# TopAY-Planner/TopAY

Hardware: AMD Instinct MI355X
Metric: trajectories/sec to L-BFGS convergence (benchmark_tables batch) at 1/2/4/8 GPU (higher is better)
Workload: dtype f64

## Files before the change

### topay_amd/csrc/topay_eval.h

```cpp
#pragma once

#include "topay_esdf.h"
#include "topay_eval_ctx.h"
#include "topay_mani.h"
#include "topay_math.h"
#include "topay_minco.h"
#include "topay_wave.h"

namespace topay {

struct GradGate {
  bool always;
  bool has_early;
  double finit, thr , early ;
  bool early_ok;
  double skip_thr;
  __device__ __forceinline__ bool needs(double f) const {
    if (always) return true;
    if (isinf(f) || isnan(f)) return false;
    if (has_early && fabs(finit - f) / (fabs(finit) + 1.0) < early) return true;
    return !(f > thr);
  }
};

struct Basis {
  double b0[6], b1[6], b2[6], b3[6];
};
__device__ __forceinline__ void make_basis(double s1, Basis& B) {
  const double s2 = s1 * s1, s3 = s2 * s1, s4 = s2 * s2, s5 = s3 * s2;
  B.b0[0] = 1.0; B.b0[1] = s1; B.b0[2] = s2; B.b0[3] = s3; B.b0[4] = s4; B.b0[5] = s5;
  B.b1[0] = 0.0; B.b1[1] = 1.0; B.b1[2] = 2.0 * s1; B.b1[3] = 3.0 * s2; B.b1[4] = 4.0 * s3; B.b1[5] = 5.0 * s4;
  B.b2[0] = 0.0; B.b2[1] = 0.0; B.b2[2] = 2.0; B.b2[3] = 6.0 * s1; B.b2[4] = 12.0 * s2; B.b2[5] = 20.0 * s3;
  B.b3[0] = 0.0; B.b3[1] = 0.0; B.b3[2] = 0.0; B.b3[3] = 6.0; B.b3[4] = 24.0 * s1; B.b3[5] = 60.0 * s2;
}
__device__ __forceinline__ void poly4(lds_cdp cL, int rows, int i, int d, const Basis& B, double& p0, double& p1,
                                      double& p2, double& p3) {
  lds_cdp c = cL + d * rows + 6 * i;
  const double c0 = c[0], c1 = c[1], c2 = c[2], c3 = c[3], c4 = c[4], c5 = c[5];
  p0 = fma(c5, B.b0[5], fma(c4, B.b0[4], fma(c3, B.b0[3], fma(c2, B.b0[2], fma(c1, B.b0[1], c0)))));
  p1 = fma(c5, B.b1[5], fma(c4, B.b1[4], fma(c3, B.b1[3], fma(c2, B.b1[2], c1))));
  p2 = fma(c5, B.b2[5], fma(c4, B.b2[4], fma(c3, B.b2[3], c2 * B.b2[2])));
  p3 = fma(c5, B.b3[5], fma(c4, B.b3[4], c3 * B.b3[3]));
}
__device__ __forceinline__ void poly3(lds_cdp cL, int rows, int i, int d, const Basis& B, double& p0, double& p1,
                                      double& p2) {
  lds_cdp c = cL + d * rows + 6 * i;
  const double c0 = c[0], c1 = c[1], c2 = c[2], c3 = c[3], c4 = c[4], c5 = c[5];
  p0 = fma(c5, B.b0[5], fma(c4, B.b0[4], fma(c3, B.b0[3], fma(c2, B.b0[2], fma(c1, B.b0[1], c0)))));
  p1 = fma(c5, B.b1[5], fma(c4, B.b1[4], fma(c3, B.b1[3], fma(c2, B.b1[2], c1))));
  p2 = fma(c5, B.b2[5], fma(c4, B.b2[4], fma(c3, B.b2[3], c2 * B.b2[2])));
}

__device__ __forceinline__ void xy_integrand(lds_cdp cL, int rows, int i, double s1, double& fx, double& fy) {
  const double s2 = s1 * s1, s3 = s2 * s1, s4 = s2 * s2, s5 = s3 * s2;
  lds_cdp ct = cL + 0 * rows + 6 * i;
  lds_cdp cs = cL + 1 * rows + 6 * i;
  const double th = fma(ct[5], s5, fma(ct[4], s4, fma(ct[3], s3, fma(ct[2], s2, fma(ct[1], s1, ct[0])))));
  const double sd = fma(cs[5], 5.0 * s4, fma(cs[4], 4.0 * s3, fma(cs[3], 3.0 * s2, fma(cs[2], 2.0 * s1, cs[1]))));
  double sn, cn;
  det_sincos(th, &sn, &cn);
  fx = sd * cn;
  fy = sd * sn;
}

__device__ __forceinline__ void kinodynamic_block(dev_params_ref P, double wM, double wA, double wD, double omg,
                                                  double step, double real_alpha, double th1, double th2, double th3,
                                                  double sd1, double sd2, double sd3, double& cost, double& gdT,
                                                  double& gth1, double& gth2, double& gs1, double& gs2) {
  const double mu = P.relu_mu;
  const double max_v = P.max_v, max_w = P.max_w, max_a = P.max_a, max_dw = P.max_dw;
  const double w = omg * step;
#pragma unroll
  for (int sgn = -1; sgn <= 1; sgn += 2) {
    const double v = sgn * max_v * th1 + max_w * sd1 - P.max_vw;
    if (v > 0) {
      double pe, pd;
      smoothL1(P, v, mu, pe, pd);
      const double gt = real_alpha * (sgn * max_v * th2 + max_w * sd2);
      gth1 += w * wM * pd * sgn * max_v;
      gs1 += w * wM * pd * max_w;
      gdT += omg * wM * (pd * gt * step + pe * TOPAY_INV_K);
      cost += w * wM * pe;
    }
  }
#pragma unroll
  for (int sgn = -1; sgn <= 1; sgn += 2) {
    const double v = sgn * max_v * th1 - max_w * sd1 - P.max_vw;
    if (v > 0) {
      double pe, pd;
      smoothL1(P, v, mu, pe, pd);
      const double gt = real_alpha * (sgn * max_v * th2 - max_w * sd2);
      gth1 += w * wM * pd * sgn * max_v;
      gs1 -= w * wM * pd * max_w;
      gdT += omg * wM * (pd * gt * step + pe * TOPAY_INV_K);
      cost += w * wM * pe;
    }
  }
  const double vAcc = sd2 * sd2 - P.max_a2;
  const double vAlp = th2 * th2 - P.max_dw2;
  if (vAcc > 0) {
    double pe, pd;
    smoothL1(P, vAcc, mu, pe, pd);
    const double gt = 2.0 * real_alpha * sd2 * sd3;
    gs2 += w * wA * pd * 2.0 * sd2;
    gdT += omg * wA * (pd * gt * step + pe * TOPAY_INV_K);
    cost += w * wA * pe;
  }
  if (vAlp > 0) {
    double pe, pd;
    smoothL1(P, vAlp, mu, pe, pd);
    const double gt = 2.0 * real_alpha * th2 * th3;
    gth2 += w * wD * pd * 2.0 * th2;
    gdT += omg * wD * (pd * gt * step + pe * TOPAY_INV_K);
    cost += w * wD * pe;
  }
}

__device__ __forceinline__ void basis_k(int k, double s, double& b0, double& b1, double& b2) {
  double pm2 = 1.0, pm1 = 1.0, p = 1.0;
#pragma unroll
  for (int t = 1; t <= 5; t++) {
    if (t <= k) p *= s;
    if (t <= k - 1) pm1 *= s;
    if (t <= k - 2) pm2 *= s;
  }
  b0 = p;
  b1 = (k >= 1) ? (double)k * pm1 : 0.0;
  b2 = (k >= 2) ? (double)(k * (k - 1)) * pm2 : 0.0;
}

template <int OCC>
__device__ __forceinline__ ManiOut sample_mani(lds_cdp cL, int rows, int i, int j, int e, bool act, double step, double half, double posx,
                                               double posy, const TOPAY_GLB DevMap* mp, glb_dp mstash, lds_dp mg_lds) {
  ManiOut mo_;
  if (topay_opaque_true()) mo_ = manipulator_block<OCC>(mp, cL, rows, i, j, half, step, posx, posy, act ? e : -1, mstash, mg_lds);
  return mo_;
}

template <int STAGE>
__device__ __forceinline__ void sample_rest(dev_params_ref P, lds_cdp cL, int rows, int i, int j, double step, double half, double posx, double posy,
                                            const TOPAY_GLB DevMap* mp, double wM, double wA, double wD, const ManiOut& mo_, lds_cdp mg_lds,
                                            double (&gB)[12], double& gdTs, double& gpx, double& gpy, bool& jva, double& cst) {
#pragma unroll
  for (int v = 0; v < 12; v++) gB[v] = 0.0;
  gdTs = 0.0; gpx = 0.0; gpy = 0.0;
  jva = false;
  Basis B;
  make_basis(j * half, B);
  const double omg = (j == 0 || j == 2 * TOPAY_K) ? 0.5 : 1.0;
  const double real_alpha = 1.0 / TOPAY_K * ((double)j / 2.0);
  double th0, th1, th2, th3, s0, sd1, sd2, sd3;
  poly4(cL, rows, i, 0, B, th0, th1, th2, th3);
  poly4(cL, rows, i, 1, B, s0, sd1, sd2, sd3);
  cst = 0.0;
  kinodynamic_block(P, wM, wA, wD, omg, step, real_alpha, th1, th2, th3, sd1, sd2, sd3, cst, gdTs, gB[1], gB[2],
                    gB[3], gB[4]);
  if (STAGE == 2) {
    double d2, g2x, g2y;
    {
      const DevMap M = load_map(mp);
      esdf2d_query(M, posx, posy, d2, g2x, g2y);
    }
    const double viola = P.chassis_r105 - d2;
    if (viola > 0) {
      double pe, pd;
      smoothL1(P, viola, P.relu_mu, pe, pd);
      const double sc = -omg * step * P.s2_collision_weight * pd;
      gpx += sc * g2x;
      gpy += sc * g2y;
      gdTs += omg * P.s2_collision_weight * (pe * TOPAY_INV_K);
      cst += omg * step * P.s2_collision_weight * pe;
    }
    double qacc = 0.0;
#pragma unroll
    for (int q = 0; q < 7; q++) {
      double a0, a1, a2, a3;
      poly4(cL, rows, i, 2 + q, B, a0, a1, a2, a3);
      const double vDq = a1 * a1 - P.joint_vel_limit2[q];
      const double vD2q = a2 * a2 - P.joint_acc_limit2[q];
      if (vDq > 0) {
        double pe, pd;
        smoothL1(P, vDq, P.relu_mu, pe, pd);
        gdTs += omg * P.s2_mani_vel_weight * (pd * (2.0 * real_alpha * a1 * a2) * step + pe * TOPAY_INV_K);
        cst += omg * step * P.s2_mani_vel_weight * pe;
        jva = true;
      }
      if (vD2q > 0) {
        double pe, pd;
        smoothL1(P, vD2q, P.relu_mu, pe, pd);
        gdTs += omg * P.s2_mani_acc_weight * (pd * (2.0 * real_alpha * a2 * a3) * step + pe * TOPAY_INV_K);
        cst += omg * step * P.s2_mani_acc_weight * pe;
        jva = true;
      }
      const double mgq = mg_lds[q * 64];
      gB[5 + q] = mgq;
      qacc += mgq * a1;
    }
    cst = cst + mo_.cost;
    gdTs = gdTs + mo_.gdT;
    gpx += mo_.gx;
    gpy += mo_.gy;
    gB[0] = mo_.gth;
    gdTs += mo_.gth * th1 * real_alpha;
    gdTs += qacc * real_alpha;
  }
}

template <int STAGE, int RMAX, int NW, int OCC = 1>
__device__ __noinline__ TOPAY_CALLS_BIG_FUNCTIONS double eval_cost_grad(EvalCtx& C, const TOPAY_GLB DevMap* mp, const GradGate gate) {
  constexpr int NT = 64 * NW;
  const lds_dp c_Tp = uniform_ptr(C.Tp);
  const lds_dp c_X = uniform_ptr(C.X);
  const double c_ex = uniform_f64(C.ex);
  const double c_ey = uniform_f64(C.ey);
  const glb_dp c_g = uniform_ptr(C.g);
  const lds_dp c_gdT = uniform_ptr(C.gdT);
  const glb_cdp c_init_xy = uniform_ptr(C.init_xy);
  const double c_lam0 = uniform_f64(C.lam0);
  const double c_lam1 = uniform_f64(C.lam1);
  const glb_dp c_lu = uniform_ptr(C.lu);
  const lds_dp c_pcs = uniform_ptr(C.pcs);
  const lds_dp c_pw = uniform_ptr(C.pw);
  const double c_rho0 = uniform_f64(C.rho0);
  const double c_rho1 = uniform_f64(C.rho1);
  const double c_sx = uniform_f64(C.sx);
  const double c_sy = uniform_f64(C.sy);
  const glb_cdp c_x = uniform_ptr(C.x);
  const lds_dp c_red = uniform_ptr(C.red);
  const lds_dp c_adj = uniform_ptr(C.adj);
  const glb_dp c_coefg = uniform_ptr(C.coefg);

  dev_params_ref P = dev_params();
  int lane = C.lane, tid = C.tid;
  const int wave = __builtin_amdgcn_readfirstlane(C.wave);
  const int N = __builtin_amdgcn_readfirstlane(C.N), rows = __builtin_amdgcn_readfirstlane(C.rows);
  lds_cdp cL = uniform_ptr(C.cL);
  const glb_dp c_sbuf = uniform_ptr(C.sbuf);
  const glb_dp c_mstash = uniform_ptr(C.mstash);
  const int c_sbs = __builtin_amdgcn_readfirstlane(C.sb_stride);
  const double g_skip_thr = uniform_f64(gate.skip_thr);
  const bool g_early_ok = __builtin_amdgcn_readfirstlane(gate.early_ok ? 1 : 0) != 0;
  GradGate ugate;
  ugate.always = __builtin_amdgcn_readfirstlane(gate.always ? 1 : 0) != 0;
  ugate.has_early = __builtin_amdgcn_readfirstlane(gate.has_early ? 1 : 0) != 0;
  ugate.finit = uniform_f64(gate.finit); ugate.thr = uniform_f64(gate.thr); ugate.early = uniform_f64(gate.early);
  ugate.early_ok = g_early_ok; ugate.skip_thr = g_skip_thr;
  int rp = 0;
  const int npl = __builtin_amdgcn_readfirstlane(C.npass_lds);
  constexpr int RD = eval_red_doubles(NW);
  const lds_dp ptot = c_red + RD;
  const lds_dp csr = c_red + RD + 2 * npl;
  TOPAY_LDS unsigned long long* jmask = (TOPAY_LDS unsigned long long*)(c_red + RD + 2 * npl + (NW > 1 ? 2 * NW * 64 : 0));
  constexpr int PBR = eval_pb_rows(NW);
  minco_generate<NW, OCC>(C);

  auto jerk_terms = [&](int i, double& e_out, double& gdT_out) __attribute__((always_inline)) {
    double w33 = 0, w43 = 0, w44 = 0, w53 = 0, w54 = 0, w55 = 0;
#pragma unroll
    for (int d = 0; d < 9; d++) {
      const double c3 = cL[d * rows + 6 * i + 3], c4 = cL[d * rows + 6 * i + 4], c5 = cL[d * rows + 6 * i + 5];
      const double e = P.energy_weights[d];
      w33 += (c3 * e) * c3; w43 += (c4 * e) * c3; w44 += (c4 * e) * c4;
      w53 += (c5 * e) * c3; w54 += (c5 * e) * c4; w55 += (c5 * e) * c5;
    }
    const double T1 = c_Tp[i], T2 = c_Tp[N + i], T3 = c_Tp[2 * N + i], T4 = c_Tp[3 * N + i], T5 = c_Tp[4 * N + i];
    e_out = 36.0 * w33 * T1 + 144.0 * w43 * T2 + 192.0 * w44 * T3 + 240.0 * w53 * T3 + 720.0 * w54 * T4 + 720.0 * w55 * T5;
    gdT_out = 36.0 * w33 + 288.0 * w43 * T1 + 576.0 * w44 * T2 + 720.0 * w53 * T2 + 2880.0 * w54 * T3 + 3600.0 * w55 * T4;
  };
  double jerk_e = 0.0;
  if (tid < N) {
    double unused_;
    jerk_terms(tid, jerk_e, unused_);
  }
  const double jerk_cost = wg_sum<NW>(c_red, rp, wave, jerk_e);

  lds_dp gxy = c_X;
  lds_dp pball = c_X + 26 * N;
  lds_dp pbuf = pball + wave * (PBR * 64);
  const int NE = TOPAY_EP * N;
  const int npass = (NE + 63) / 64;
  const int nround = (npass + NW - 1) / NW;
  const double wT = STAGE == 1 ? P.s1_time_weight : P.s2_time_weight;
  const double time_cost = wT * wg_sum<NW>(c_red, rp, wave, tid < N ? c_Tp[tid] : 0.0);
  bool skip_body = false;
  double f_skip = 0.0;
  if (STAGE == 2 && g_early_ok) {
    const double partial = jerk_cost + time_cost;
    if (partial > g_skip_thr && partial <= 1.79769313486231570e308) {
      skip_body = true;
      f_skip = partial;
    }
  }
  const double wM = STAGE == 1 ? P.s1_moment_weight : P.s2_moment_weight;
  const double wA = STAGE == 1 ? P.s1_acc_weight : P.s2_acc_weight;
  const double wD = STAGE == 1 ? P.s1_domega_weight : P.s2_domega_weight;

  STAMP(C, 3);
  for (int k = 0; k < nround; k++) {
    const int pass = k * NW + wave;
    if (pass < npass) {
      const int e = pass * 64 + lane;
      const bool act = e < NE;
      const int i = act ? e / TOPAY_EP : N - 1;
      const int m = act ? e - TOPAY_EP * i : 0;
      const int j = 2 * m;
      const double T1 = c_Tp[i];
      const double step = T1 / TOPAY_K, half = step / 2.0, coeff = step / 6.0;
      double f0x, f0y, Ix = 0.0, Iy = 0.0;
      xy_integrand(cL, rows, i, j * half, f0x, f0y);
      if (act && m < TOPAY_K) {
        double f1x, f1y, f2x, f2y;
        xy_integrand(cL, rows, i, (j + 1) * half, f1x, f1y);
        xy_integrand(cL, rows, i, (j + 2) * half, f2x, f2y);
        Ix = coeff * f0x + 4 * coeff * f1x + coeff * f2x;
        Iy = coeff * f0y + 4 * coeff * f1y + coeff * f2y;
      }
      const double incx = wave_incl_scan(Ix, lane), incy = wave_incl_scan(Iy, lane);
      if (act) {
        gxy[2 * e] = incx - Ix;
        gxy[2 * e + 1] = incy - Iy;
      }
      if (lane == 63) {
        ptot[2 * pass] = incx;
        ptot[2 * pass + 1] = incy;
      }
    }
  }
  wg_barrier<NW>();

  double carryx = 0.0, carryy = 0.0;
  int pc = 0;
  double cost_pen = 0.0;
  for (int k = 0; k < nround; k++) {
    const int pass = k * NW + wave;
    double cst_out = 0.0;
    if (pass < npass) {
      while (pc < pass) {
        carryx = uniform_f64(carryx + ptot[2 * pc]);
        carryy = uniform_f64(carryy + ptot[2 * pc + 1]);
        pc++;
      }
      int e, i, m, j;
      bool act;
      double step, half, posx, posy;
      auto geometry = [&](int ln) __attribute__((always_inline)) {
        e = pass * 64 + ln;
        act = e < NE;
        i = act ? e / TOPAY_EP : N - 1;
        m = act ? e - TOPAY_EP * i : 0;
        j = 2 * m;
        const double T1 = c_Tp[i];
        step = T1 / TOPAY_K;
        half = step / 2.0;
        const double px0 = act ? gxy[2 * e] : 0.0, py0 = act ? gxy[2 * e + 1] : 0.0;
        posx = c_sx + (carryx + px0);
        posy = c_sy + (carryy + py0);
      };
      geometry(lane);
      if (act && m == TOPAY_K) {
        c_pcs[2 * N + 2 * (i + 1)] = posx;
        c_pcs[2 * N + 2 * (i + 1) + 1] = posy;
      }
      if (!skip_body) {
        ManiOut mo;
        mo.gx = mo.gy = mo.gth = mo.cost = mo.gdT = 0.0;
        if (STAGE == 2) {
          mo = sample_mani<OCC>(cL, rows, i, j, e, act, step, half, posx, posy, mp, c_mstash, pbuf + lane);
          lane = fresh_lane_id(lane);
          tid = wave * 64 + lane;
          geometry(lane);
        }
        double gB[12], gdTs, gpx, gpy, cst;
        bool jva;
        sample_rest<STAGE>(P, cL, rows, i, j, step, half, posx, posy, mp, wM, wA, wD, mo, pbuf + lane, gB, gdTs, gpx, gpy, jva, cst);
        if (act) {
          cst_out = cst;
          gxy[2 * e] = gpx;
          gxy[2 * e + 1] = gpy;
          glb_dp sb = c_sbuf + e;
          const int ss = c_sbs;
#pragma unroll
          for (int v = 0; v < 5; v++) sb[v * ss] = gB[v];
          sb[5 * ss] = gdTs;
          if (STAGE == 2) {
#pragma unroll
            for (int v = 0; v < 7; v++) sb[(6 + v) * ss] = gB[5 + v];
            sb[13 * ss] = jva ? 1.0 : 0.0;
          }
        }
      }
    }
    lds_dp cs = csr + (k & 1) * (NW * 64);
    if (NW > 1) {
      cs[wave * 64 + lane] = cst_out;
      wg_barrier<NW>();
    }
#pragma unroll
    for (int q = 0; q < NW; q++) {
      const int p2 = k * NW + q;
      if (p2 < npass) {
        cost_pen += NW > 1 ? cs[q * 64 + lane] : cst_out;
        if (STAGE == 2 && g_early_ok && !skip_body && p2 + 1 < npass) {
          const double partial = jerk_cost + wave_sum(cost_pen) + time_cost;
          if (partial > g_skip_thr && partial <= 1.79769313486231570e308) {
            skip_body = true;
            f_skip = partial;
          }
        }
      }
    }
  }
  while (pc < npass) {
    carryx = uniform_f64(carryx + ptot[2 * pc]);
    carryy = uniform_f64(carryy + ptot[2 * pc + 1]);
    pc++;
  }
  if (NW == 1) lds_sync();
  STAMP(C, 4);

  double cost_piece = 0.0;
  double chain0x = 0.0, chain0y = 0.0;
  double mt_add_all = 0.0, mt_add_own = 0.0;
  if (STAGE == 1) {
    if (tid < N) {
      const double ex = c_pcs[2 * N + 2 * (tid + 1)] - c_init_xy[2 * tid];
      const double ey = c_pcs[2 * N + 2 * (tid + 1) + 1] - c_init_xy[2 * tid + 1];
      cost_piece = P.s1_path_pos_weight * (ex * ex + ey * ey);
      c_pcs[2 * tid] = P.s1_path_pos_weight * 2.0 * ex;
      c_pcs[2 * tid + 1] = P.s1_path_pos_weight * 2.0 * ey;
    }
    wg_barrier<NW>();
  } else {
    const double Tm = tid < N ? c_Tp[tid] : 0.0;
    const double avg = wg_sum<NW>(c_red, rp, wave, Tm) / N;
    double add_all = 0.0, add_own = 0.0;
    if (tid < N) {
      const double wMT = P.s2_mean_time_weight;
      if (Tm < avg * 0.5) {
        const double dd = Tm - avg * 0.5;
        cost_piece += wMT * dd * dd;
        add_all += wMT * 2.0 * dd * (-0.5 / N);
        add_own += wMT * 2.0 * dd;
      }
      if (Tm > avg * 2.0) {
        const double dd = Tm - avg * 2.0;
        cost_piece += wMT * dd * dd;
        add_all += wMT * 2.0 * dd * (-2.0 / N);
        add_own += wMT * 2.0 * dd;
      }
    }
    mt_add_all = add_all;
    mt_add_own = add_own;
    C.fxe0 = (c_sx + carryx) - c_ex;
    C.fxe1 = (c_sy + carryy) - c_ey;
    const double ea = C.fxe0 + c_lam0 / c_rho0, eb = C.fxe1 + c_lam1 / c_rho1;
    if (tid == 0) cost_piece += 0.5 * (c_rho0 * (ea * ea) + c_rho1 * (eb * eb));
    chain0x = c_rho0 * ea;
    chain0y = c_rho1 * eb;
  }
  double penalty_cost = wg_sum<NW>(c_red, rp, wave, (wave == 0 ? cost_pen : 0.0) + cost_piece);
  const bool bad = (STAGE == 2) && !(fabs(penalty_cost) <= 1.79769313486231570e308);
  const double f_total = jerk_cost + (bad ? 1.0e+22 : penalty_cost) + time_cost;

  STAMP(C, 5);
  if (skip_body) return f_skip;
  if (!ugate.needs(f_total)) return f_total;

  int rrow[RMAX], rpiece[RMAX], rk[RMAX];
  bool ract[RMAX];
#pragma unroll
  for (int r = 0; r < RMAX; r++) {
    rrow[r] = tid + NT * r;
    ract[r] = rrow[r] < rows;
    rpiece[r] = rrow[r] / 6;
    rk[r] = rrow[r] - 6 * rpiece[r];
  }
  double jerk_gdT = 0.0;
  if (tid < N) {
    double unused_;
    jerk_terms(tid, unused_, jerk_gdT);
  }
  double a0[RMAX], a1[RMAX], aq[RMAX][7];
  double rbh[RMAX][3];
#pragma unroll
  for (int r = 0; r < RMAX; r++) {
    a0[r] = 0.0;
    a1[r] = 0.0;
#pragma unroll
    for (int q = 0; q < 7; q++) aq[r][q] = 0.0;
    rbh[r][0] = rbh[r][1] = rbh[r][2] = 0.0;
    if (ract[r]) {
      const double hs = c_Tp[rpiece[r]] / TOPAY_K / 2.0;
      basis_k(rk[r], hs, rbh[r][0], rbh[r][1], rbh[r][2]);
    }
  }
  constexpr int NV = (STAGE == 2) ? 13 : 6;
  if constexpr (NW == 1) {
    for (int pass = 0; pass < npass; pass++) {
      const int e = pass * 64 + lane;
      const bool act = e < NE;
      const int i = act ? e / TOPAY_EP : N - 1;
      const int m = act ? e - TOPAY_EP * i : 0;
      const int j = 2 * m;
      const double step = c_Tp[i] / TOPAY_K, half = step / 2.0;
      bool jva = false;
      double rawq[7];
      {
        glb_cdp sb = c_sbuf + (act ? e : NE - 1);
        const int ss = c_sbs;
        double raw[14];
#pragma unroll
        for (int v = 0; v < ((STAGE == 2) ? 14 : 6); v++) raw[v] = sb[v * ss];
#pragma unroll
        for (int v = 0; v < 6; v++) pbuf[v * 64 + lane] = act ? raw[v] : 0.0;
#pragma unroll
        for (int v = 0; v < 7; v++) rawq[v] = (STAGE == 2 && act) ? raw[6 + v] : 0.0;
        if (STAGE == 2) jva = act && raw[13] != 0.0;
      }
      lds_sync();
#pragma unroll
      for (int r = 0; r < RMAX; r++) {
        if (ract[r]) {
          const int pi = rpiece[r];
          const double h0 = rbh[r][0], h1 = rbh[r][1], h2 = rbh[r][2];
          const int k0 = rk[r], k1 = rk[r] >= 1 ? rk[r] - 1 : 0, k2 = rk[r] >= 2 ? rk[r] - 2 : 0;
          const int e_lo = max(TOPAY_EP * pi, pass * 64), e_hi = min(min(TOPAY_EP * pi + TOPAY_EP, pass * 64 + 64), NE);
          double gt = 0.0;
          constexpr int CH = 3;
          for (int c0 = e_lo; c0 < e_hi; c0 += CH) {
            double pb[CH][6], t0[CH], t1[CH], t2[CH];
#pragma unroll
            for (int u = 0; u < CH; u++) {
              const int ee = (c0 + u < e_hi) ? c0 + u : e_hi - 1;
              const int l = ee - pass * 64, mm = ee - TOPAY_EP * pi;
              lds_cdp pj = c_pw + 12 * mm;
              t0[u] = pj[k0]; t1[u] = pj[k1]; t2[u] = pj[k2];
#pragma unroll
              for (int v = 0; v < 6; v++) pb[u][v] = pbuf[v * 64 + l];
            }
#pragma unroll
            for (int u = 0; u < CH; u++) {
              const bool ok = c0 + u < e_hi;
              const double b0 = h0 * t0[u], b1 = h1 * t1[u], b2 = h2 * t2[u];
              const double i0 = fma(b2, pb[u][2], fma(b1, pb[u][1], b0 * pb[u][0]));
              const double i1 = fma(b2, pb[u][4], b1 * pb[u][3]);
              a0[r] += ok ? i0 : 0.0;
              a1[r] += ok ? i1 : 0.0;
              gt += ok ? pb[u][5] : 0.0;
            }
          }
          if (e_lo < e_hi && rk[r] == 0) c_gdT[pi] += gt;
        }
      }
      if (STAGE == 2) {
        lds_sync();
#pragma unroll
        for (int v = 0; v < 7; v++) pbuf[v * 64 + lane] = rawq[v];
// ... 99 lines not shown
      double raw[14];
#pragma unroll
      for (int v = 0; v < ((STAGE == 2) ? 14 : 6); v++) raw[v] = sb[v * ss];
#pragma unroll
      for (int v = 0; v < 6; v++) pbuf[v * 64 + lane] = act ? raw[v] : 0.0;
      if (STAGE == 2) {
#pragma unroll
        for (int v = 0; v < 7; v++) pbuf[(6 + v) * 64 + lane] = act ? raw[6 + v] : 0.0;
        jva = act && raw[13] != 0.0;
      }
    }
    if (STAGE == 2) {
      const unsigned long long mk = __ballot(jva);
      if (lane == 0) jmask[wave] = mk;
    }
    wg_barrier<NW>();
    auto accumulate = [&](int r, int q) __attribute__((always_inline)) {
      const int p2 = k * NW + q;
      const int pi = rpiece[r];
      const double h0 = rbh[r][0], h1 = rbh[r][1], h2 = rbh[r][2];
      const int k0 = rk[r], k1 = rk[r] >= 1 ? rk[r] - 1 : 0, k2 = rk[r] >= 2 ? rk[r] - 2 : 0;
      const int e_lo = max(TOPAY_EP * pi, p2 * 64), e_hi = min(min(TOPAY_EP * pi + TOPAY_EP, p2 * 64 + 64), NE);
      if (e_lo >= e_hi) return;
      lds_cdp pq = pball + q * (PBR * 64);
      double gt = 0.0;
      constexpr int CH = 3;
      for (int c0 = e_lo; c0 < e_hi; c0 += CH) {
        double pb[CH][NV], t0[CH], t1[CH], t2[CH];
#pragma unroll
        for (int u = 0; u < CH; u++) {
          const int ee = (c0 + u < e_hi) ? c0 + u : e_hi - 1;
          const int l = ee - p2 * 64, mm = ee - TOPAY_EP * pi;
          lds_cdp pj = c_pw + 12 * mm;
          t0[u] = pj[k0]; t1[u] = pj[k1]; t2[u] = pj[k2];
#pragma unroll
          for (int v = 0; v < NV; v++) pb[u][v] = pq[v * 64 + l];
        }
#pragma unroll
        for (int u = 0; u < CH; u++) {
          const bool ok = c0 + u < e_hi;
          const double b0 = h0 * t0[u], b1 = h1 * t1[u], b2 = h2 * t2[u];
          const double i0 = fma(b2, pb[u][2], fma(b1, pb[u][1], b0 * pb[u][0]));
          const double i1 = fma(b2, pb[u][4], b1 * pb[u][3]);
          a0[r] += ok ? i0 : 0.0;
          a1[r] += ok ? i1 : 0.0;
          gt += ok ? pb[u][5] : 0.0;
          if (STAGE == 2) {
#pragma unroll
            for (int qq = 0; qq < 7; qq++) {
              const double nq = fma(b0, pb[u][6 + qq], aq[r][qq]);
              aq[r][qq] = ok ? nq : aq[r][qq];
            }
          }
        }
      }
      if (rk[r] == 0) c_gdT[pi] += gt;
    };
    unsigned long long any = 0;
    if (STAGE == 2) {
#pragma unroll
      for (int q = 0; q < NW; q++) any |= jmask[q];
    }
    if (any == 0) {
#pragma unroll
      for (int r = 0; r < RMAX; r++) {
        if (ract[r]) {
          for (int q = 0; q < NW; q++) accumulate(r, q);
        }
      }
    } else {
      for (int q = 0; q < NW; q++) {
#pragma unroll
        for (int r = 0; r < RMAX; r++) {
          if (ract[r]) accumulate(r, q);
        }
        unsigned long long todo = jmask[q];
        if (todo == 0) continue;
        wg_barrier<NW>();
        if (wave == q && jva) {
          Basis B;
          make_basis(j * half, B);
          const double omg = (j == 0 || j == 2 * TOPAY_K) ? 0.5 : 1.0;
#pragma unroll
          for (int qq = 0; qq < 7; qq++) {
            double p0, p1, p2, g1 = 0.0, g2 = 0.0;
            poly3(cL, rows, i, 2 + qq, B, p0, p1, p2);
            const double vDq = p1 * p1 - P.joint_vel_limit2[qq];
            const double vD2q = p2 * p2 - P.joint_acc_limit2[qq];
            if (vDq > 0) {
              double pe, pd;
              smoothL1(P, vDq, P.relu_mu, pe, pd);
              g1 = omg * step * P.s2_mani_vel_weight * pd * 2.0 * p1;
            }
            if (vD2q > 0) {
              double pe, pd;
              smoothL1(P, vD2q, P.relu_mu, pe, pd);
              g2 = omg * step * P.s2_mani_acc_weight * pd * 2.0 * p2;
            }
            pbuf[qq * 64 + lane] = g1;
            pbuf[(7 + qq) * 64 + lane] = g2;
          }
        }
        wg_barrier<NW>();
        lds_cdp pq = pball + q * (PBR * 64);
        while (todo) {
          const int src = __ffsll(todo) - 1;
          todo &= todo - 1;
          const int se = (k * NW + q) * 64 + src;
          const int spi = se / TOPAY_EP, smm = se - TOPAY_EP * spi;
          double b1v[7], b2v[7];
#pragma unroll
          for (int qq = 0; qq < 7; qq++) { b1v[qq] = pq[qq * 64 + src]; b2v[qq] = pq[(7 + qq) * 64 + src]; }
#pragma unroll
          for (int r = 0; r < RMAX; r++) {
            if (ract[r] && rpiece[r] == spi) {
              const int k1 = rk[r] >= 1 ? rk[r] - 1 : 0, k2 = rk[r] >= 2 ? rk[r] - 2 : 0;
              const double b1 = rbh[r][1] * c_pw[12 * smm + k1], b2 = rbh[r][2] * c_pw[12 * smm + k2];
#pragma unroll
              for (int qq = 0; qq < 7; qq++) {
                double a = aq[r][qq];
                a = fma(b1, b1v[qq], a);
                a = fma(b2, b2v[qq], a);
                aq[r][qq] = a;
              }
            }
          }
        }
      }
    }
    wg_barrier<NW>();
  }

  }
  if (STAGE == 2) {
    const double all = wg_sum<NW>(c_red, rp, wave, mt_add_all);
    if (tid < N) c_gdT[tid] += all + mt_add_own;
  }
  wg_barrier<NW>();
  if (!bad) {
    if (STAGE == 2) {
      for (int k = 0; k < nround; k++) {
        const int pass = k * NW + wave;
        if (pass < npass) {
          const int e = pass * 64 + lane;
          const bool act = e < NE;
          const double gx = act ? gxy[2 * e] : 0.0, gy = act ? gxy[2 * e + 1] : 0.0;
          const double sx_ = wave_incl_rscan(gx, lane), sy_ = wave_incl_rscan(gy, lane);
          if (lane == 0) {
            ptot[2 * pass] = sx_;
            ptot[2 * pass + 1] = sy_;
          }
        }
      }
      wg_barrier<NW>();
    }
    double rcx = chain0x, rcy = chain0y;
    pc = npass;
    for (int k = nround - 1; k >= 0; k--) {
      const int pass = k * NW + wave;
      double v0 = 0, v1 = 0, v2 = 0, v3 = 0, vT = 0;
      if (pass < npass) {
        const int e = pass * 64 + lane;
        const bool act = e < NE;
        const int i = act ? e / TOPAY_EP : N - 1;
        const int m = act ? e - TOPAY_EP * i : 0;
        const int j = 2 * m;
        double chx_in, chy_in, chx_ex, chy_ex;
        if (STAGE == 2) {
          while (pc > pass + 1) {
            pc--;
            rcx += ptot[2 * pc];
            rcy += ptot[2 * pc + 1];
          }
          const double gx = act ? gxy[2 * e] : 0.0, gy = act ? gxy[2 * e + 1] : 0.0;
          const double sx_ = wave_incl_rscan(gx, lane), sy_ = wave_incl_rscan(gy, lane);
          chx_in = sx_ + rcx; chy_in = sy_ + rcy;
          chx_ex = chx_in - gx;   chy_ex = chy_in - gy;
        } else {
          double sx_ = 0.0, sy_ = 0.0;
          for (int ii = i + 1; ii < N; ii++) { sx_ += c_pcs[2 * ii]; sy_ += c_pcs[2 * ii + 1]; }
          chx_in = chx_ex = sx_;
          chy_in = chy_ex = sy_;
        }
        if (act) {
          const double T1 = c_Tp[i];
          const double step = T1 / TOPAY_K, half = step / 2.0, coeff = step / 6.0;
          const int int_6K = TOPAY_K * 6;
#pragma unroll
          for (int odd = 0; odd < 2; odd++) {
            if (odd == 1 && m == TOPAY_K) break;
            const int jj = j + odd;
            Basis B;
            make_basis(jj * half, B);
            double th0, th1, th2, s0, sd1, sd2;
            poly3(cL, rows, i, 0, B, th0, th1, th2);
            poly3(cL, rows, i, 1, B, s0, sd1, sd2);
            double sn, cn;
            det_sincos(th0, &sn, &cn);
            const double alpha = 1.0 / (2 * TOPAY_K) * jj;
            const double W = odd ? 4.0 : ((jj == 0 || jj == 2 * TOPAY_K) ? 1.0 : 2.0);
            const double Cx = (odd ? chx_ex : chx_in) * W, Cy = (odd ? chy_ex : chy_in) * W;
            const double aTh = (-sd1 * sn * coeff) * Cx + (sd1 * cn * coeff) * Cy;
            const double aS = (cn * coeff) * Cx + (sn * coeff) * Cy;
            const double gTx = (sd2 * cn - sd1 * th1 * sn) * alpha * coeff + sd1 * cn / int_6K;
            const double gTy = (sd2 * sn + sd1 * th1 * cn) * alpha * coeff + sd1 * sn / int_6K;
            vT += gTx * Cx + gTy * Cy;
            if (odd) { v2 = aTh; v3 = aS; } else { v0 = aTh; v1 = aS; }
          }
        }
      }
      pbuf[0 * 64 + lane] = v0; pbuf[1 * 64 + lane] = v1; pbuf[2 * 64 + lane] = v2; pbuf[3 * 64 + lane] = v3;
      pbuf[4 * 64 + lane] = vT;
      wg_barrier<NW>();
#pragma unroll
      for (int r = 0; r < RMAX; r++) {
        if (ract[r]) {
          const int pi = rpiece[r];
          const double h0 = rbh[r][0], h1 = rbh[r][1];
          const int k1 = rk[r] >= 1 ? rk[r] - 1 : 0;
          for (int q = NW - 1; q >= 0; q--) {
            const int p2 = k * NW + q;
            const int e_lo = max(TOPAY_EP * pi, p2 * 64), e_hi = min(min(TOPAY_EP * pi + TOPAY_EP, p2 * 64 + 64), NE);
            if (e_lo >= e_hi) continue;
            lds_cdp pq = pball + q * (PBR * 64);
            double gt = 0.0;
            constexpr int CH = 3;
            for (int c0 = e_lo; c0 < e_hi; c0 += CH) {
              double pb[CH][5], tb[CH][4];
#pragma unroll
              for (int u = 0; u < CH; u++) {
                const int ee = (c0 + u < e_hi) ? c0 + u : e_hi - 1;
                const int l = ee - p2 * 64, mm = ee - TOPAY_EP * pi;
                lds_cdp pj = c_pw + 12 * mm;
                tb[u][0] = pj[rk[r]]; tb[u][1] = pj[k1]; tb[u][2] = pj[6 + rk[r]]; tb[u][3] = pj[6 + k1];
#pragma unroll
                for (int v = 0; v < 5; v++) pb[u][v] = pq[v * 64 + l];
              }
#pragma unroll
              for (int u = 0; u < CH; u++) {
                const bool ok = c0 + u < e_hi;
                const double b0 = h0 * tb[u][0], b1 = h1 * tb[u][1];
                const double o0 = h0 * tb[u][2], o1 = h1 * tb[u][3];
                const double i0 = fma(o0, pb[u][2], b0 * pb[u][0]);
                const double i1 = fma(o1, pb[u][3], b1 * pb[u][1]);
                a0[r] += ok ? i0 : 0.0;
                a1[r] += ok ? i1 : 0.0;
                gt += ok ? pb[u][4] : 0.0;
              }
            }
            if (rk[r] == 0) c_gdT[pi] += gt;
          }
        }
      }
      wg_barrier<NW>();
    }
  } else {
    penalty_cost = 1.0e+22;
#pragma unroll
    for (int r = 0; r < RMAX; r++) {
      a0[r] = 0.0;
      a1[r] = 0.0;
#pragma unroll
      for (int q = 0; q < 7; q++) aq[r][q] = 0.0;
    }
    if (tid < N) c_gdT[tid] = 0.0;
    wg_barrier<NW>();
  }

  STAMP(C, 6);
  double tot[RMAX][9];
#pragma unroll
  for (int r = 0; r < RMAX; r++) {
    if (ract[r]) {
      const int pi = rpiece[r], kk = rk[r];
      const double T1 = c_Tp[pi], T2 = c_Tp[N + pi], T3 = c_Tp[2 * N + pi], T4 = c_Tp[3 * N + pi], T5 = c_Tp[4 * N + pi];
#pragma unroll
      for (int d = 0; d < 9; d++) {
        double jg = 0.0;
        if (kk >= 3) {
          const double c3 = cL[d * rows + 6 * pi + 3], c4 = cL[d * rows + 6 * pi + 4], c5 = cL[d * rows + 6 * pi + 5];
          const double e = P.energy_weights[d];
          if (kk == 5) jg = 240.0 * c3 * e * T3 + 720.0 * c4 * e * T4 + 1440.0 * c5 * e * T5;
          else if (kk == 4) jg = 144.0 * c3 * e * T2 + 384.0 * c4 * e * T3 + 720.0 * c5 * e * T4;
          else jg = 72.0 * c3 * e * T1 + 144.0 * c4 * e * T2 + 240.0 * c5 * e * T3;
        }
        tot[r][d] = jg + (d == 0 ? a0[r] : (d == 1 ? a1[r] : aq[r][d >= 2 ? d - 2 : 0]));
      }
    }
  }
  for (int t = tid; t < 9 * rows; t += NT) c_coefg[t] = cL[t];
  C.cl_in_lds = 0;
  wg_global_barrier<NW>();
#pragma unroll
  for (int r = 0; r < RMAX; r++) {
    if (ract[r]) {
#pragma unroll
      for (int d = 0; d < 9; d++) c_adj[d * rows + rrow[r]] = tot[r][d];
    }
  }
  wg_barrier<NW>();
  if (wave == 0) {
    const bool owner = lane < 9;
    const lds_dp mine = c_adj + (owner ? lane : 8) * rows;
    band_sweep<2>(mine, owner, (glb_cdp)c_lu, c_X, rows, lane);
    band_sweep<3>(mine, owner, (glb_cdp)c_lu, c_X, rows, lane);
  }
  wg_barrier<NW>();
  STAMP(C, 7);
#pragma unroll
  for (int r = 0; r < RMAX; r++) {
    if (ract[r]) {
      const int row = rrow[r];
      int pi, br;
      bool use = true;
      if (row >= rows - 3) { pi = N - 1; br = 10 + (row - (rows - 3)); }
      else if (row < 3) { use = false; pi = 0; br = 0; }
      else { pi = (row - 3) / 6; br = (row - 3) - 6 * pi; }
      double part = 0.0;
      if (use) {
        const double T1 = c_Tp[pi], T2 = c_Tp[N + pi], T3 = c_Tp[2 * N + pi], T4 = c_Tp[3 * N + pi];
#pragma unroll
        for (int d = 0; d < 9; d++) {
          glb_cdp cg = c_coefg + d * rows + 6 * pi;
          const double c1 = cg[1], c2 = cg[2], c3 = cg[3], c4 = cg[4], c5 = cg[5];
          double b;
          if (br == 0) b = -(24.0 * c4 + 120.0 * T1 * c5);
          else if (br == 1) b = -120.0 * c5;
          else if (br == 2 || br == 3 || br == 10) b = -(c1 + 2.0 * T1 * c2 + 3.0 * T2 * c3 + 4.0 * T3 * c4 + 5.0 * T4 * c5);
          else if (br == 4 || br == 11) b = -(2.0 * c2 + 6.0 * T1 * c3 + 12.0 * T2 * c4 + 20.0 * T3 * c5);
          else b = -(6.0 * c3 + 24.0 * T1 * c4 + 60.0 * T2 * c5);
          part += b * c_adj[d * rows + row];
        }
      }
      c_X[row] = part;
    }
  }
  wg_barrier<NW>();
  double gdT_tot = 0.0;
  if (tid < N) {
    const int i = tid;
    double s = 0.0;
    if (i < N - 1) { for (int r = 0; r < 6; r++) s += c_X[6 * i + 3 + r]; }
    else { for (int r = 0; r < 3; r++) s += c_X[rows - 3 + r]; }
    gdT_tot = jerk_gdT + c_gdT[i] + s;
  }
  glb_cdp Tau = c_x;
  glb_cdp Vq = c_x + 3 * N - 1;
  if (tid < N) c_g[tid] = (gdT_tot + wT) * dTdTau(Tau[tid]);
  for (int t = tid; t < 9 * (N - 1); t += NT) {
    const int i = t / 9, d = t - 9 * i;
    const double gp = c_adj[d * rows + 6 * i + 5];
    const int dq = d >= 2 ? d - 2 : 0;
    if (d == 0) c_g[N + i] = gp;
    else if (d == 1) c_g[2 * N - 1 + i] = gp;
    else c_g[3 * N - 1 + 7 * i + dq] = gp * dQdVq(Vq[7 * i + dq], P.joint_pos_limit_max[dq]);
  }
  if (tid == 0) c_g[3 * N - 2] = c_adj[1 * rows + rows - 3];
  wg_global_barrier<NW>();
  STAMP(C, 8);
  return f_total;
}

}
```

### topay_amd/csrc/topay_eval_ctx.h

```cpp
#pragma once

#include <hip/hip_runtime.h>

#include "topay_types.h"

__constant__ DevParams g_P;
typedef const TOPAY_CST DevParams& dev_params_ref;
__device__ __forceinline__ dev_params_ref dev_params() {
#ifndef TOPAY_CPU_EMU
  const TOPAY_CST DevParams* p = (const TOPAY_CST DevParams*)&g_P;
  asm("" : "+s"(p));
  return *p;
#else
  return g_P;
#endif
}

namespace topay {

__device__ __forceinline__ double expC2(double tau) {
  return tau > 0.0 ? ((0.5 * tau + 1.0) * tau + 1.0) : 1.0 / ((0.5 * tau - 1.0) * tau + 1.0);
}
__device__ __forceinline__ double logC2(double T) {
  return T > 1.0 ? (sqrt(2.0 * T - 1.0) - 1.0) : (1.0 - sqrt(2.0 / T - 1.0));
}
__device__ __forceinline__ double dTdTau(double tau) {
  if (tau > 0) return tau + 1.0;
  double den = (0.5 * tau - 1.0) * tau + 1.0;
  return (1.0 - tau) / (den * den);
}
__device__ __forceinline__ double sigmoidC2(double vq, double max_q) {
  double e = expC2(vq);
  return 2.0 * max_q * e / (1.0 + e) - max_q;
}
__device__ __forceinline__ double invSigmoidC2(double q, double max_q) {
  double b = 0.5 * (max_q + q) / max_q;
  return logC2(b / (1 - b));
}
__device__ __forceinline__ double dQdVq(double vq, double max_q) {
  double e1 = expC2(vq) + 1.0;
  return 2.0 * max_q * dTdTau(vq) / (e1 * e1);
}
__device__ __forceinline__ void smoothL1(dev_params_ref P, double x, double mu, double& f, double& df) {
  if (x < mu) {
    f = (P.sl_f4c * x + P.sl_f3c) * x * x * x;
    df = (P.sl_d3c * x + P.sl_d2c) * x * x;
  } else {
    f = x - P.sl_half;
    df = 1.0;
  }
}
#define TOPAY_INV_K (1.0 / TOPAY_K)

struct EvalCtx {
  int lane, N, rows, n;
  int tid, wave;
  lds_dp red;
  lds_dp adj;
  glb_dp coefg;
  int cl_in_lds;
  lds_dp cL;
  lds_dp Tp;
  glb_cdp hd, tl;
  int npass_lds;
  lds_dp gdT;
  lds_dp pcs;
  lds_dp gC;
  glb_dp sbuf;
  int sb_stride;
  glb_dp mstash;
  lds_dp pw;
  lds_dp X;
  glb_cdp x;
  glb_dp g;
  glb_dp lu;
  glb_cdp init_xy;
  double sx, sy, ex, ey;
  double lam0, lam1, rho0, rho1;
  double fxe0, fxe1;
  TOPAY_GLB long long* stamps;
  long long t_last;
};

__device__ __forceinline__ void fill_power_table(lds_dp pw, int lane) {
  for (int t = lane; t < 156; t += 64) {
    const int jj = t / 6, k = t - 6 * jj;
    double v = 1.0;
    for (int u = 0; u < k; u++) v *= (double)jj;
    pw[t] = v;
  }
}

#ifdef TOPAY_STAMPS
#define STAMP(C, k)                                                    \
  do {                                                                 \
    const long long now_ = (long long)__builtin_amdgcn_s_memtime();    \
    if ((C).stamps && (C).lane == 0) (C).stamps[k] += now_ - (C).t_last; \
    (C).t_last = (long long)__builtin_amdgcn_s_memtime();              \
  } while (0)
#else
#define STAMP(C, k) do { } while (0)
#endif
#ifdef TOPAY_STAMPS
#define SUBSTAMP_BEGIN(C) const long long sub_t0_ = (long long)__builtin_amdgcn_s_memtime()
#define SUBSTAMP_END(C, k)                                                                                   \
  do {                                                                                                       \
    if ((C).stamps && (C).lane == 0) (C).stamps[k] += (long long)__builtin_amdgcn_s_memtime() - sub_t0_;      \
  } while (0)
#else
#define SUBSTAMP_BEGIN(C) do { } while (0)
#define SUBSTAMP_END(C, k) do { } while (0)
#endif

__host__ __device__ constexpr int eval_pb_rows(int NW) { return NW == 1 ? 7 : 14; }
__host__ __device__ constexpr int eval_npass(int Nmax) { return (TOPAY_EP * Nmax + 63) / 64; }
__host__ __device__ constexpr int eval_red_doubles(int NW) { return NW > 1 ? 8 : 0; }
__host__ __device__ constexpr int eval_misc_doubles(int Nmax, int NW) {
  return eval_red_doubles(NW) + 2 * eval_npass(Nmax) + (NW > 1 ? 2 * NW * 64 : 0) + NW;
}
__host__ __device__ constexpr int eval_union_doubles(int Nmax, int NW) {
  const int rows = 6 * Nmax;
  const int lu = 14 * rows, sw = 9 * rows + 26 * Nmax + eval_pb_rows(NW) * 64 * NW;
  return lu > sw ? lu : sw;
}
__host__ __device__ constexpr int eval_borrow_doubles(int Nmax, int NW) { return eval_union_doubles(Nmax, NW) - 9 * 6 * Nmax; }
template <typename P>
struct EvalLds {
  P Tp, gdT, pcs, pw, red, cL, adj, gC, X;
};
template <typename L, typename P>
__host__ __device__ constexpr P eval_lds_plan(L& C, P base, int Nmax, int NW) {
  const int rows = 6 * Nmax;
  P p = base;
  C.Tp = p; p += 5 * Nmax;
  C.gdT = p; p += Nmax;
  C.pcs = p; p += 4 * (Nmax + 1);
  C.pw = p; p += 156;
  C.red = p; p += eval_misc_doubles(Nmax, NW);
  C.cL = p;
  C.adj = C.cL;
  C.gC = C.adj;
  C.X = p + 9 * rows;
  return p + eval_union_doubles(Nmax, NW);
}
__host__ __device__ constexpr int eval_lds_total(int Nmax, int NW) {
  EvalLds<int> offsets{};
  return eval_lds_plan(offsets, 0, Nmax, NW);
}
__device__ __forceinline__ void eval_lds_carve(EvalCtx& C, lds_dp base, int Nmax, int NW) {
  eval_lds_plan(C, base, Nmax, NW);
  C.npass_lds = eval_npass(Nmax);
}
static_assert(eval_lds_total(10, 1) == 1515 && eval_lds_total(15, 1) == 1967 && eval_lds_total(21, 1) == 2509 &&
              eval_lds_total(32, 1) == 3503 && eval_lds_total(42, 1) == 4407 && eval_lds_total(64, 1) == 6395, "LDS plan, one wave");
static_assert(eval_lds_total(42, 2) == 6016 && eval_lds_total(64, 2) == 8004, "LDS plan, two waves");
static_assert(eval_lds_total(10, 4) == 5174 && eval_lds_total(15, 4) == 5626 && eval_lds_total(21, 4) == 6168 &&
              eval_lds_total(32, 4) == 7162 && eval_lds_total(42, 4) == 8066 && eval_lds_total(64, 4) == 10054 &&
              eval_lds_total(85, 4) == 11954 && eval_lds_total(128, 4) == 15840 && eval_lds_total(TOPAY_MAX_N, 4) == 19638,
              "LDS plan, four waves");

}
```

### topay_amd/csrc/topay_host_batch.h

```cpp

#pragma once

static topay_status run_init(topay_ctx* c) {
  const int B = c->B;
  topay_status ps = push_params(c);
  if (ps != TOPAY_OK) return ps;
  const int scratch_stride = (3 * c->Pmax + 1 + TOPAY_MAX_N) * ND;
  hipLaunchKernelGGL(k_init, dim3((B + 63) / 64), dim3(64), 0, c->stream, c->db, c->paths.as<double>(),
                     c->path_off.as<long long>(), c->path_len.as<int>(), c->bvel.as<double>(), c->bacc.as<double>(),
                     c->scratch.as<double>(), scratch_stride, TOPAY_MAX_N, kX0Stride);
  HIPCHK(hipGetLastError());
  return TOPAY_OK;
}

static topay_status set_init_traj_impl(topay_ctx* c, int batch, const int* path_len, const double* init_paths, const double* boundary_vel,
                                       const double* boundary_acc, const int* map_ids, hipMemcpyKind kind) {
  if (!c || batch <= 0 || !path_len || !init_paths) return TOPAY_ERR_INVALID_ARG;
  HIPCHK(hipSetDevice(c->device));
  if (topay_status ws = wait_pending(c)) return ws;
  c->have_traj = false;
  c->solved = false;
  std::vector<long long> off(batch + 1, 0);
  int Pmax = 0;
  for (int b = 0; b < batch; b++) {
    if (path_len[b] < 2) { set_err("every init path needs at least 2 states"); return TOPAY_ERR_INVALID_ARG; }
    off[b + 1] = off[b] + path_len[b];
    Pmax = std::max(Pmax, path_len[b]);
  }
  if (check_map_slots(c, batch, map_ids, kMapResident, "topay_set_init_traj") != TOPAY_OK) return TOPAY_ERR_NO_MAP;
  std::vector<int> mids(batch, 0);
  if (map_ids) mids.assign(map_ids, map_ids + batch);
  c->B = batch;
  c->Pmax = Pmax;
  c->h_map_id = mids;
  const size_t tot = (size_t)off[batch];
  topay_status s;
#define ENS(buf, bytes) if ((s = c->buf.ensure(bytes)) != TOPAY_OK) return s
  ENS(paths, tot * 10 * 8);
  ENS(path_off, (size_t)(batch + 1) * 8);
  ENS(path_len, (size_t)batch * 4);
  ENS(bvel, (size_t)batch * 20 * 8);
  ENS(bacc, (size_t)batch * 20 * 8);
  ENS(scratch, (size_t)batch * (3 * Pmax + 1 + TOPAY_MAX_N) * ND * 8);
  ENS(N, (size_t)batch * 4);
  ENS(s1_past, (size_t)batch * 4);
  ENS(map_id, (size_t)batch * 4);
  ENS(head, (size_t)batch * kHeadLen * 8);
  ENS(tail, (size_t)batch * kHeadLen * 8);
  ENS(start_xy, (size_t)batch * 2 * 8);
  ENS(goal_xy, (size_t)batch * 2 * 8);
  ENS(init_xy, (size_t)batch * kInitXyStride * 8);
  ENS(x0, (size_t)batch * kX0Stride * 8);
  ENS(order, (size_t)batch * 4);
  HIPCHK(copy_sync(c, c->paths.as<double>(), init_paths, tot * 10, kind));
  HIPCHK(h2d_sync(c, c->path_off.as<long long>(), off.data(), (size_t)(batch + 1)));
  HIPCHK(h2d_sync(c, c->path_len.as<int>(), path_len, (size_t)batch));
  HIPCHK(h2d_sync(c, c->map_id.as<int>(), mids.data(), (size_t)batch));
  if (boundary_vel) HIPCHK(copy_sync(c, c->bvel.as<double>(), boundary_vel, (size_t)batch * 20, kind));
  else HIPCHK(hipMemsetAsync(c->bvel.p, 0, (size_t)batch * 20 * 8, c->stream));
  if (boundary_acc) HIPCHK(h2d_sync(c, c->bacc.as<double>(), boundary_acc, (size_t)batch * 20));
  else HIPCHK(hipMemsetAsync(c->bacc.p, 0, (size_t)batch * 20 * 8, c->stream));
  DevBatch& d = c->db;
  memset(&d, 0, sizeof(d));
  d.B = batch;
  d.N = c->N.as<int>(); d.s1_past = c->s1_past.as<int>(); d.map_id = c->map_id.as<int>();
  d.head = c->head.as<double>(); d.tail = c->tail.as<double>();
  d.start_xy = c->start_xy.as<double>(); d.goal_xy = c->goal_xy.as<double>();
  d.init_xy = c->init_xy.as<double>(); d.x0 = c->x0.as<double>();
  d.order = c->order.as<int>();
  if ((s = run_init(c)) != TOPAY_OK) return s;
  HIPCHK(hipStreamSynchronize(c->stream));
  c->hN.assign(batch, 0);
  HIPCHK(d2h_sync(c, c->hN.data(), c->N.as<int>(), (size_t)batch));
  int Nmax = 0;
  for (int b = 0; b < batch; b++) {
    if (c->hN[b] <= 0) c->hN[b] = 0;
    Nmax = std::max(Nmax, c->hN[b]);
  }
  if (Nmax == 0) { set_err("every trajectory needs more pieces than TOPAY_MAX_N"); return TOPAY_ERR_TOO_MANY_PIECES; }
  c->Nmax = Nmax;
  c->h_poff.assign((size_t)batch + 1, 0);
  c->h_noff.assign((size_t)batch + 1, 0);
  for (int b = 0; b < batch; b++) {
    c->h_poff[b + 1] = c->h_poff[b] + c->hN[b];
    c->h_noff[b + 1] = c->h_noff[b] + (c->hN[b] > 0 ? 10 * c->hN[b] - 8 : 0);
  }
  const size_t P = (size_t)c->h_poff[batch], NN = (size_t)c->h_noff[batch];
  const int m = std::max(c->hp.s1_lbfgs.mem_size, c->hp.s2_lbfgs.mem_size);
  std::vector<int> idx(batch);
  std::iota(idx.begin(), idx.end(), 0);
  std::stable_sort(idx.begin(), idx.end(), [&](int a, int b2) {
    return c->hN[a] != c->hN[b2] ? c->hN[a] > c->hN[b2] : path_len[a] > path_len[b2];
  });
  for (auto& v : c->cls) v.clear();
  for (int b : idx) {
    if (c->hN[b] == 0) continue;
    c->cls[bucket_of(c->hN[b])].push_back(b);
  }
  c->h_path_len.assign(path_len, path_len + batch);
  {
    std::vector<int> ord;
    for (int k = topay_ctx::NBUCKET - 1; k >= 0; k--) ord.insert(ord.end(), c->cls[k].begin(), c->cls[k].end());
    ord.resize(batch, 0);
    HIPCHK(h2d_sync(c, c->order.as<int>(), ord.data(), (size_t)batch));
  }
  ENS(poff, ((size_t)batch + 1) * 8);
  ENS(noff, ((size_t)batch + 1) * 8);
  HIPCHK(h2d_sync(c, c->poff.as<long long>(), c->h_poff.data(), ((size_t)batch + 1)));
  HIPCHK(h2d_sync(c, c->noff.as<long long>(), c->h_noff.data(), ((size_t)batch + 1)));
  ENS(x, NN * 8);
  ENS(work, 4 * NN * 8);
  ENS(hist_s, (size_t)m * NN * 8);
  ENS(hist_y, (size_t)m * NN * 8);
  ENS(hist_ys, (size_t)batch * m * 8);
  ENS(hist_alpha, (size_t)batch * m * 8);
  ENS(lu, kLuPerPiece * P * 8);
  ENS(success, (size_t)batch * 4);
  ENS(cost, (size_t)batch * 8);
  ENS(stats, (size_t)batch * kStatsLen * 4);
  ENS(xyerr, (size_t)batch * 2 * 8);
  ENS(coef, kCoefPerPiece * P * 8);
  ENS(T, P * 8);
  ENS(knots, 2 * (P + batch) * 8);
  ENS(alm, (size_t)batch * kAlmLen * 8);
  ENS(fout, (size_t)batch * 8);
  ENS(sbuf, kSbufPerPiece * P * 8);
  ENS(mstash, kMstashPerPiece * P * 8);
  ENS(elapsed, (size_t)batch * 8);
  ENS(startus, (size_t)batch * 8);
  ENS(hwid, (size_t)batch * 4);
  ENS(feas_flags, (size_t)batch * 2 * 4);
  ENS(feas_report, (size_t)batch * kReportLen * 8);
  ENS(interrupted, (size_t)batch * 4);
#undef ENS
  {
    DevBuf* all[] = {&c->paths, &c->path_off, &c->path_len, &c->bvel, &c->bacc, &c->scratch, &c->N, &c->s1_past, &c->map_id, &c->head, &c->tail,
                     &c->start_xy, &c->goal_xy, &c->init_xy, &c->x0, &c->order, &c->poff, &c->noff, &c->x, &c->work, &c->hist_s, &c->hist_y,
                     &c->hist_ys, &c->hist_alpha, &c->lu, &c->success, &c->cost, &c->stats, &c->xyerr, &c->coef, &c->T, &c->knots, &c->alm,
                     &c->fout, &c->sbuf, &c->mstash, &c->elapsed, &c->startus, &c->hwid};
    c->workspace_bytes = 0;
    for (DevBuf* q : all) c->workspace_bytes += q->bytes;
  }
  d.hist_m = m;
  d.poff = c->poff.as<long long>(); d.noff = c->noff.as<long long>();
  d.x = c->x.as<double>(); d.work = c->work.as<double>();
  d.hist_s = c->hist_s.as<double>(); d.hist_y = c->hist_y.as<double>();
  d.hist_ys = c->hist_ys.as<double>(); d.hist_alpha = c->hist_alpha.as<double>();
  d.lu = c->lu.as<double>();
  d.success = c->success.as<int>(); d.cost = c->cost.as<double>(); d.stats = c->stats.as<int>();
  d.xyerr = c->xyerr.as<double>(); d.coef = c->coef.as<double>(); d.T = c->T.as<double>();
  d.knots = c->knots.as<double>(); d.alm = c->alm.as<double>(); d.fout = c->fout.as<double>();
  d.sbuf = c->sbuf.as<double>();
  d.mstash = c->mstash.as<double>();
  d.elapsed_us = c->elapsed.as<double>();
  d.start_us = c->startus.as<double>();
  d.hw_id = c->hwid.as<int>();
  d.gate_in_solve = 1;
  d.feas_flags = c->feas_flags.as<int>();
  d.feas_report = c->feas_report.as<double>();
  d.interrupted = c->interrupted.as<int>();
  HIPCHK(hipMemsetAsync(c->interrupted.p, 0, (size_t)batch * 4, c->stream));
  c->h_group.clear();
  c->n_groups = 0;
  d.group_id = nullptr; d.group_tau = nullptr; d.cancel_budget = 0; d.cancel_flag = nullptr;
  c->gate_done = false;
  HIPCHK(hipMemsetAsync(c->elapsed.p, 0, (size_t)batch * 8, c->stream));
  HIPCHK(hipMemsetAsync(c->success.p, 0, (size_t)batch * 4, c->stream));
  HIPCHK(hipMemsetAsync(c->cost.p, 0xFF, (size_t)batch * 8, c->stream));
  HIPCHK(hipMemsetAsync(c->stats.p, 0, (size_t)batch * kStatsLen * 4, c->stream));
  c->have_traj = true;
  return TOPAY_OK;
}

static void compute_grids(topay_ctx* c, const int* nm, double cus, int* grid) {
  const ClassDef* ct = kClassTable;
  double wt[topay_ctx::NBUCKET] = {0}, rk[topay_ctx::NBUCKET] = {0}, need = 0.0;
  for (int k = 0; k < topay_ctx::NBUCKET; k++) {
    grid[k] = 0;
    if (c->cls[k].empty()) continue;
    double t = ct[k].nw == 1 ? 1.0 : (ct[k].nw == 2 ? 1.0 / 1.48 : 0.5);
    const double regs = (double)ct[k].nw / (4.0 * ct[k].occ), lds = (double)class_lds_bytes(ct[k], nm[k]) / (160.0 * 1024.0);
    rk[k] = std::max(regs, lds);
    if (ct[k].occ == 2 && lds <= 0.1875) t *= 2.0 / kOcc2Gain;
    if (k == 0) t *= 0.8;
    for (int b : c->cls[k]) wt[k] += t * std::pow((double)c->hN[b], 1.5);
    need += wt[k] * rk[k];
  }
  if (need <= 0.0) return;
  const double G = cus / need;
  for (int k = 0; k < topay_ctx::NBUCKET; k++) {
    if (c->cls[k].empty()) continue;
    grid[k] = std::max(1, std::min((int)c->cls[k].size(), (int)std::floor(G * wt[k] + 0.5)));
  }
}

static std::once_flag g_attr_once[16];
static hipError_t g_attr_err[16];
static hipError_t set_kernel_attributes(int device) {
  std::call_once(g_attr_once[device % 16], [device] {
    (void)device;
    hipError_t e = hipSuccess;
    const ClassDef* ct = kClassTable;
    const int lds = kLdsDoublesPerCU * 8;
    for (int k = 0; k < TOPAY_NBUCKET && e == hipSuccess; k++) {
      e = hipFuncSetAttribute((const void*)ct[k].solve, hipFuncAttributeMaxDynamicSharedMemorySize, lds);
      if (e == hipSuccess) e = hipFuncSetAttribute((const void*)ct[k].eval, hipFuncAttributeMaxDynamicSharedMemorySize, lds);
      if (e == hipSuccess && ct[k].lat) e = hipFuncSetAttribute((const void*)ct[k].lat, hipFuncAttributeMaxDynamicSharedMemorySize, lds);
    }
    g_attr_err[device % 16] = e;
  });
  return g_attr_err[device % 16];
}

static int steal_floor(int k) {
  const ClassDef* ct = kClassTable;
  int lo = k;
  while (lo > 0 && ct[lo - 1].nw == ct[k].nw && ((lo - 1 >= kBigFirst) == (k >= kBigFirst))) lo--;
  return lo;
}

template <bool EVAL, typename... Args>
static topay_status launch_classes(topay_ctx* c, bool persistent, Args... args) {
  const ClassDef* ct = kClassTable;
  int launches = 0, helper_launches = 0, off = 0;
  topay_status ps = push_params(c);
  if (ps != TOPAY_OK) return ps;
  HIPCHK(set_kernel_attributes(c->device));
  int slots = 0;
  if (persistent) {
    if (c->qnext.ensure(sizeof(int) * topay_ctx::NBUCKET) != TOPAY_OK) return TOPAY_ERR_NO_DEVICE;
    HIPCHK(hipMemsetAsync(c->qnext.p, 0, sizeof(int) * topay_ctx::NBUCKET, c->stream));
    slots = c->simd_slots;
  }
  int pgrid[topay_ctx::NBUCKET] = {0}, nmk[topay_ctx::NBUCKET] = {0};
  for (int k = 0; k < topay_ctx::NBUCKET; k++) {
    for (int b : c->cls[k]) nmk[k] = std::max(nmk[k], c->hN[b]);
    if (persistent && c->steal)
      for (int k2 = steal_floor(k); k2 < k; k2++)
        for (int b : c->cls[k2]) nmk[k] = std::max(nmk[k], c->hN[b]);
  }
  if (persistent) {
    compute_grids(c, nmk, slots / 4.0 * 1.08, pgrid);
  }
  HIPCHK(hipEventRecord(c->bstart, c->stream));
  for (int k = topay_ctx::NBUCKET - 1; k >= 0; k--) {
    const std::vector<int>& v = c->cls[k];
    const int nk = (int)v.size();
    if (nk == 0) continue;
    const int nm = nmk[k];
    DevBatch d = c->db;
    d.order = c->db.order + off;
    int grid = nk;
    if (persistent) {
      d.order = c->db.order;
      d.queue_next = c->qnext.as<int>();
      d.queue_class = k;
      d.queue_lowest = c->steal ? steal_floor(k) : k;
      int o2 = 0;
      for (int kk = topay_ctx::NBUCKET - 1; kk >= 0; kk--) {
        d.queue_off[kk] = o2;
        d.queue_count[kk] = (int)c->cls[kk].size();
        o2 += d.queue_count[kk];
      }
      grid = pgrid[k];
    }
    off += nk;
    const bool lat = !EVAL && ct[k].lat && (c->latency_mode == 2 || (c->latency_mode == 1 && c->B <= c->simd_slots));
    size_t lds = class_lds_bytes(ct[k], nm);
    if (lat) {
      lds = (size_t)(eval_lds_total(nm, kLatWaves) + solve_tail_doubles(true)) * sizeof(double);
      grid = nk;
    }
    if (k == topay_ctx::NBUCKET - 2 && !c->cls[topay_ctx::NBUCKET - 1].empty() && c->bstream[k] == c->stream)
      HIPCHK(hipStreamCreateWithFlags(&c->bstream[k], hipStreamNonBlocking));
    hipStream_t st = c->bstream[k];
    if (st != c->stream) HIPCHK(hipStreamWaitEvent(st, c->bstart, 0));
    if constexpr (EVAL) hipLaunchKernelGGL(ct[k].eval, dim3(grid), dim3(64 * ct[k].nw), lds, st, d, (const DevMap*)c->dmaps.p, args..., nm);
    else if (lat) { hipLaunchKernelGGL(ct[k].lat, dim3(grid), dim3(64 * kLatWaves), lds, st, d, (const DevMap*)c->dmaps.p, nm); helper_launches++; }
    else hipLaunchKernelGGL(ct[k].solve, dim3(grid), dim3(64 * ct[k].nw), lds, st, d, (const DevMap*)c->dmaps.p, nm);
    HIPCHK(hipGetLastError());
    if (st != c->stream) HIPCHK(hipEventRecord(c->bevent[k], st));
    launches++;
  }
  for (int k = 0; k < topay_ctx::NBUCKET; k++)
    if (!c->cls[k].empty() && c->bstream[k] != c->stream) HIPCHK(hipStreamWaitEvent(c->stream, c->bevent[k], 0));
  c->last_launches = launches;
  c->last_helper_launches = helper_launches;
  return TOPAY_OK;
}


static bool batch_done(topay_ctx* p) { return !p->pending || hipStreamQuery(p->stream) == hipSuccess; }

static topay_status upload_order(topay_ctx* c, bool shortest_first) {
  std::vector<int> ord;
  for (int k = topay_ctx::NBUCKET - 1; k >= 0; k--) {
    std::vector<int>& v = c->cls[k];
    if (shortest_first) std::stable_sort(v.begin(), v.end(), [&](int a, int b2) { return c->hN[a] < c->hN[b2]; });
    else std::stable_sort(v.begin(), v.end(), [&](int a, int b2) {
      return c->hN[a] != c->hN[b2] ? c->hN[a] > c->hN[b2] : (c->h_path_len[a] != c->h_path_len[b2] ? c->h_path_len[a] > c->h_path_len[b2] : a < b2);
    });
    ord.insert(ord.end(), v.begin(), v.end());
  }
  ord.resize(c->B, 0);
  HIPCHK(h2d_sync(c, c->order.as<int>(), ord.data(), (size_t)c->B));
  return TOPAY_OK;
}

extern "C" {

topay_status topay_set_init_traj(topay_ctx* c, int batch, const int* path_len, const double* init_paths,
                                 const double* boundary_vel, const double* boundary_acc, const int* map_ids) {
  return set_init_traj_impl(c, batch, path_len, init_paths, boundary_vel, boundary_acc, map_ids, hipMemcpyHostToDevice);
}

topay_status topay_reset(topay_ctx* c) {
  if (!c || !c->have_traj) return TOPAY_ERR_NO_TRAJ;
  HIPCHK(hipSetDevice(c->device));
  if (topay_status ws = wait_pending(c)) return ws;
  c->solved = false;
  return run_init(c);
}

topay_status topay_optimize_async(topay_ctx* c) {
  if (!c || !c->have_traj) return TOPAY_ERR_NO_TRAJ;
  HIPCHK(hipSetDevice(c->device));
  if (topay_status s0 = wait_pending(c)) return s0;
  {
    std::lock_guard<std::mutex> lk(g_issue_mutex);
    topay_ctx* p = g_last_issued;
    if (p && p != c && p->pending && p->device == c->device && p->h_started) {
      volatile int* cnt = p->h_started;
      const auto t0 = std::chrono::steady_clock::now();
      while (*cnt < p->n_gate) {
        if (batch_done(p)) break;
        if (std::chrono::steady_clock::now() - t0 > std::chrono::seconds(120)) {
          c->gate_timeouts++;
          set_err("dispatch gate: the previous batch did not become resident within 120 s; issuing anyway");
          break;
        }
        std::this_thread::sleep_for(std::chrono::microseconds(100));
      }
    }
    c->h_started[0] = 0;
    int nl = 0, ng = 0;
    for (int k = 0; k < topay_ctx::NBUCKET; k++) {
      nl += (int)c->cls[k].size();
      if (k < kBigFirst) ng += (int)c->cls[k].size();
    }
    c->n_launched = nl;
    c->n_gate = ng;
    c->db.gate_maxN = kBucketMaxN[kBigFirst - 1];
    void* dp = nullptr;
    HIPCHK(hipHostGetDevicePointer(&dp, c->h_started, 0));
    c->db.started = (int*)dp;
    g_last_issued = c;
  }
  HIPCHK(c->solve_timer.start(c->stream));
  c->h_cancel[0] = 0;
  {
    void* dp = nullptr;
    HIPCHK(hipHostGetDevicePointer(&dp, c->h_cancel, 0));
    c->db.cancel_flag = (const int*)dp;
  }
  c->h_started[12] = 0;
  {
    void* dp = nullptr;
    HIPCHK(hipHostGetDevicePointer(&dp, c->h_started + 12, 0));
    c->db.gate_truncated = (int*)dp;
  }
  c->db.cancel_budget = c->n_groups > 0 ? c->cancel_budget : 0;
  if (c->n_groups > 0) HIPCHK(hipMemsetAsync(c->group_tau.p, 0x7f, (size_t)c->n_groups * 4, c->stream));
  HIPCHK(hipMemsetAsync(c->interrupted.p, 0, (size_t)c->B * 4, c->stream));
  HIPCHK(hipMemsetAsync(c->feas_flags.p, 0, (size_t)c->B * 8, c->stream));
  c->gate_done = false;
  HIPCHK(hipMemsetAsync(c->success.p, 0, (size_t)c->B * 4, c->stream));
  HIPCHK(hipMemsetAsync(c->cost.p, 0xFF, (size_t)c->B * 8, c->stream));
  topay_status s = launch_classes<false>(c, c->persistent);
  if (s != TOPAY_OK) {
    for (int k = 0; k < topay_ctx::NBUCKET; k++)
      if (c->bstream[k]) (void)hipStreamSynchronize(c->bstream[k]);
    (void)hipStreamSynchronize(c->stream);
    return s;
  }
  HIPCHK(c->solve_timer.stop(c->stream));
  c->pending = true;
  return TOPAY_OK;
}

topay_status topay_synchronize(topay_ctx* c) {
  if (!c) return TOPAY_ERR_INVALID_ARG;
  HIPCHK(hipSetDevice(c->device));
  HIPCHK(hipStreamSynchronize(c->stream));
  if (c->pending) {
    HIPCHK(c->solve_timer.read(&c->last_ms));
    c->solved = true;
    c->pending = false;
    c->gate_done = c->h_started[12] == 0;
    if (c->n_groups > 0 && c->cancel_budget > 0) {
      const int B = c->B;
      std::vector<int> succ(B), st((size_t)B * kStatsLen), fl((size_t)B * 2), intr(B), tau(c->n_groups);
      HIPCHK(d2h_sync(c, succ.data(), c->success.as<int>(), (size_t)B));
      HIPCHK(d2h_sync(c, st.data(), c->stats.as<int>(), st.size()));
      HIPCHK(d2h_sync(c, fl.data(), c->feas_flags.as<int>(), fl.size()));
      HIPCHK(d2h_sync(c, intr.data(), c->interrupted.as<int>(), (size_t)B));
      HIPCHK(d2h_sync(c, tau.data(), c->group_tau.as<int>(), (size_t)c->n_groups));
      bool changed = false;
      for (int b = 0; b < B; b++) {
        const int g = c->h_group[b];
        if (g < 0 || intr[b] || c->hN[b] == 0) continue;
        const int* sb = &st[(size_t)b * kStatsLen];
        const long long clock = (long long)(sb[2] + sb[5]) * c->hN[b];
        if (clock > (long long)tau[g] + c->cancel_budget) {
          intr[b] = 1; succ[b] = 0; fl[2 * b] = 0; fl[2 * b + 1] = 0;
          st[(size_t)b * kStatsLen + 3] = TOPAY_INTERRUPTED;
          changed = true;
        }
      }
      if (changed) {
        HIPCHK(h2d_sync(c, c->success.as<int>(), succ.data(), (size_t)B));
        HIPCHK(h2d_sync(c, c->stats.as<int>(), st.data(), st.size()));
        HIPCHK(h2d_sync(c, c->feas_flags.as<int>(), fl.data(), fl.size()));
        HIPCHK(h2d_sync(c, c->interrupted.as<int>(), intr.data(), (size_t)B));
      }
    }
  }
  return TOPAY_OK;
}

topay_status topay_set_groups(topay_ctx* c, const int* group_id, int cancel_budget) {
  if (!c || !c->have_traj) return TOPAY_ERR_NO_TRAJ;
  if (cancel_budget < 0) return TOPAY_ERR_INVALID_ARG;
  HIPCHK(hipSetDevice(c->device));
  if (topay_status ws = wait_pending(c)) return ws;
  const bool had_groups = c->n_groups > 0;
  c->h_group.clear();
  c->n_groups = 0;
  c->cancel_budget = cancel_budget;
  c->db.group_id = nullptr; c->db.group_tau = nullptr;
  if (!group_id || cancel_budget == 0) {
    if (had_groups) return upload_order(c, false);
    return TOPAY_OK;
  }
  if (std::max(c->hp.s1_lbfgs.mem_size, c->hp.s2_lbfgs.mem_size) < 64) {
    set_err("cancellation window: the L-BFGS mem_size must be at least 64 (the in-solve gate works in the history block)");
    return TOPAY_ERR_INVALID_ARG;
  }
  std::vector<int> dense(c->B, -1);
  {
    std::vector<int> ids;
    for (int b = 0; b < c->B; b++) {
      if (group_id[b] < -1) return TOPAY_ERR_INVALID_ARG;
      if (group_id[b] >= 0) ids.push_back(group_id[b]);
    }
    std::sort(ids.begin(), ids.end());
    ids.erase(std::unique(ids.begin(), ids.end()), ids.end());
    for (int b = 0; b < c->B; b++)
      if (group_id[b] >= 0) dense[b] = (int)(std::lower_bound(ids.begin(), ids.end(), group_id[b]) - ids.begin());
    c->n_groups = (int)ids.size();
  }
  const int ng = c->n_groups;
  c->h_group = dense;
  if (ng == 0) { c->cancel_budget = cancel_budget; return TOPAY_OK; }
  topay_status s;
  if ((s = c->group_id.ensure((size_t)c->B * 4)) != TOPAY_OK) return s;
  if ((s = c->group_tau.ensure((size_t)std::max(1, ng) * 4)) != TOPAY_OK) return s;
  HIPCHK(h2d_sync(c, c->group_id.as<int>(), dense.data(), (size_t)c->B));
  c->db.group_id = c->group_id.as<int>();
  c->db.group_tau = c->group_tau.as<int>();
  return upload_order(c, true);
}

topay_status topay_set_latency_mode(topay_ctx* c, int mode) {
  if (!c || mode < 0 || mode > 2) return TOPAY_ERR_INVALID_ARG;
  c->latency_mode = mode;
  return TOPAY_OK;
}

topay_status topay_cancel(topay_ctx* c) {
  if (!c) return TOPAY_ERR_INVALID_ARG;
  if (c->h_cancel) __atomic_store_n(c->h_cancel, 1, __ATOMIC_RELEASE);
  return TOPAY_OK;
}

topay_status topay_get_interrupted(topay_ctx* c, int* interrupted) {
  if (!c || !c->have_traj || !interrupted) return TOPAY_ERR_NO_TRAJ;
  HIPCHK(hipSetDevice(c->device));
  if (topay_status ws = wait_pending(c)) return ws;
  HIPCHK(d2h_sync(c, interrupted, c->interrupted.as<int>(), (size_t)c->B));
  return TOPAY_OK;
}

topay_status topay_optimize(topay_ctx* c) {
  topay_status s = topay_optimize_async(c);
  if (s != TOPAY_OK) return s;
  return topay_synchronize(c);
}

topay_status topay_optimize_within(topay_ctx* c, double budget_ms, int* timed_out) {
  if (timed_out) *timed_out = 0;
  if (!(budget_ms > 0.0)) return TOPAY_ERR_INVALID_ARG;
  const auto t0 = std::chrono::steady_clock::now();
  topay_status s = topay_optimize_async(c);
  if (s != TOPAY_OK) return s;
  while (hipStreamQuery(c->stream) == hipErrorNotReady) {
    if (std::chrono::duration<double, std::milli>(std::chrono::steady_clock::now() - t0).count() >= budget_ms) {
      (void)topay_cancel(c);
      if (timed_out) *timed_out = 1;
      break;
    }
    std::this_thread::sleep_for(std::chrono::microseconds(200));
  }
  return topay_synchronize(c);
}

}
```

### topay_amd/csrc/topay_host_ctx.h

```cpp

#pragma once

static thread_local std::string g_err;
static void set_err(const std::string& s) { g_err = s; }
#define HIPCHK(call)                                                                             \
  do {                                                                                           \
    hipError_t e_ = (call);                                                                      \
    if (e_ != hipSuccess) {                                                                      \
      set_err(std::string(#call) + ": " + hipGetErrorString(e_));                                \
      return TOPAY_ERR_NO_DEVICE;                                                                \
    }                                                                                            \
  } while (0)


struct Carver {
  uintptr_t base;
  size_t off = 0;
  explicit Carver(void* b = nullptr) : base((uintptr_t)b) {}
  template <typename T> T* take(size_t count) {
    off = (off + alignof(T) - 1) & ~(alignof(T) - 1);
    T* q = (T*)(base + off);
    off += count * sizeof(T);
    return q;
  }
};

struct DevBuf {
  void* p = nullptr;
  size_t bytes = 0;
  DevBuf() = default;
  DevBuf(const DevBuf&) = delete; DevBuf& operator=(const DevBuf&) = delete;
  DevBuf(DevBuf&& o) noexcept { *this = std::move(o); }
  DevBuf& operator=(DevBuf&& o) noexcept {
    if (this != &o) { release(); p = o.p; bytes = o.bytes; o.p = nullptr; o.bytes = 0; }
    return *this;
  }
  ~DevBuf() { release(); }
  topay_status ensure(size_t n) {
    if (n <= bytes) return TOPAY_OK;
    release();
    const hipError_t e_ = hipMalloc(&p, n);
    if (e_ != hipSuccess) {
      p = nullptr;
      set_err("device allocation of " + std::to_string(n >> 20) + " MiB failed: " + hipGetErrorString(e_));
      return TOPAY_ERR_NO_DEVICE;
    }
    bytes = n;
    return TOPAY_OK;
  }
  topay_status ensure_keep(hipStream_t stream, size_t need, size_t used) {
    if (need <= bytes) return TOPAY_OK;
    DevBuf nb;
    const topay_status s = nb.ensure(std::max(need, 2 * bytes));
    if (s != TOPAY_OK) return s;
    if (used > 0 && p) {
      hipError_t e = hipMemcpyAsync(nb.p, p, used, hipMemcpyDeviceToDevice, stream);
      if (e == hipSuccess) e = hipStreamSynchronize(stream);
      if (e != hipSuccess) { set_err(std::string("grow_keep: ") + hipGetErrorString(e)); return TOPAY_ERR_NO_DEVICE; }
    }
    *this = std::move(nb);
    return TOPAY_OK;
  }
  void release() {
    if (p) (void)hipFree(p);
    p = nullptr;
    bytes = 0;
  }
  template <typename T> T* as() { return (T*)p; }
  template <typename F> topay_status carve(F&& lay) {
    Carver size;
    lay(size);
    const topay_status s = ensure(size.off);
    Carver at(p);
    if (s == TOPAY_OK) lay(at);
    return s;
  }
  template <typename B> topay_status place(B& block) {
    return carve([&](Carver& k) { block.lay(k); });
  }
};

struct DevTimer {
  hipEvent_t a = nullptr, b = nullptr;
  bool stopped = false;
  DevTimer() = default;
  DevTimer(const DevTimer&) = delete; DevTimer& operator=(const DevTimer&) = delete;
  DevTimer(DevTimer&& o) noexcept { *this = std::move(o); }
  DevTimer& operator=(DevTimer&& o) noexcept {
    if (this != &o) { release(); a = o.a; b = o.b; stopped = o.stopped; o.a = o.b = nullptr; o.stopped = false; }
    return *this;
  }
  ~DevTimer() { release(); }
  hipError_t start(hipStream_t stream) {
    stopped = false;
    hipError_t e = a ? hipSuccess : hipEventCreate(&a);
    if (e == hipSuccess && !b) e = hipEventCreate(&b);
    return e == hipSuccess ? hipEventRecord(a, stream) : e;
  }
  hipError_t stop(hipStream_t stream) {
    const hipError_t e = hipEventRecord(b, stream);
    stopped = e == hipSuccess;
    return e;
  }
  hipError_t read(double* ms) const {
    float f = 0.f;
    const hipError_t e = stopped ? hipEventElapsedTime(&f, a, b) : hipErrorNotReady;
    if (e == hipSuccess) *ms = f;
    return e;
  }
  void release() {
    if (a) (void)hipEventDestroy(a);
    if (b) (void)hipEventDestroy(b);
    a = b = nullptr;
    stopped = false;
  }
};

static const int kBucketMaxN[TOPAY_NBUCKET] = {10, 15, 21, 32, 42, 64, TOPAY_MAX_N};
static const int kBigFirst = 4;

typedef void (*solve_kernel_t)(DevBatch, const DevMap*, int);
typedef void (*eval_kernel_t)(DevBatch, const DevMap*, int, int, int);
struct ClassDef {
  int max_n, rmax, nw;
  solve_kernel_t solve;
  eval_kernel_t eval;
  int occ = 2;
  solve_kernel_t lat = nullptr;
  int solver_rmax = 0;
  int srmax() const { return solver_rmax ? solver_rmax : rmax; }
  bool helpers() const { return nw > 1; }
};
static const int kLatWaves = 4;
static const ClassDef kClassTable[TOPAY_NBUCKET] = {
    {10, 1, 1, k_solve1, k_eval1, 2, k_lat1}, {15, 2, 1, k_solve2, k_eval2, 2, k_lat2}, {21, 2, 1, k_solve2, k_eval2, 2, k_lat2},
    {32, 3, 1, k_solve3, k_eval3, 2, k_lat3},
    {42, 2, 4, k_long5, k_eval2w4, 2, nullptr, 5}, {64, 2, 4, k_long5, k_eval2w4, 2, nullptr, 5},
    {TOPAY_MAX_N, 4, 4, k_long14, k_eval4w4, 2, nullptr, 14}};
static const double kOcc2Gain = 1.7;
static const int kLdsDoublesPerCU = 160 * 1024 / 8;
static size_t class_lds_bytes(const ClassDef& cd, int nm) {
  return (size_t)(eval_lds_total(nm, cd.nw) + solve_tail_doubles(cd.helpers())) * sizeof(double);
}

__attribute__((constructor)) static void topay_request_hw_queues() { setenv("GPU_MAX_HW_QUEUES", "24", 0); }
struct topay_ctx;
static std::mutex g_issue_mutex;
static std::mutex g_registry_mutex;
static std::vector<topay_ctx*> g_contexts;

static topay_ctx* g_last_issued = nullptr;

struct PlanStore {
  struct Entry { int n_pieces = 0, piece0 = 0, knot0 = 0, front0 = 0, front_len = 0; };
  struct Winners {
    std::vector<int> call, idx, piece_off{0}, front_off{0};
    void add(int p, int b, int n_pieces, int front_len) {
      call.push_back(p); idx.push_back(b);
      piece_off.push_back(piece_off.back() + n_pieces); front_off.push_back(front_off.back() + front_len);
    }
    size_t size() const { return idx.size(); }
  };
  struct Dest { double *dur, *coef, *knots, *front; };

  void reset(int n_calls) { calls.assign((size_t)n_calls, Entry()); pieces = winners = states = 0; }
  void clear() { calls.clear(); }
  bool empty() const { return calls.empty(); }
  bool has(int call) const { return call >= 0 && call < (int)calls.size(); }
  const Entry& entry(int call) const { return calls[(size_t)call]; }
  size_t n_pieces() const { return pieces; }
  double* durations() { return dur.as<double>(); }
  double* coeffs() { return coef.as<double>(); }
  double* knots() { return kn.as<double>(); }
  double* fronts() { return front.as<double>(); }
  static long long front_double0(const Entry& e) { return 10ll * e.front0; }

  topay_status reserve(hipStream_t stream, const Winners& W, Dest& d) {
    const size_t np = (size_t)W.piece_off.back(), nw = W.size(), ns = (size_t)W.front_off.back();
    for (size_t w = 0; w < nw; w++) {
      Entry& e = calls[(size_t)W.call[w]];
      e.n_pieces = W.piece_off[w + 1] - W.piece_off[w];
      e.piece0 = (int)pieces + W.piece_off[w];
      e.knot0 = (int)pieces + (int)winners + W.piece_off[w] + (int)w;
      e.front0 = (int)states + W.front_off[w];
      e.front_len = W.front_off[w + 1] - W.front_off[w];
    }
    topay_status s;
    if ((s = dur.ensure_keep(stream, (pieces + np) * 8, pieces * 8)) != TOPAY_OK ||
        (s = coef.ensure_keep(stream, (pieces + np) * kCoefPerPiece * 8, pieces * kCoefPerPiece * 8)) != TOPAY_OK ||
        (s = kn.ensure_keep(stream, 2 * (pieces + winners + np + nw) * 8, 2 * (pieces + winners) * 8)) != TOPAY_OK ||
        (s = front.ensure_keep(stream, (states + ns) * 80, states * 80)) != TOPAY_OK)
      return s;
    d.dur = durations() + pieces; d.coef = coeffs() + kCoefPerPiece * pieces; d.knots = knots() + 2 * (pieces + winners); d.front = fronts() + 10 * states;
    return TOPAY_OK;
  }
  void appended(const Winners& W) { pieces += (size_t)W.piece_off.back(); winners += W.size(); states += (size_t)W.front_off.back(); }

 private:
  DevBuf dur, coef, kn, front;
  std::vector<Entry> calls;
  size_t pieces = 0, winners = 0, states = 0;
};

struct PlanWork {
  DevBuf raw, jps_io;
  DevBuf io, tab, mc;
  DevBuf paths, bvel;
  DevBuf idx, win;
  std::vector<DevTimer> timers;
  std::vector<int> timer_stage;
  double stage_ms[TOPAY_PLAN_MS_LEN] = {0};
  int chunk = 0;
};

struct FrontState {
  DevBuf mc_i, mc_d, mc_k, mc_rs, mc_in;
  int mc_n = 0, mc_node_cap = 0;
  DevBuf tp_i, tp_d, tp_raw, tp_pts, tp_io;
  int tp_n = 0, tp_pt_cap = 0, tp_nbuf = 0;
  topay_topo_params_t tp_P;
  DevTimer tp_timer;
};

struct TrackSlot { topay::TrackDesc d[2] = {{0, 0, 0}, {0, 0, 0}}; long long cap[2] = {0, 0}; double T[2] = {0, 0}; };
struct TrackState {
  DevBuf arena, stage, io;
  size_t used = 0;
  std::vector<TrackSlot> slots;
  DevTimer safe_timer;
  double safe_ms = 0.0;
  const topay::TrackDesc* find(int robot, int w) const { return slots.empty() || slots[robot].d[w].N <= 0 ? nullptr : &slots[robot].d[w]; }
};

struct EeState {
  DevBuf hist, io;
  DevTimer timer;
  double ms = 0.0;
};

struct WorldState {
  DevBuf occ, prims, io;
  int first = 0, n = 0, dims[3] = {0, 0, 0}, path = 0;
  int force_path = 0, max_tries = 0;
  enum { kGen, kRaster, kFields, kSample };
  DevTimer timer[4];
  double ms[4] = {0, 0, 0, 0};
  static size_t pad16(size_t bytes) { return (bytes + 15) & ~(size_t)15; }
  const signed char* occ3_of(int slot, int* d) const {
    if (n <= 0 || slot < first || slot >= first + n || !occ.p) return nullptr;
    for (int a = 0; a < 3; a++) d[a] = dims[a];
    return (const signed char*)occ.p + (size_t)(slot - first) * dims[0] * dims[1] * dims[2];
  }
  const signed char* occ2_of(int slot, bool critical) const {
    const size_t n2 = (size_t)dims[0] * dims[1], b3 = pad16((size_t)n * n2 * dims[2]), b2 = pad16((size_t)n * n2);
    return (const signed char*)occ.p + b3 + (critical ? b2 : 0) + (size_t)(slot - first) * n2;
  }
  void forget(int first_, int n_) {
    if (n > 0 && first_ < first + n && first < first_ + n_) { n = 0; occ.release(); }
  }
};

struct SenseBelief {
  DevBuf buf;
  float* logodds = nullptr; int* cnt = nullptr; int* box = nullptr;
  topay_map_desc_t desc;
  topay_sense_params_t prm;
  int batch_counter = 0, pending_rays = 0;
  size_t occ3_off = 0, occ2_off = 0, occ2c_off = 0;
  bool have = false, have_occ = false;
};
struct SenseState {
  std::vector<SenseBelief> slot;
  DevBuf pts, io, scan, occ;
  size_t scan_points = 0;
  enum { kScan, kInsert, kFlush, kCommit };
  DevTimer timer[4];
  double ms[4] = {0, 0, 0, 0};
  bool has_belief(int m) const { return m >= 0 && m < (int)slot.size() && slot[m].have; }
  bool has_occ(int m) const { return m >= 0 && m < (int)slot.size() && slot[m].have_occ; }
  const signed char* occ3_of(int m, int* d) const {
    if (!has_occ(m)) return nullptr;
    for (int a = 0; a < 3; a++) d[a] = slot[m].desc.dims[a];
    return (const signed char*)occ.p + slot[m].occ3_off;
  }
  const signed char* occ2_of(int m, bool critical) const { return (const signed char*)occ.p + (critical ? slot[m].occ2c_off : slot[m].occ2_off); }
  void forget(int first, int n) {
    for (int m = first; m < first + n && m < (int)slot.size(); m++) slot[m].have_occ = false;
  }
};

struct MpcState {
  DevBuf slots, sims, io, dense;
  std::vector<topay_mpc_params_t> prm;
  std::vector<char> have, sim_have;
  DevTimer timer;
  double ms = 0.0;
  topay_status alloc(hipStream_t stream) {
    if (slots.p) return TOPAY_OK;
    topay_status s;
    if ((s = slots.ensure(sizeof(topay::MpcSlot) * TOPAY_TRACK_SLOTS)) != TOPAY_OK) return s;
    if ((s = sims.ensure(sizeof(topay::SimSlot) * TOPAY_TRACK_SLOTS)) != TOPAY_OK) return s;
    HIPCHK(hipMemsetAsync(slots.p, 0, slots.bytes, stream));
    HIPCHK(hipMemsetAsync(sims.p, 0, sims.bytes, stream));
    HIPCHK(hipStreamSynchronize(stream));
    prm.resize(TOPAY_TRACK_SLOTS);
    have.assign(TOPAY_TRACK_SLOTS, 0);
    sim_have.assign(TOPAY_TRACK_SLOTS, 0);
    return TOPAY_OK;
  }
};

struct EdtState {
  DevBuf occ, thr, tmp1, tmp2, v, z, out2;
  DevTimer timer;
  double ms = 0.0;
};

struct topay_ctx {
  int device = 0;
  topay_params_t hp;
  DevParams dp;
  hipStream_t stream = nullptr;
  std::vector<DevMap> hmaps = std::vector<DevMap>(TOPAY_MAX_MAPS);
  std::vector<DevBuf> map2d = std::vector<DevBuf>(TOPAY_MAX_MAPS), map3d = std::vector<DevBuf>(TOPAY_MAX_MAPS);
  std::vector<DevBuf> map2d_inf = std::vector<DevBuf>(TOPAY_MAX_MAPS), map2d_crit = std::vector<DevBuf>(TOPAY_MAX_MAPS);
  struct MapArena { DevBuf buf; int first = 0, n = 0; };
  std::vector<MapArena> map_arenas;
  DevBuf dmaps;
  std::vector<char> have_map = std::vector<char>(TOPAY_MAX_MAPS, 0);
  std::vector<topay_ctx*> map_owner = std::vector<topay_ctx*>(TOPAY_MAX_MAPS, nullptr);
  std::vector<topay_ctx*> map_sharers;
  std::vector<int> h_map_id;
  std::vector<int> h_path_len;
  int B = 0, Nmax = 0, total_states = 0, Pmax = 0;
  std::vector<long long> h_poff, h_noff;
  DevBuf poff, noff;
  size_t workspace_bytes = 0;
  std::vector<int> hN;
  static constexpr int NBUCKET = TOPAY_NBUCKET;
  std::vector<int> cls[NBUCKET];
  hipStream_t bstream[NBUCKET] = {nullptr};
  hipEvent_t bevent[NBUCKET] = {nullptr};
  hipEvent_t bstart = nullptr;
  bool pending = false;
  int* h_started = nullptr;
  int n_launched = 0;
  int n_gate = 0;
  int latency_mode = 0;
  bool gate_done = false;
  std::vector<int> h_group;
  int n_groups = 0, cancel_budget = 0;
  DevBuf group_id, group_tau, interrupted;
  int* h_cancel = nullptr;
  void* comm = nullptr;
  int comm_world = 0, comm_rank = 0;
  hipStream_t comm_stream = nullptr;
  DevBuf comm_send, comm_recv;
  int gate_timeouts = 0;
  bool persistent = true;
  bool steal = true;
  int simd_slots = 1024;
  DevBuf qnext;
  DevBuf paths, path_off, path_len, bvel, bacc, scratch;
  DevBuf N, s1_past, map_id, head, tail, start_xy, goal_xy, init_xy, x0;
  DevBuf x, work, hist_s, hist_y, hist_ys, hist_alpha, lu;
  DevBuf success, cost, stats, xyerr, coef, T, knots, alm, fout, order, trace, elapsed, startus, hwid, sbuf, mstash, feas_cseq, feas_tk, feas_report, feas_flags, pb_io;
  DevTimer solve_timer, eval_timer;
  FrontState front;
  PlanWork plan;
  PlanStore plan_store;
  TrackState track;
  EeState ee;
  WorldState world;
  SenseState sense;
  MpcState mpc;
  EdtState edt;
  int trace_cap = 0;
  DevBatch db;
  bool have_traj = false, solved = false;
  double last_ms = 0.0;
  int last_launches = 0, last_helper_launches = 0;
};

static DevLbfgs to_dev_lbfgs(const topay_lbfgs_params_t& a) {
  DevLbfgs b;
  b.mem_size = a.mem_size; b.past = a.past; b.max_iterations = a.max_iterations; b.max_linesearch = a.max_linesearch;
  b.g_epsilon = a.g_epsilon; b.delta = a.delta; b.min_step = a.min_step; b.max_step = a.max_step;
  b.f_dec_coeff = a.f_dec_coeff; b.s_curv_coeff = a.s_curv_coeff; b.cautious_factor = a.cautious_factor;
  b.machine_prec = a.machine_prec;
  return b;
}

static bool all_finite(const double* v, size_t n, double bound = 1.0e9) {
  for (size_t i = 0; i < n; i++)
    if (!(std::fabs(v[i]) < bound)) return false;
  return true;
}

static void make_dev_params(const topay_params_t& p, DevParams& d) {
  memset(&d, 0, sizeof(d));
  d.relu_mu = p.relu_mu;
  {
    const double pe = p.relu_mu;
    d.sl_half = 0.5 * pe;
    d.sl_f3c = 1.0 / (pe * pe);
    d.sl_f4c = -0.5 * d.sl_f3c / pe;
    d.sl_d2c = 3.0 * d.sl_f3c;
    d.sl_d3c = 4.0 * d.sl_f4c;
  }
  for (int i = 0; i < 9; i++) d.energy_weights[i] = p.energy_weights[i];
  d.s1_time_weight = p.s1_time_weight; d.s1_moment_weight = p.s1_moment_weight; d.s1_acc_weight = p.s1_acc_weight;
  d.s1_domega_weight = p.s1_domega_weight; d.s1_path_pos_weight = p.s1_path_pos_weight;
  d.s2_time_weight = p.s2_time_weight; d.s2_moment_weight = p.s2_moment_weight; d.s2_acc_weight = p.s2_acc_weight;
  d.s2_domega_weight = p.s2_domega_weight; d.s2_collision_weight = p.s2_collision_weight;
  d.s2_mani_colli_weight = p.s2_mani_colli_weight; d.s2_self_colli_weight = p.s2_self_colli_weight;
  d.s2_mani_pos_weight = p.s2_mani_pos_weight; d.s2_mani_vel_weight = p.s2_mani_vel_weight;
  d.s2_mani_acc_weight = p.s2_mani_acc_weight; d.s2_mean_time_weight = p.s2_mean_time_weight;
  for (int i = 0; i < 2; i++) {
    d.alm_init_lambda[i] = p.alm_init_lambda[i]; d.alm_init_rho[i] = p.alm_init_rho[i];
    d.alm_rho_max[i] = p.alm_rho_max[i]; d.alm_gamma[i] = p.alm_gamma[i];
  }
  d.alm_tolerance = p.alm_tolerance;
  d.alm_max_outer = p.alm_max_outer;
  d.alm_work_budget = p.alm_work_budget;
  d.min_piece_num = p.min_piece_num;
  d.sample_interval = p.sample_interval;
  d.s1_normal_past = p.s1_normal_past; d.s1_shot_path_past = p.s1_shot_path_past;
  d.s1_shot_path_horizon = p.s1_shot_path_horizon;
  d.s1_lbfgs = to_dev_lbfgs(p.s1_lbfgs);
  d.s2_lbfgs = to_dev_lbfgs(p.s2_lbfgs);
  d.chassis_height = p.chassis_height; d.chassis_colli_radius = p.chassis_colli_radius;
  d.max_v = p.max_v; d.max_a = p.max_a; d.max_w = p.max_w; d.max_dw = p.max_dw;
  for (int i = 0; i < 8; i++) d.colli_length[i] = p.colli_length[i];
  int s = 0;
  for (int i = 0; i < 16 && s < TOPAY_NSPH; i++)
    if (p.colli_points[i] != 0.0) {
      d.sph_off[s] = p.colli_points[i];
      d.sph_r[s] = p.colli_point_radius[i];
      s++;
    }
  for (int i = 0; i < 7; i++) {
    d.joint_pos_limit_max[i] = p.joint_pos_limit_max[i];
    d.joint_vel_limit[i] = p.joint_vel_limit[i];
    d.joint_acc_limit[i] = p.joint_acc_limit[i];
  }
  for (int i = 0; i < 9; i++) d.relR[i] = p.relative_R[i];
// ... 289 lines not shown
```

### topay_amd/csrc/topay_host_results.h

```cpp

#pragma once

static bool class_for_waves(int N, int nw, ClassDef& out) {
  static const ClassDef w1[] = {{10, 1, 1, nullptr, k_eval1, 2}, {21, 2, 1, nullptr, k_eval2, 2}, {32, 3, 1, nullptr, k_eval3, 2},
                                {42, 4, 1, nullptr, k_eval4, 2}, {64, 6, 1, nullptr, k_eval6, 2}};
  static const ClassDef w2[] = {{42, 2, 2, nullptr, k_eval2w2, 2}, {64, 3, 2, nullptr, k_eval3w2, 2}};
  static const ClassDef w4[] = {{85, 2, 4, nullptr, k_eval2w4, 2}, {128, 3, 4, nullptr, k_eval3w4, 2}, {TOPAY_MAX_N, 4, 4, nullptr, k_eval4w4, 2}};
  const ClassDef* t = nw == 1 ? w1 : (nw == 2 ? w2 : (nw == 4 ? w4 : nullptr));
  const int cnt = nw == 1 ? 5 : (nw == 4 ? 3 : 2);
  if (!t) return false;
  for (int k = 0; k < cnt; k++)
    if (N <= t[k].max_n) { out = t[k]; return true; }
  return false;
}

static topay_status eval_one(topay_ctx* c, int stage, int i, const double* x, const double* alm_lambda, const double* alm_rho,
                             double* f, double* g, double* final_xy_error, bool commit, int force_nw = 0) {
  if (!c || !c->have_traj) return TOPAY_ERR_NO_TRAJ;
  if (i < 0 || i >= c->B || (stage != 1 && stage != 2) || !x) return TOPAY_ERR_INVALID_ARG;
  HIPCHK(hipSetDevice(c->device));
  if (topay_status ws = wait_pending(c)) return ws;
  const int N = c->hN[i], nn = 10 * N - 8;
  if (N == 0) return TOPAY_ERR_TOO_MANY_PIECES;
  HIPCHK(h2d_sync(c, c->db.x_of(c->h_noff[i]), x, (size_t)nn));
  double alm[kAlmLen] = {alm_lambda ? alm_lambda[0] : c->hp.alm_init_lambda[0], alm_lambda ? alm_lambda[1] : c->hp.alm_init_lambda[1],
                   alm_rho ? alm_rho[0] : c->hp.alm_init_rho[0], alm_rho ? alm_rho[1] : c->hp.alm_init_rho[1]};
  HIPCHK(h2d_sync(c, c->db.alm_of(i), alm, kAlmLen));
  DevBuf tmp;
  topay_status s = tmp.ensure(4);
  if (s != TOPAY_OK) return s;
  HIPCHK(h2d_sync(c, tmp.as<int>(), &i, 1));
  DevBatch d = c->db;
  d.order = tmp.as<int>();
  ClassDef cd = kClassTable[bucket_of(N)];
  if (force_nw > 0 && !class_for_waves(N, force_nw, cd)) { set_err("no kernel with that many waves holds this candidate"); return TOPAY_ERR_UNSUPPORTED; }
  const size_t lds = class_lds_bytes(cd, N);
  if ((s = push_params(c)) != TOPAY_OK) return s;
  HIPCHK(set_kernel_attributes(c->device));
  if (force_nw > 0) HIPCHK(hipFuncSetAttribute((const void*)cd.eval, hipFuncAttributeMaxDynamicSharedMemorySize, kLdsDoublesPerCU * 8));
  hipLaunchKernelGGL(cd.eval, dim3(1), dim3(64 * cd.nw), lds, c->stream, d, (const DevMap*)c->dmaps.p, stage | (commit ? 16 : 0), 1, N);
  HIPCHK(hipGetLastError());
  HIPCHK(hipStreamSynchronize(c->stream));
  if (f) HIPCHK(d2h_sync(c, f, c->fout.as<double>() + i, 1));
  if (g) HIPCHK(d2h_sync(c, g, c->db.work_of(c->h_noff[i]), (size_t)nn));
  if (final_xy_error) HIPCHK(d2h_sync(c, final_xy_error, c->db.xyerr_of(i), 2));
  return TOPAY_OK;
}

extern "C" {

topay_status topay_get_nmax(topay_ctx* c, int* nmax, int* Nmax) {
  if (!c || !c->have_traj) return TOPAY_ERR_NO_TRAJ;
  if (nmax) *nmax = 10 * c->Nmax - 8;
  if (Nmax) *Nmax = c->Nmax;
  return TOPAY_OK;
}

topay_status topay_get_batch(topay_ctx* c, int* success, double* cost, int* n_pieces) {
  if (!c || !c->have_traj) return TOPAY_ERR_NO_TRAJ;
  HIPCHK(hipSetDevice(c->device));
  if (success) HIPCHK(d2h_sync(c, success, c->success.as<int>(), (size_t)c->B));
  if (cost) HIPCHK(d2h_sync(c, cost, c->cost.as<double>(), (size_t)c->B));
  if (n_pieces) memcpy(n_pieces, c->hN.data(), (size_t)c->B * 4);
  return TOPAY_OK;
}

topay_status topay_get_elapsed_us(topay_ctx* c, double* us, double* start_us, int* hw_id) {
  if (!c || !c->have_traj) return TOPAY_ERR_NO_TRAJ;
  HIPCHK(hipSetDevice(c->device));
  if (us) HIPCHK(d2h_sync(c, us, c->elapsed.as<double>(), (size_t)c->B));
  if (start_us) HIPCHK(d2h_sync(c, start_us, c->startus.as<double>(), (size_t)c->B));
  if (hw_id) HIPCHK(d2h_sync(c, hw_id, c->hwid.as<int>(), (size_t)c->B));
  return TOPAY_OK;
}

topay_status topay_playback(topay_ctx* c, int i, int n_times, const double* times, double* states, int seq_cap, double* seq,
                            int* n_seq) {
  if (!c || !c->have_traj || !c->solved) return TOPAY_ERR_NO_TRAJ;
  if (i < 0 || i >= c->B || n_times < 0 || (n_times > 0 && (!times || !states))) return TOPAY_ERR_INVALID_ARG;
  HIPCHK(hipSetDevice(c->device));
  std::vector<double> hT((size_t)std::max(1, c->hN[i]));
  if (c->hN[i] > 0) HIPCHK(d2h_sync(c, hT.data(), c->db.T_of(c->h_poff[i]), (size_t)c->hN[i]));
  double t = 0.0;
  for (int k = 0; k < c->hN[i]; k++) t += hT[k];
  if (!(t > 0.0 && t < 1.0e4)) t = 0.0;
  const long long cap_panels = (long long)(t / 0.025) + 4;
  const long long nseq_max = cap_panels / 4 + 2;
  topay_status s;
  if ((s = c->feas_cseq.ensure((size_t)2 * (cap_panels + 1) * 8)) != TOPAY_OK) return s;
  double *d_times, *d_states, *d_seq; int* d_nseq;
  auto lay = [&](Carver& k) {
    d_times = k.take<double>((size_t)n_times); d_states = k.take<double>((size_t)n_times * 10); d_seq = k.take<double>((size_t)nseq_max * 4);
    d_nseq = k.take<int>(1);
  };
  if ((s = c->pb_io.carve(lay)) != TOPAY_OK) return s;
  if (n_times) HIPCHK(h2d(c, d_times, times, (size_t)n_times));
  topay_status ps = push_params(c);
  if (ps != TOPAY_OK) return ps;
  hipLaunchKernelGGL(k_playback, dim3(1), dim3(64), 0, c->stream, c->db, i, c->feas_cseq.as<double>(), cap_panels, n_times,
                     (const double*)d_times, d_states, d_seq, d_nseq);
  HIPCHK(hipGetLastError());
  HIPCHK(hipStreamSynchronize(c->stream));
  int ns = 0;
  HIPCHK(d2h_sync(c, &ns, d_nseq, 1));
  if (n_seq) *n_seq = ns;
  if (seq && ns > 0) HIPCHK(d2h_sync(c, seq, d_seq, (size_t)std::min(ns, seq_cap) * 4));
  if (n_times) HIPCHK(d2h_sync(c, states, d_states, (size_t)n_times * 10));
  return TOPAY_OK;
}

topay_status topay_default_mesh_params(topay_mesh_params_t* p) {
  if (!p) return TOPAY_ERR_INVALID_ARG;
  const double ll[7] = {0.2405, 0.0, 0.256, 0.0, 0.21, 0.0, 0.144};
  const double lo[7] = {-3.1, -2.26, -3.1, -2.355, -3.1, -2.23, -6.28};
  for (int i = 0; i < 7; i++) {
    p->link_length[i] = ll[i];
    p->joint_pos_limit_min[i] = lo[i];
    for (int k = 0; k < 3; k++) { p->joint_offset[3 * i + k] = 0.0; p->joint_dof_axis[3 * i + k] = 0.0; }
    if (i < 6) {
      p->joint_offset[3 * i] = (i % 2 == 0) ? -1.5708 : 1.5708;
      p->joint_dof_axis[3 * i + 1] = (i % 2 == 0) ? -1.0 : 1.0;
    } else {
      p->joint_dof_axis[3 * i + 2] = 1.0;
    }
  }
  return TOPAY_OK;
}

topay_status topay_mesh_poses(topay_ctx* c, const topay_mesh_params_t* mesh, int n, const double* states, double* parts) {
  if (!c || !mesh || n < 0 || (n > 0 && (!states || !parts))) return TOPAY_ERR_INVALID_ARG;
  if (n == 0) return TOPAY_OK;
  HIPCHK(hipSetDevice(c->device));
  topay_status s;
  double *d_st, *d_parts;
  if ((s = c->pb_io.carve([&](Carver& k) { d_st = k.take<double>((size_t)n * 10); d_parts = k.take<double>((size_t)n * 77); })) != TOPAY_OK) return s;
  HIPCHK(h2d(c, d_st, states, (size_t)n * 10));
  topay_status ps = push_params(c);
  if (ps != TOPAY_OK) return ps;
  hipLaunchKernelGGL(k_mesh_pose, dim3((n + 63) / 64), dim3(64), 0, c->stream, *mesh, n, (const double*)d_st, d_parts);
  HIPCHK(hipGetLastError());
  HIPCHK(d2h(c, parts, d_parts, (size_t)n * 77));
  HIPCHK(hipStreamSynchronize(c->stream));
  return TOPAY_OK;
}

topay_status topay_mesh_traj(topay_ctx* c, int i, const topay_mesh_params_t* mesh, int res, int cap_states, double* parts,
                             double* yaws, double* arc_lengths, int* n_states) {
  if (!c || !c->have_traj || !c->solved) return TOPAY_ERR_NO_TRAJ;
  if (i < 0 || i >= c->B || !mesh || res <= 0 || cap_states < res + 1 || !parts || !yaws || !arc_lengths || !n_states) return TOPAY_ERR_INVALID_ARG;
  HIPCHK(hipSetDevice(c->device));
  std::vector<double> hT((size_t)std::max(1, c->hN[i]));
  if (c->hN[i] > 0) HIPCHK(d2h_sync(c, hT.data(), c->db.T_of(c->h_poff[i]), (size_t)c->hN[i]));
  double T = 0.0;
  for (int k = 0; k < c->hN[i]; k++) T += hT[k];
  if (!(T > 0.0 && T < 1.0e4)) { *n_states = 0; return TOPAY_OK; }
  const double intvl = T / res;
  std::vector<double> times;
  for (double t = 0.0; t < T && (int)times.size() < cap_states; t += intvl) times.push_back(t);
  const int n = (int)times.size();
  std::vector<double> st((size_t)(n + 1) * 10);
  times.push_back(0.0);
  topay_status s = topay_playback(c, i, n + 1, times.data(), st.data(), 0, nullptr, nullptr);
  if (s != TOPAY_OK) return s;
  if ((s = topay_mesh_poses(c, mesh, n, st.data(), parts)) != TOPAY_OK) return s;
  double acc = 0.0;
  const double* prev = &st[(size_t)n * 10];
  for (int k = 0; k < n; k++) {
    const double* cur = &st[(size_t)k * 10];
    const double dx = cur[0] - prev[0], dy = cur[1] - prev[1];
    acc += std::sqrt(dx * dx + dy * dy);
    arc_lengths[k] = acc;
    yaws[k] = cur[2];
    prev = cur;
  }
  *n_states = n;
  return TOPAY_OK;
}

topay_status topay_get_total_durations(topay_ctx* c, double* total) {
  if (!c || !c->have_traj || !total) return TOPAY_ERR_NO_TRAJ;
  HIPCHK(hipSetDevice(c->device));
  std::vector<double> hT((size_t)c->h_poff[c->B] + 1);
  HIPCHK(d2h_sync(c, hT.data(), c->T.as<double>(), (size_t)c->h_poff[c->B]));
  for (int b = 0; b < c->B; b++) {
    double t = 0.0;
    for (int i = 0; i < c->hN[b]; i++) t += hT[(size_t)c->h_poff[b] + i];
    total[b] = c->hN[b] > 0 ? t : 0.0 / 0.0;
  }
  return TOPAY_OK;
}

topay_status topay_get_alm(topay_ctx* c, double* alm) {
  if (!c || !c->have_traj || !alm) return TOPAY_ERR_NO_TRAJ;
  HIPCHK(hipSetDevice(c->device));
  HIPCHK(d2h_sync(c, alm, c->alm.as<double>(), (size_t)c->B * kAlmLen));
  return TOPAY_OK;
}

topay_status topay_get_stats(topay_ctx* c, int* stats) {
  if (!c || !c->have_traj || !stats) return TOPAY_ERR_NO_TRAJ;
  HIPCHK(hipSetDevice(c->device));
  HIPCHK(d2h_sync(c, stats, c->stats.as<int>(), (size_t)c->B * kStatsLen));
  return TOPAY_OK;
}

topay_status topay_get_result(topay_ctx* c, int i, int* success, double* cost, int* n_pieces, double* durations,
                              double* coeffs, double* knots_xy) {
  if (!c || !c->have_traj) return TOPAY_ERR_NO_TRAJ;
  if (i < 0 || i >= c->B) return TOPAY_ERR_INVALID_ARG;
  HIPCHK(hipSetDevice(c->device));
  if (topay_status ws = wait_pending(c)) return ws;
  const int N = c->hN[i], rows = 6 * N;
  if (N == 0) {
    if (success) *success = 0;
    if (cost) *cost = 0.0 / 0.0;
    if (n_pieces) *n_pieces = 0;
    return TOPAY_OK;
  }
  if (success) HIPCHK(d2h_sync(c, success, c->success.as<int>() + i, 1));
  if (cost) HIPCHK(d2h_sync(c, cost, c->cost.as<double>() + i, 1));
  if (n_pieces) *n_pieces = N;
  if (durations) HIPCHK(d2h_sync(c, durations, c->db.T_of(c->h_poff[i]), (size_t)N));
  if (coeffs) {
    std::vector<double> cm((size_t)9 * rows);
    HIPCHK(d2h_sync(c, cm.data(), c->db.coef_of(c->h_poff[i]), cm.size()));
    for (int p = 0; p < N; p++)
      for (int d = 0; d < 9; d++)
        for (int k = 0; k < 6; k++) coeffs[((size_t)p * 9 + d) * 6 + k] = cm[(size_t)d * rows + 6 * p + 5 - k];
  }
  if (knots_xy)
    HIPCHK(d2h_sync(c, knots_xy, c->db.knots_of(c->h_poff[i], i), (size_t)2 * (N + 1)));
  return TOPAY_OK;
}

topay_status topay_get_results(topay_ctx* c, int n, const int* idx, int cap_pieces, int* piece_off, double* durations,
                               double* coeffs, double* knots_xy) {
  if (!c || !c->have_traj) return TOPAY_ERR_NO_TRAJ;
  if (n < 0 || (n > 0 && (!idx || !piece_off))) return TOPAY_ERR_INVALID_ARG;
  if (n == 0) return TOPAY_OK;
  HIPCHK(hipSetDevice(c->device));
  if (topay_status ws = wait_pending(c)) return ws;
  if (!c->solved) { set_err("topay_get_results: the batch has not been optimised"); return TOPAY_ERR_NO_TRAJ; }
  std::vector<int> off((size_t)n + 1, 0);
  for (int k = 0; k < n; k++) {
    if (idx[k] < 0 || idx[k] >= c->B) return TOPAY_ERR_INVALID_ARG;
    off[k + 1] = off[k] + c->hN[idx[k]];
  }
  const int np = off[n];
  memcpy(piece_off, off.data(), ((size_t)n + 1) * sizeof(int));
  if (np > cap_pieces) { set_err("topay_get_results: cap_pieces too small for the selection"); return TOPAY_ERR_INVALID_ARG; }
  if (np == 0 || (!durations && !coeffs && !knots_xy)) return TOPAY_OK;
  const size_t kn = (size_t)2 * (np + n), dbl = (size_t)np + (size_t)np * kCoefPerPiece + kn;
  int *d_idx, *d_off; double *d_dur, *d_coef, *d_kn;
  auto lay = [&](Carver& k) {
    d_idx = k.take<int>((size_t)n); d_off = k.take<int>((size_t)n + 1);
    d_dur = k.take<double>((size_t)np); d_coef = k.take<double>((size_t)np * kCoefPerPiece); d_kn = k.take<double>(kn);
  };
  if (topay_status s = c->pb_io.carve(lay); s != TOPAY_OK) return s;
  HIPCHK(h2d(c, d_idx, idx, (size_t)n));
  HIPCHK(h2d(c, d_off, off.data(), (size_t)n + 1));
  HIPCHK(hipMemsetAsync(d_kn, 0, kn * sizeof(double), c->stream));
  hipLaunchKernelGGL(k_gather_results, dim3(n), dim3(64), 0, c->stream, c->db, n, (const int*)d_idx, (const int*)d_off, d_dur,
                     d_coef, d_kn);
  HIPCHK(hipGetLastError());
  std::vector<double> host(dbl);
  HIPCHK(d2h_sync(c, host.data(), d_dur, dbl));
  if (durations) memcpy(durations, host.data(), (size_t)np * 8);
  if (coeffs) memcpy(coeffs, host.data() + np, (size_t)np * kCoefPerPiece * 8);
  if (knots_xy) memcpy(knots_xy, host.data() + np + (size_t)np * kCoefPerPiece, kn * 8);
  return TOPAY_OK;
}

topay_status topay_get_polytraj_msg(topay_ctx* c, int i, int cap_pieces, unsigned char* order, float* coeff, float* durations,
                                    signed char* directions, int* n_pieces) {
  if (!c || !c->have_traj) return TOPAY_ERR_NO_TRAJ;
  if (i < 0 || i >= c->B) return TOPAY_ERR_INVALID_ARG;
  const int N = c->hN[i];
  if (n_pieces) *n_pieces = N;
  if (order) *order = 5;
  if (N == 0) return TOPAY_OK;
  if (N > cap_pieces) return TOPAY_ERR_INVALID_ARG;
  constexpr int CP = kCoefPerPiece;
  std::vector<double> dur((size_t)N), cf((size_t)N * CP);
  topay_status s = topay_get_result(c, i, nullptr, nullptr, nullptr, dur.data(), cf.data(), nullptr);
  if (s != TOPAY_OK) return s;
  for (int p = 0; p < N; p++) {
    if (durations) durations[p] = (float)dur[p];
    if (coeff)
      for (int t = 0; t < CP; t++) coeff[(size_t)p * CP + t] = (float)cf[(size_t)p * CP + t];
    if (directions) {
      const double* a = &cf[(size_t)p * CP + 6], t = 0.5 * dur[p];
      const double sd = ((((5.0 * a[0]) * t + 4.0 * a[1]) * t + 3.0 * a[2]) * t + 2.0 * a[3]) * t + a[4];
      directions[p] = sd < 0.0 ? -1 : 1;
    }
  }
  return TOPAY_OK;
}

topay_status topay_get_x(topay_ctx* c, int i, int* n, double* x) {
  if (!c || !c->have_traj) return TOPAY_ERR_NO_TRAJ;
  if (i < 0 || i >= c->B) return TOPAY_ERR_INVALID_ARG;
  HIPCHK(hipSetDevice(c->device));
  if (c->hN[i] == 0) { if (n) *n = 0; return TOPAY_ERR_TOO_MANY_PIECES; }
  const int nn = 10 * c->hN[i] - 8;
  if (n) *n = nn;
  if (x) {
    if (c->solved) HIPCHK(d2h_sync(c, x, c->db.x_of(c->h_noff[i]), (size_t)nn));
// ... 191 lines not shown
```

### topay_amd/csrc/topay_kernels.h

```cpp
#pragma once
#include <hip/hip_runtime.h>

#include "topay_solve.h"
#include "topay_feas.h"
#include "topay_edt.h"
#include "topay_front.h"
#include "topay_mcrrt.h"
#include "topay_jps.h"

using namespace topay;

#ifndef TOPAY_CPU_EMU
extern __shared__ double topay_lds[];
#define TOPAY_LDS_PTR ((lds_dp)topay_lds)
#else
#define TOPAY_LDS_PTR ((lds_dp)hip_emu::S().dyn_smem)
#endif

__global__ void k_init(DevBatch Bt, const double* paths, const long long* path_off, const int* path_len,
                       const double* bvel, const double* bacc, double* scratch, int scratch_stride, int maxN, int stride_n) {
  const int b = blockIdx.x * blockDim.x + threadIdx.x;
  if (b >= Bt.B) return;
  init_one(g_P, paths + path_off[b] * 10, path_len[b], bvel + (size_t)b * 20, bacc + (size_t)b * 20,
           scratch + (size_t)b * scratch_stride, maxN, Bt.N + b, Bt.s1_past + b, Bt.head_of(b), Bt.tail_of(b),
           Bt.start_xy + 2 * b, Bt.goal_xy + 2 * b, Bt.init_xy + (size_t)b * 2 * maxN, Bt.x0 + (size_t)b * stride_n);
}

__device__ __forceinline__ long long uniform_i64(long long v) {
  const unsigned lo = (unsigned)__builtin_amdgcn_readfirstlane((int)(v & 0xffffffffLL)), hi = (unsigned)__builtin_amdgcn_readfirstlane((int)(v >> 32));
  return (long long)(((unsigned long long)hi << 32) | lo);
}

template <int NW>
__host__ __device__ __forceinline__ int eval_lds_doubles(int Nmax_lds) {
  return eval_lds_total(Nmax_lds, NW);
}

template <int NW>
__device__ __forceinline__ void load_ctx(EvalCtx& C, const DevBatch& Bt, int b, int Nmax_lds) {
  C.tid = threadIdx.x;
  C.lane = threadIdx.x & 63;
  C.wave = threadIdx.x >> 6;
  C.N = __builtin_amdgcn_readfirstlane(Bt.N[b]);
  C.rows = 6 * C.N;
  C.n = 10 * C.N - 8;
  C.red = nullptr; C.adj = nullptr; C.cl_in_lds = 1;
  eval_lds_carve(C, TOPAY_LDS_PTR, Nmax_lds, NW);
  fill_power_table(C.pw, C.lane);
  C.hd = (glb_cdp)(Bt.head + (size_t)b * kHeadLen);
  C.tl = (glb_cdp)(Bt.tail + (size_t)b * kHeadLen);
  const long long po = uniform_i64(Bt.poff[b]);
  C.lu = (glb_dp)Bt.lu_of(po);
  C.sb_stride = TOPAY_EP * C.N;
  C.sbuf = (glb_dp)Bt.sbuf_of(po);
  C.mstash = (glb_dp)Bt.mstash_of(po);
  C.coefg = (glb_dp)Bt.coef_of(po);
  C.init_xy = (glb_cdp)Bt.init_xy_of(b);
  C.sx = Bt.start_xy[2 * b]; C.sy = Bt.start_xy[2 * b + 1];
  C.ex = Bt.goal_xy[2 * b];  C.ey = Bt.goal_xy[2 * b + 1];
  C.fxe0 = 0.0; C.fxe1 = 0.0;
  C.stamps = nullptr;
  C.t_last = 0;
#ifdef TOPAY_STAMPS
  if (Bt.trace && Bt.trace_cap >= 32) C.stamps = (TOPAY_GLB long long*)(Bt.trace + (size_t)b * Bt.trace_cap) + 8;
  C.t_last = (long long)__builtin_amdgcn_s_memtime();
#endif
}

template <int NW>
__device__ __forceinline__ void store_result(const EvalCtx& C, const DevBatch& Bt, int b) {
  constexpr int NT = 64 * NW;
  const int N = C.N, rows = C.rows;
  const long long po = uniform_i64(Bt.poff[b]);
  if (C.cl_in_lds) {
    double* coef = Bt.coef_of(po);
    for (int t = C.tid; t < 9 * rows; t += NT) coef[t] = C.cL[t];
  }
  for (int t = C.tid; t < N; t += NT) Bt.T[po + t] = C.Tp[t];
  double* kn = Bt.knots_of(po, b);
  if (C.tid == 0) { kn[0] = C.sx; kn[1] = C.sy; }
  for (int t = C.tid; t < 2 * N; t += NT) kn[2 + t] = C.pcs[2 * N + 2 + t];
}

template <int RMAX, int NW, int OCC>
__device__ __forceinline__ void eval_body(const DevBatch& Bt, const DevMap* maps, int stage, int Nmax_lds, int repeats) {
  const int b = Bt.order[blockIdx.x];
  const bool commit = (stage & 16) != 0;
  stage &= 15;
  EvalCtx C;
  load_ctx<NW>(C, Bt, b, Nmax_lds);
  const TOPAY_GLB DevMap* mp = (const TOPAY_GLB DevMap*)(maps + __builtin_amdgcn_readfirstlane(Bt.map_id[b]));
  const long long no = uniform_i64(Bt.noff[b]);
  C.x = (glb_cdp)Bt.x_of(no);
  C.g = (glb_dp)Bt.work_of(no);
  const double* alm = Bt.alm_of(b);
  C.lam0 = alm[0]; C.lam1 = alm[1]; C.rho0 = alm[2]; C.rho1 = alm[3];
  __syncthreads();
  double f = 0.0;
  const bool cost_only = repeats < 0;
  if (cost_only) repeats = -repeats;
  for (int r = 0; r < repeats; r++) {
    GradGate gate;
    gate.always = !cost_only; gate.has_early = false; gate.finit = 0.0; gate.thr = -1.0e300; gate.early = 0.0;
    gate.early_ok = false; gate.skip_thr = 0.0;
    __syncthreads();
    if (stage == 1) f = eval_cost_grad<1, RMAX, NW, OCC>(C, mp, gate);
    else f = eval_cost_grad<2, RMAX, NW, OCC>(C, mp, gate);
  }
  if (C.tid == 0) {
    Bt.fout[b] = f;
    Bt.xyerr_of(b)[0] = C.fxe0;
    Bt.xyerr_of(b)[1] = C.fxe1;
  }
  if (commit) {
    __syncthreads();
    store_result<NW>(C, Bt, b);
    if (C.tid == 0) { Bt.cost[b] = f; Bt.success[b] = 1; }
  }
}

__device__ __forceinline__ FeasIO feas_io_of(const DevBatch& Bt, int b, long long po) {
  FeasIO F;
  F.coef = Bt.coef_of(po);
  F.T = Bt.T_of(po);
  F.N = Bt.N[b];
  F.x0 = Bt.start_xy[2 * b]; F.y0 = Bt.start_xy[2 * b + 1];
  F.th0 = Bt.head_of(b)[0];
  F.cseq = nullptr; F.tk = nullptr;
  F.cap_panels = 0; F.cap_samples = 0;
  F.report = nullptr; F.feasible = nullptr; F.truncated = nullptr;
  return F;
}

template <int OCC>
__device__ __noinline__ void feasibility_gate_in_solve(const FeasIO F, const TOPAY_GLB DevMap* mp) { feasibility_gate(F, mp); }

template <int RMAX, int OCC, int NWE = 1, int RMAX_E = RMAX>
__device__ __forceinline__ void solve_one(const DevBatch& Bt, const DevMap* maps, int Nmax_lds, int b) {
  constexpr int NT = 64 * NWE;
  const unsigned long long t_begin = wall_clock64();
  if (threadIdx.x == 0 && Bt.started && Bt.N[b] <= Bt.gate_maxN) {
#ifndef TOPAY_CPU_EMU
    __hip_atomic_fetch_add(Bt.started, 1, __ATOMIC_RELAXED, __HIP_MEMORY_SCOPE_SYSTEM);
#else
    Bt.started[0] += 1;
#endif
  }
  EvalCtx C;
  load_ctx<NWE>(C, Bt, b, Nmax_lds);
  const TOPAY_GLB DevMap* mp = (const TOPAY_GLB DevMap*)(maps + __builtin_amdgcn_readfirstlane(Bt.map_id[b]));
  lds_dp pf = TOPAY_LDS_PTR + eval_lds_doubles<NWE>(Nmax_lds);
  const long long no = uniform_i64(Bt.noff[b]);
  const int n = C.n;
  SolveIO S;
  S.x = (glb_dp)Bt.x_of(no);
  S.g = (glb_dp)Bt.work_of(no);
  S.xp = (glb_dp)(Bt.work_of(no) + n);
  S.gp = (glb_dp)(Bt.work_of(no) + 2 * (long long)n);
  S.d = (glb_dp)(Bt.work_of(no) + 3 * (long long)n);
  S.hist_s = (glb_dp)Bt.hist_s_of(no);
  S.hist_y = (glb_dp)Bt.hist_y_of(no);
  S.hist_ys = (glb_dp)Bt.hist_ys_of(b);
  S.hist_al = (glb_dp)Bt.hist_alpha_of(b);
  S.nstride = n;
  S.stats = (glb_ip)Bt.stats_of(b);
  S.trace = Bt.trace ? (glb_dp)(Bt.trace + (size_t)b * Bt.trace_cap) : (glb_dp)nullptr;
  S.trace_cap = Bt.trace_cap;
  const int grp = Bt.group_id ? __builtin_amdgcn_readfirstlane(Bt.group_id[b]) : -1;
  S.grp_tau = (grp >= 0 && Bt.cancel_budget > 0) ? (TOPAY_GLB int*)(Bt.group_tau + grp) : (TOPAY_GLB int*)nullptr;
  S.cancel_flag = (const TOPAY_GLB int*)Bt.cancel_flag;
  S.cancel_budget = Bt.cancel_budget;
  {
    const double* x0 = Bt.x0_of(b);
    for (int e = C.tid; e < C.n; e += NT) S.x[e] = x0[e];
  }
  int success = 0, interrupted = 0;
  double cost = 0.0;
  if constexpr (NWE != 1) {
    C.x = S.x;
    C.g = S.g;
    __syncthreads();
    if (C.wave == 0) solve_trajectory<RMAX, OCC, NWE, RMAX_E>(C, mp, S, Bt.s1_past[b], pf, success, cost, interrupted);
    else eval_helper_loop<RMAX_E, NWE, OCC>(C, mp, pf + kSolvePastDoubles + kSolveParkDoubles);
  } else {
    solve_trajectory<RMAX, OCC>(C, mp, S, Bt.s1_past[b], pf, success, cost, interrupted);
  }
  __syncthreads();
  store_result<NWE>(C, Bt, b);
  if (Bt.gate_in_solve) {
    __syncthreads();
    int* fl = Bt.flags_of(b);
    if (interrupted) {
      if (C.tid == 0) { fl[0] = 0; fl[1] = 0; }
    } else if (threadIdx.x < 64) {
      const long long po = uniform_i64(Bt.poff[b]);
      const long long hist_doubles = (long long)Bt.hist_m * C.n;
      FeasIO F;
      F.coef = Bt.coef_of(po);
      F.T = Bt.T_of(po);
      F.N = C.N;
      F.x0 = C.sx; F.y0 = C.sy;
      F.th0 = Bt.head_of(b)[0];
      F.cseq = Bt.hist_s_of(no);
      F.tk = Bt.hist_y_of(no);
      F.cap_panels = hist_doubles / 2 - 1;
      F.cap_samples = hist_doubles;
      F.report = Bt.report_of(b);
      F.feasible = fl;
      F.truncated = Bt.gate_truncated;
      feasibility_gate_in_solve<OCC>(F, mp);
      if (S.grp_tau && success) {
        wave_global_sync();
        if (C.tid == 0 && fl[0]) {
          const int clock = (S.stats[2] + S.stats[5]) * C.N;
          atomicMin((int*)S.grp_tau, clock);
        }
      }
    }
    __syncthreads();
  }
  if (C.tid == 0) {
    if (Bt.interrupted) Bt.interrupted[b] = interrupted;
    Bt.success[b] = success;
    Bt.cost[b] = cost;
    Bt.xyerr_of(b)[0] = C.fxe0;
    Bt.xyerr_of(b)[1] = C.fxe1;
    Bt.alm_of(b)[0] = C.lam0; Bt.alm_of(b)[1] = C.lam1; Bt.alm_of(b)[2] = C.rho0; Bt.alm_of(b)[3] = C.rho1;
    Bt.elapsed_us[b] = (double)(wall_clock64() - t_begin) * 0.01;
    Bt.start_us[b] = (double)t_begin * 0.01;
#ifndef TOPAY_CPU_EMU
    {
      const unsigned hw = __builtin_amdgcn_s_getreg((4 ) | (0 << 6) | (31 << 11));
      const unsigned xcc = __builtin_amdgcn_s_getreg((20 ) | (0 << 6) | (3 << 11));
      Bt.hw_id[b] = (int)(((xcc & 0xF) << 16) | (((hw >> 13) & 0x7) << 12) | (((hw >> 8) & 0xF) << 4) | ((hw >> 4) & 0x3));
    }
#else
    Bt.hw_id[b] = 0;
#endif
  }
}

template <int RMAX, int OCC, int NWE = 1, int RMAX_E = RMAX>
__device__ __forceinline__ void drain_queues(const DevBatch& B, const DevMap* maps, int Nmax_lds, int my_class) {
  const bool queued = B.queue_next != nullptr;
  const int lowest = queued ? B.queue_lowest : my_class;
  for (int cls = my_class; cls >= lowest; cls--) {
    const int count = queued ? B.queue_count[cls] : 1, off = queued ? B.queue_off[cls] : (int)blockIdx.x;
    for (int once = 0;; once++) {
      int pos = 0;
      if (threadIdx.x == 0) {
        pos = queued ? atomicAdd(B.queue_next + cls, 1) : once;
        int stop = 0;
#ifndef TOPAY_CPU_EMU
        if (B.cancel_flag) stop = __hip_atomic_load(B.cancel_flag, __ATOMIC_RELAXED, __HIP_MEMORY_SCOPE_SYSTEM) != 0;
#else
        if (B.cancel_flag) stop = *B.cancel_flag != 0;
#endif
        pos = (pos < 0x40000000 ? pos : 0x3fffffff) | (stop << 30);
      }
      if (NWE == 1) {
        pos = __shfl(pos, 0);
      } else {
        TOPAY_LDS int* w0 = (TOPAY_LDS int*)TOPAY_LDS_PTR;
        if (threadIdx.x == 0) w0[0] = pos;
        __syncthreads();
        pos = w0[0];
        __syncthreads();
      }
      const bool cancelled = (pos & 0x40000000) != 0;
      pos &= 0x3fffffff;
      if (cancelled && pos < count) {
        if (threadIdx.x == 0) {
          const int b = B.order[off + pos];
          int* st = B.stats_of(b);
          for (int q = 0; q < kStatsLen; q++) st[q] = 0;
          st[3] = TOPAY_INTERRUPTED;
          if (B.interrupted) B.interrupted[b] = 1;
          B.success[b] = 0;
          if (B.gate_in_solve) { B.flags_of(b)[0] = 0; B.flags_of(b)[1] = 0; }
        }
        continue;
      }
      if (pos >= count) break;
      solve_one<RMAX, OCC, NWE, RMAX_E>(B, maps, Nmax_lds, B.order[off + pos]);
      __syncthreads();
    }
  }
}

template <int RMAX, int OCC, int NWE = 1, int RMAX_E = RMAX>
__device__ __forceinline__ void solve_body(const DevBatch& Bt, const DevMap* maps, int Nmax_lds) {
  drain_queues<RMAX, OCC, NWE, RMAX_E>(Bt, maps, Nmax_lds, Bt.queue_class);
}

#define TOPAY_SOLVE_KERNEL(NAME, R, OCC)                                                             \
  __global__ void __launch_bounds__(64, OCC) NAME(DevBatch Bt, const DevMap* maps, int Nmax_lds) {   \
    solve_body<R, OCC>(Bt, maps, Nmax_lds);                                                          \
  }
#define TOPAY_LATENCY_KERNEL(NAME, RS, RE, WE, OCC)                                                        \
  __global__ void __launch_bounds__(64 * WE, OCC) NAME(DevBatch Bt, const DevMap* maps, int Nmax_lds) {    \
    solve_body<RS, OCC, WE, RE>(Bt, maps, Nmax_lds);                                                       \
  }
#define TOPAY_EVAL_KERNEL(NAME, R, W, OCC)                                                                          \
  __global__ void __launch_bounds__(64 * W, OCC) NAME(DevBatch Bt, const DevMap* maps, int stage, int repeats, int Nmax_lds) { \
    eval_body<R, W, OCC>(Bt, maps, stage, Nmax_lds, repeats);                                              \
  }
#ifndef TOPAY_NO_KERNEL_TABLE
TOPAY_SOLVE_KERNEL(k_solve1, 1, 2)
TOPAY_SOLVE_KERNEL(k_solve2, 2, 2)
TOPAY_SOLVE_KERNEL(k_solve3, 3, 2)
TOPAY_LATENCY_KERNEL(k_long5, 5, 2, 4, 2)
TOPAY_LATENCY_KERNEL(k_long14, 14, 4, 4, 2)
TOPAY_LATENCY_KERNEL(k_lat1, 1, 1, 4, 2)
TOPAY_LATENCY_KERNEL(k_lat2, 2, 1, 4, 2)
TOPAY_LATENCY_KERNEL(k_lat3, 3, 1, 4, 2)
TOPAY_EVAL_KERNEL(k_eval1, 1, 1, 2)
TOPAY_EVAL_KERNEL(k_eval2, 2, 1, 2)
TOPAY_EVAL_KERNEL(k_eval3, 3, 1, 2)
TOPAY_EVAL_KERNEL(k_eval2w2, 2, 2, 2)
TOPAY_EVAL_KERNEL(k_eval3w2, 3, 2, 2)
TOPAY_EVAL_KERNEL(k_eval3w4, 3, 4, 2)
TOPAY_EVAL_KERNEL(k_eval4w4, 4, 4, 2)
TOPAY_EVAL_KERNEL(k_eval4, 4, 1, 2)
TOPAY_EVAL_KERNEL(k_eval6, 6, 1, 2)
TOPAY_EVAL_KERNEL(k_eval2w4, 2, 4, 2)
#endif

__global__ void __launch_bounds__(64, 2) k_feasible(DevBatch Bt, const DevMap* maps, double* cseq, double* tk, long long cap_panels,
                                                 long long cap_samples, double* report, int* flags) {
  const int b = blockIdx.x;
  const int N = Bt.N[b];
  if (N <= 0) {
    if (threadIdx.x == 0) { flags[2 * b] = 0; flags[2 * b + 1] = 0; }
    return;
  }
  FeasIO F = feas_io_of(Bt, b, Bt.poff[b]);
  F.cseq = cseq + (size_t)b * 2 * (cap_panels + 1);
  F.tk = tk + (size_t)b * cap_samples;
  F.cap_panels = cap_panels; F.cap_samples = cap_samples;
  F.report = report + (size_t)b * kReportLen;
  F.feasible = flags + 2 * b;
  const TOPAY_GLB DevMap* mp = (const TOPAY_GLB DevMap*)(maps + __builtin_amdgcn_readfirstlane(Bt.map_id[b]));
  feasibility_gate(F, mp);
}

__global__ void __launch_bounds__(64) k_mesh_pose(topay_mesh_params_t K, int n, const double* states, double* parts) {
  const int i = blockIdx.x * blockDim.x + threadIdx.x;
  if (i >= n) return;
  double st[10];
  for (int k = 0; k < 10; k++) st[k] = states[(size_t)i * 10 + k];
  mesh_pose(K, st, parts + (size_t)i * 77);
}

__global__ void __launch_bounds__(64) k_playback(DevBatch Bt, int b, double* cseq, long long cap_panels, int nq, const double* times,
                                                 double* states, double* seq_out, int* nseq_out) {
  const int N = Bt.N[b];
  if (N <= 0) {
    if (threadIdx.x == 0) *nseq_out = 0;
    return;
  }
  FeasIO F = feas_io_of(Bt, b, Bt.poff[b]);
  F.cseq = cseq;
  F.cap_panels = cap_panels;
  playback(F, nq, times, states, seq_out, nseq_out);
}

__global__ void k_gather_results(DevBatch Bt, int n, const int* idx, const int* piece_off, double* durations, double* coeffs,
                                 double* knots) {
  const int k = blockIdx.x;
  if (k >= n) return;
  const int b = idx[k];
  const int N = piece_off[k + 1] - piece_off[k];
  if (N <= 0) return;
  const int rows = 6 * N, p0 = piece_off[k];
  const long long po = Bt.poff[b];
  const double* cm = Bt.coef_of(po);
  constexpr int CP = kCoefPerPiece;
  for (int t = threadIdx.x; t < N * CP; t += blockDim.x) {
    const int p = t / CP, r = t - CP * p, d = r / 6, kk = r - 6 * d;
    coeffs[(size_t)p0 * CP + t] = cm[(size_t)d * rows + 6 * p + 5 - kk];
  }
  for (int t = threadIdx.x; t < N; t += blockDim.x) durations[p0 + t] = Bt.T_of(po)[t];
  for (int t = threadIdx.x; t < 2 * (N + 1); t += blockDim.x) knots[2 * (size_t)(p0 + k) + t] = Bt.knots_of(po, b)[t];
}

__global__ void k_whole_body(const DevMap* maps, int map_id, int n, const double* states, int* out) {
  const int i = blockIdx.x * blockDim.x + threadIdx.x;
  if (i >= n) return;
  const DevMap M = maps[map_id];
  out[i] = whole_body_collision(M, states + (size_t)i * 10) ? 1 : 0;
}

__global__ void k_math(const double* a, const double* b, double* out, int n) {
  const int i = blockIdx.x * blockDim.x + threadIdx.x;
  if (i >= n) return;
  double s, c;
  det_sincos(a[i], &s, &c);
  out[4 * i] = s;
  out[4 * i + 1] = c;
  out[4 * i + 2] = det_atan2(a[i], b[i]);
  out[4 * i + 3] = sqrt(fabs(a[i])) / (1.0 + fabs(b[i]));
}
```

### topay_amd/csrc/topay_minco.h

```cpp
#pragma once

#include <hip/hip_runtime.h>

#include "topay_eval_ctx.h"
#include "topay_wave.h"

namespace topay {

#define BAND(i, j) band[((i) - (j) + 6) * rows + (j)]

#define TOPAY_SWEEP_CHUNK 24
#define TOPAY_SWEEP_WCOLS 30
#define TOPAY_SWEEP_WIN (7 * TOPAY_SWEEP_WCOLS)
static_assert(2 * TOPAY_SWEEP_WIN <= eval_borrow_doubles(1, 1) && 2 * TOPAY_SWEEP_WIN <= eval_borrow_doubles(1, 2) &&
              2 * TOPAY_SWEEP_WIN <= eval_borrow_doubles(1, 4), "the sweeps' windows fit behind the coefficients");
template <int MODE>
__device__ __forceinline__ void band_sweep(lds_dp v, bool owner, glb_cdp lu, lds_dp win, int rows, int lane) {
  constexpr bool FWD = (MODE == 0 || MODE == 2);
  constexpr bool SCALE = (MODE == 1 || MODE == 2);
  constexpr int D0 = (MODE == 0 || MODE == 3) ? 7 : 0;
  constexpr int CH = TOPAY_SWEEP_CHUNK, WC = TOPAY_SWEEP_WCOLS, WIN = TOPAY_SWEEP_WIN;
  constexpr int NEL = (SCALE ? 7 : 6) * WC;
  constexpr int NQ = (NEL + 63) / 64;
  double w[6];
  double x = 0.0;
#pragma unroll
  for (int t = 0; t < 6; t++) w[t] = 0.0;
  if (owner) {
    if (FWD) {
      x = v[0];
#pragma unroll
      for (int t = 0; t < 6; t++) w[t] = v[1 + t];
    } else {
      x = v[rows - 1];
#pragma unroll
      for (int t = 0; t < 6; t++) w[t] = v[rows - 2 - t];
    }
  }
  const int nchunk = (rows + CH - 1) / CH;
  auto chunk_clo = [&](int k) { return FWD ? CH * k : rows - 1 - CH * k - (WC - 1); };
  auto request = [&](int k, double (&q)[NQ]) {
    const int clo = chunk_clo(k);
#pragma unroll
    for (int u = 0; u < NQ; u++) {
      const int e = lane + 64 * u;
      const int r = e / WC, cc = e - r * WC;
      int c = clo + cc;
      c = c < 0 ? 0 : (c > rows - 1 ? rows - 1 : c);
      const int d = (r < 6 ? D0 + r : 13);
      q[u] = lu[(d < 14 ? d : 13) * rows + c];
    }
  };
  auto deposit = [&](int k, const double (&q)[NQ]) {
    lds_dp wb = win + (k & 1) * WIN;
#pragma unroll
    for (int u = 0; u < NQ; u++) {
      const int e = lane + 64 * u;
      if (e < NEL) wb[e] = q[u];
    }
  };
  double q[NQ];
  request(0, q);
  deposit(0, q);
  lds_sync();
  for (int k = 0; k < nchunk; k++) {
    const bool more = k + 1 < nchunk;
    if (more) request(k + 1, q);
    if (owner) {
      lds_cdp wb = win + (k & 1) * WIN;
      const int clo = chunk_clo(k);
#pragma unroll 1
      for (int b0 = CH * k; b0 < CH * (k + 1) && b0 < rows; b0 += 6) {
        double cf[6][6], sc[6], nw[6];
#pragma unroll
        for (int u = 0; u < 6; u++) {
          const int j = FWD ? b0 + u : rows - 1 - (b0 + u);
#pragma unroll
          for (int t = 1; t <= 6; t++) {
            int idx;
            if (MODE == 0) idx = (t - 1) * WC + (j - clo);
            else if (MODE == 1) idx = (6 - t) * WC + (j - clo);
            else if (MODE == 2) idx = (6 - t) * WC + (j + t - clo);
            else idx = (t - 1) * WC + (j - t - clo);
            cf[u][t - 1] = wb[idx];
          }
          if (SCALE) sc[u] = wb[6 * WC + (j - clo)];
          int in = FWD ? j + 7 : j - 7;
          in = in < 0 ? 0 : (in > rows - 1 ? rows - 1 : in);
          nw[u] = v[in];
        }
        double xo[6];
#pragma unroll
        for (int u = 0; u < 6; u++) {
          const double xs = SCALE ? x * sc[u] : x;
          xo[u] = xs;
#pragma unroll
          for (int t = 0; t < 6; t++) w[(u + t) % 6] -= cf[u][t] * xs;
          x = w[u % 6];
          w[u % 6] = nw[u];
        }
#pragma unroll
        for (int u = 0; u < 6; u++) {
          const int j = FWD ? b0 + u : rows - 1 - (b0 + u);
          v[j] = xo[u];
        }
      }
    }
    if (more) deposit(k + 1, q);
    lds_sync();
  }
}

template <int NW, int OCC>
__device__ __noinline__ void minco_generate(EvalCtx& C) {
  constexpr int NT = 64 * NW;
  const lds_dp c_Tp = C.Tp;
  const lds_dp c_X = C.X;
  const lds_dp c_gdT = C.gdT;
  const glb_cdp c_hd = C.hd, c_tl = C.tl;
  const glb_dp c_lu = C.lu;
  const glb_cdp c_x = C.x;
  dev_params_ref P = dev_params();
  const int tid = C.tid, lane = C.lane, wave = __builtin_amdgcn_readfirstlane(C.wave);
  const int N = __builtin_amdgcn_readfirstlane(C.N), rows = __builtin_amdgcn_readfirstlane(C.rows);
  lds_dp cL = C.cL;
  lds_dp band = cL;
  lds_dp rdiag = cL + 13 * rows;
  glb_cdp Tau = c_x;
  glb_cdp Theta = c_x + N;
  glb_cdp Arc = c_x + 2 * N - 1;
  glb_cdp Vq = c_x + 3 * N - 1;

  const double tau_v = tid < N ? Tau[tid] : 0.0;
  constexpr int NI = 9;
  double inner_v[NI];
#pragma unroll
  for (int u = 0; u < NI; u++) {
    const int t = tid + NT * u;
    inner_v[u] = 0.0;
    if (t < 9 * (N - 1)) {
      const int i = t / 9, d = t - 9 * i;
      const int dq = d >= 2 ? d - 2 : 0;
      inner_v[u] = d == 0 ? Theta[i] : (d == 1 ? Arc[i] : Vq[i * 7 + dq]);
    }
  }
  double bc_v[6] = {0.0, 0.0, 0.0, 0.0, 0.0, 0.0};
  if (tid < 9) {
    const int d = tid;
    bc_v[0] = c_hd[0 * 9 + d]; bc_v[1] = c_hd[1 * 9 + d]; bc_v[2] = c_hd[2 * 9 + d];
    bc_v[3] = (d == 1) ? Arc[N - 1] : c_tl[0 * 9 + d];
    bc_v[4] = c_tl[1 * 9 + d]; bc_v[5] = c_tl[2 * 9 + d];
  }
  for (int t = tid; t < 13 * rows; t += NT) band[t] = 0.0;
  if (tid < N) {
    double T1 = expC2(tau_v);
    double T2 = T1 * T1, T3 = T2 * T1, T4 = T2 * T2, T5 = T4 * T1;
    c_Tp[0 * N + tid] = T1; c_Tp[1 * N + tid] = T2; c_Tp[2 * N + tid] = T3;
    c_Tp[3 * N + tid] = T4; c_Tp[4 * N + tid] = T5;
    c_gdT[tid] = 0.0;
  }
  wg_barrier<NW>();
  if (tid == 0) {
    BAND(0, 0) = 1.0; BAND(1, 1) = 1.0; BAND(2, 2) = 2.0;
  }
  if (tid < N - 1) {
    const int i = tid;
    const double T1 = c_Tp[i], T2 = c_Tp[N + i], T3 = c_Tp[2 * N + i], T4 = c_Tp[3 * N + i], T5 = c_Tp[4 * N + i];
    const int r = 6 * i;
    BAND(r + 3, r + 3) = 6.0;  BAND(r + 3, r + 4) = 24.0 * T1; BAND(r + 3, r + 5) = 60.0 * T2; BAND(r + 3, r + 9) = -6.0;
    BAND(r + 4, r + 4) = 24.0; BAND(r + 4, r + 5) = 120.0 * T1; BAND(r + 4, r + 10) = -24.0;
    BAND(r + 5, r) = 1.0; BAND(r + 5, r + 1) = T1; BAND(r + 5, r + 2) = T2; BAND(r + 5, r + 3) = T3;
    BAND(r + 5, r + 4) = T4; BAND(r + 5, r + 5) = T5;
    BAND(r + 6, r) = 1.0; BAND(r + 6, r + 1) = T1; BAND(r + 6, r + 2) = T2; BAND(r + 6, r + 3) = T3;
    BAND(r + 6, r + 4) = T4; BAND(r + 6, r + 5) = T5; BAND(r + 6, r + 6) = -1.0;
    BAND(r + 7, r + 1) = 1.0; BAND(r + 7, r + 2) = 2 * T1; BAND(r + 7, r + 3) = 3 * T2; BAND(r + 7, r + 4) = 4 * T3;
    BAND(r + 7, r + 5) = 5 * T4; BAND(r + 7, r + 7) = -1.0;
    BAND(r + 8, r + 2) = 2.0; BAND(r + 8, r + 3) = 6 * T1; BAND(r + 8, r + 4) = 12 * T2; BAND(r + 8, r + 5) = 20 * T3;
    BAND(r + 8, r + 8) = -2.0;
  }
  if (tid == NT - 1) {
    const int i = N - 1, R0 = 6 * N;
    const double T1 = c_Tp[i], T2 = c_Tp[N + i], T3 = c_Tp[2 * N + i], T4 = c_Tp[3 * N + i], T5 = c_Tp[4 * N + i];
    BAND(R0 - 3, R0 - 6) = 1.0; BAND(R0 - 3, R0 - 5) = T1; BAND(R0 - 3, R0 - 4) = T2; BAND(R0 - 3, R0 - 3) = T3;
    BAND(R0 - 3, R0 - 2) = T4; BAND(R0 - 3, R0 - 1) = T5;
    BAND(R0 - 2, R0 - 5) = 1.0; BAND(R0 - 2, R0 - 4) = 2 * T1; BAND(R0 - 2, R0 - 3) = 3 * T2; BAND(R0 - 2, R0 - 2) = 4 * T3;
    BAND(R0 - 2, R0 - 1) = 5 * T4;
    BAND(R0 - 1, R0 - 4) = 2; BAND(R0 - 1, R0 - 3) = 6 * T1; BAND(R0 - 1, R0 - 2) = 12 * T2; BAND(R0 - 1, R0 - 1) = 20 * T3;
  }
  wg_barrier<NW>();
  STAMP(C, 0);
  if (wave == 0) {
    const int t = lane / 7 + 1, u = lane - (lane / 7) * 7;
    const bool lane_in = lane < 42;
    const int o_kk = 6 * rows;
    const int o_ik = lane_in ? (t + 6) * rows : o_kk;
    const int o_ij = lane_in ? (t - u + 6) * rows + u : o_kk;
    const int o_kj = lane_in ? (6 - u) * rows + u : o_kk;
    for (int k = 0; k <= rows - 2; k++) {
      const int i = k + t, j = k + u;
      const bool act = lane_in && (i < rows) && (j < rows);
      double akk = band[o_kk + k], aik = band[o_ik + k], aij = band[o_ij + k], akj = band[o_kj + k];
      TOPAY_OPAQUE(aij); TOPAY_OPAQUE(akj);
      const double m = aik / akk;
      const double nv = (u == 0) ? m : (aij - m * akj);
      lds_sync();
      if (act) band[o_ij + k] = nv;
      lds_sync();
    }
  }
  wg_barrier<NW>();
  STAMP(C, 1);
  for (int t = tid; t < rows; t += NT) rdiag[t] = 1.0 / BAND(t, t);
  wg_barrier<NW>();
  for (int t = tid; t < 14 * rows; t += NT) c_lu[t] = band[t];
  if (NW == 1) lds_sync();
  else { wave_global_sync(); wg_barrier<NW>(); }
  for (int t = tid; t < 9 * rows; t += NT) cL[t] = 0.0;
  wg_barrier<NW>();
  if (tid < 9) {
    const int d = tid;
    cL[d * rows + 0] = bc_v[0];
    cL[d * rows + 1] = bc_v[1];
    cL[d * rows + 2] = bc_v[2];
    cL[d * rows + rows - 3] = bc_v[3];
    cL[d * rows + rows - 2] = bc_v[4];
    cL[d * rows + rows - 1] = bc_v[5];
  }
#pragma unroll
  for (int u = 0; u < NI; u++) {
    const int t = tid + NT * u;
    if (t < 9 * (N - 1)) {
      const int i = t / 9, d = t - 9 * i;
      const int dq = d >= 2 ? d - 2 : 0;
      cL[d * rows + 6 * i + 5] = d >= 2 ? sigmoidC2(inner_v[u], P.joint_pos_limit_max[dq]) : inner_v[u];
    }
  }
  wg_barrier<NW>();
  if (wave == 0) {
    const bool owner = lane < 9;
    const lds_dp mine = cL + (owner ? lane : 8) * rows;
    band_sweep<0>(mine, owner, (glb_cdp)c_lu, c_X, rows, lane);
    band_sweep<1>(mine, owner, (glb_cdp)c_lu, c_X, rows, lane);
  }
  C.cl_in_lds = 1;
  wg_barrier<NW>();
  STAMP(C, 2);
}

}
```

### topay_amd/csrc/topay_solve.h

```cpp
#pragma once
#include "topay_eval.h"

#define TOPAY_PF_ELEMS 24
#define TOPAY_PF_MAX 12

namespace topay {

struct SolveIO {
  glb_dp x;
  glb_dp g;
  glb_dp xp;
  glb_dp gp;
  glb_dp d;
  glb_dp hist_s;
  glb_dp hist_y;
  glb_dp hist_ys;
  glb_dp hist_al;
  int nstride;
  glb_ip stats;
  glb_dp trace;
  int trace_cap;
  TOPAY_GLB int* grp_tau;
  const TOPAY_GLB int* cancel_flag;
  int cancel_budget;
};

typedef double dpair __attribute__((vector_size(16)));
typedef const TOPAY_GLB dpair* glb_cpp;
typedef TOPAY_GLB dpair* glb_pp;
__device__ __forceinline__ bool vec_in(int tid, int t, int n) { return 2 * (64 * (t >> 1) + tid) < n; }
#define TOPAY_HIST_AUX 0
template <bool STREAM = false>
__device__ __forceinline__ dpair row_pair_or_zero(glb_cdp row, int n, int i) {
#ifndef TOPAY_CPU_EMU
  typedef unsigned int u32x4 __attribute__((vector_size(16)));
  const __amdgpu_buffer_rsrc_t rs = __builtin_amdgcn_make_buffer_rsrc((void*)row, (short)0, n * 8, 0x00020000);
  const u32x4 v = __builtin_amdgcn_raw_buffer_load_b128(rs, i * 16, 0, STREAM ? TOPAY_HIST_AUX : 0);
  return __builtin_bit_cast(dpair, v);
#else
  dpair q;
  q[0] = 2 * i < n ? row[2 * i] : 0.0;
  q[1] = 2 * i < n ? row[2 * i + 1] : 0.0;
  return q;
#endif
}
template <int EPL>
__device__ __forceinline__ void vec_load(glb_cdp a, int n, int tid, double (&v)[EPL]) {
  static_assert(EPL % 2 == 0, "pairs");
#pragma unroll
  for (int p = 0; p < EPL / 2; p++) {
    const dpair q = row_pair_or_zero(a, n, 64 * p + tid);
    v[2 * p] = q[0];
    v[2 * p + 1] = q[1];
  }
}
template <int EPL>
__device__ __forceinline__ void vec_store(glb_dp a, int n, int tid, const double (&v)[EPL]) {
  const glb_pp ap = (glb_pp)a;
#pragma unroll
  for (int p = 0; p < EPL / 2; p++) {
    const int i = 64 * p + tid;
    dpair q;
    q[0] = v[2 * p];
    q[1] = v[2 * p + 1];
    if (2 * i < n) ap[i] = q;
  }
}
template <int EPL>
__device__ __forceinline__ double vec_dot_part(glb_cdp a, glb_cdp b, int n, int tid) {
  double av[EPL], bv[EPL];
  vec_load<EPL>(a, n, tid, av);
  vec_load<EPL>(b, n, tid, bv);
  double s = 0.0;
#pragma unroll
  for (int t = 0; t < EPL; t++) s += vec_in(tid, t, n) ? av[t] * bv[t] : 0.0;
  return s;
}

#define TOPAY_CMD_DOUBLES 16
constexpr int kSolvePastDoubles = 8;
constexpr int kSolveParkDoubles = 40;
__host__ __device__ constexpr int solve_tail_doubles(bool helpers) {
  return kSolvePastDoubles + kSolveParkDoubles + (helpers ? TOPAY_CMD_DOUBLES : 0);
}
static_assert(kLbfgsMaxMem <= eval_borrow_doubles(1, 1) && kLbfgsMaxMem <= eval_borrow_doubles(1, 4), "the alpha ring fits behind the coefficients");
template <int RMAX_E, int NWE, int OCC>
__device__ __forceinline__ void eval_helper_loop(EvalCtx& C, const TOPAY_GLB DevMap* mp, lds_dp cmd) {
  for (;;) {
    __syncthreads();
    const TOPAY_LDS int* ic = (const TOPAY_LDS int*)(cmd + 8);
    if (__builtin_amdgcn_readfirstlane(ic[0]) == 0) break;
    GradGate gate;
    gate.finit = cmd[0]; gate.thr = cmd[1]; gate.early = cmd[2]; gate.skip_thr = cmd[3];
    C.lam0 = cmd[4]; C.lam1 = cmd[5]; C.rho0 = cmd[6]; C.rho1 = cmd[7];
    const int stage = __builtin_amdgcn_readfirstlane(ic[1]);
    gate.always = ic[2] != 0; gate.has_early = ic[3] != 0; gate.early_ok = ic[4] != 0;
    if (stage == 1) (void)eval_cost_grad<1, RMAX_E, NWE, OCC>(C, mp, gate);
    else (void)eval_cost_grad<2, RMAX_E, NWE, OCC>(C, mp, gate);
    wg_lds_barrier();
  }
}

#ifdef TOPAY_STAMPS
#define LSTAMP(k)                                                                              \
  do {                                                                                         \
    const long long now_ = (long long)__builtin_amdgcn_s_memtime();                            \
    if (C.stamps && C.lane == 0) C.stamps[k] += now_ - lt_;                                    \
    lt_ = (long long)__builtin_amdgcn_s_memtime();                                             \
  } while (0)
#else
#define LSTAMP(k) do { } while (0)
#endif
template <int RMAX, int OCC = 2, int NWE = 1, int RMAX_E = RMAX>
__device__ __forceinline__ void solve_trajectory(EvalCtx& C, const TOPAY_GLB DevMap* mp, SolveIO& S, int s1_past,
                                                 lds_dp pf , int& success_out,
                                                 double& cost_out, int& interrupted_out) {
  constexpr bool HELPERS = NWE != 1;
  dev_params_ref P = dev_params();
  auto ssync = [&]() {
    if constexpr (HELPERS) { wave_global_sync(); lds_sync(); }
    else __syncthreads();
  };
  const int tid = C.tid, n = __builtin_amdgcn_readfirstlane(C.n);
  constexpr int EPL = 2 * RMAX;
  int stage = 1;
  int alm_iter = 0;
  bool success = false, interrupted = false;
  int st_s1_ret = 0, st_s1_it = 0, st_s1_ev = 0, st_s2_ret = 0, st_s2_it = 0, st_s2_ev = 0, st_sumb = 0;
  C.lam0 = P.alm_init_lambda[0]; C.lam1 = P.alm_init_lambda[1];
  C.rho0 = P.alm_init_rho[0];    C.rho1 = P.alm_init_rho[1];
  C.x = S.x;
  C.g = S.g;

  int k = 0, end = 0, bound = 0, count = 0, ret = 0, evals = 0;
  double fx = 0.0, step = 0.0, stp = 0.0, finit = 0.0, dginit = 0.0, dgtest = 0.0, dstest = 0.0, mu = 0.0, nu = 0.0;
  bool brackt = false, touched = false;
  enum { MODE_INIT = 0, MODE_LS = 1 };
  int mode = MODE_INIT;
  double cost = 0.0;
  int ntrace = 0;

#ifdef TOPAY_STAMPS
  long long lt_ = (long long)__builtin_amdgcn_s_memtime();
#endif
  for (;;) {
    const DevLbfgs& lp = stage == 1 ? P.s1_lbfgs : P.s2_lbfgs;
    const int past = stage == 1 ? s1_past : lp.past;
    const int mem = lp.mem_size;
    if (stage == 2 && (S.grp_tau || S.cancel_flag)) {
      int stop = 0;
      if (tid == 0) {
        const int clock = (st_s1_ev + st_s2_ev + evals) * C.N;
        const int poll_mask = C.N <= 16 ? 7 : (C.N <= 32 ? 3 : 0);
#ifndef TOPAY_CPU_EMU
        if (S.grp_tau) stop = (long long)clock > (long long)__hip_atomic_load(S.grp_tau, __ATOMIC_RELAXED, __HIP_MEMORY_SCOPE_AGENT) + S.cancel_budget;
        if (S.cancel_flag && (evals & poll_mask) == 0) stop |= __hip_atomic_load(S.cancel_flag, __ATOMIC_RELAXED, __HIP_MEMORY_SCOPE_SYSTEM) != 0;
#else
        if (S.grp_tau) stop = (long long)clock > (long long)*S.grp_tau + S.cancel_budget;
        if (S.cancel_flag && (evals & poll_mask) == 0) stop |= *S.cancel_flag != 0;
#endif
      }
      stop = __shfl(stop, 0);
      if (stop) {
        st_s2_ret = TOPAY_INTERRUPTED; st_s2_it += k; st_s2_ev += evals;
        interrupted = true;
        success = false;
        break;
      }
    }
    ssync();
    STAMP(C, 9);
    double f;
    GradGate gate;
    gate.always = (mode == MODE_INIT);
    gate.has_early = past > 0;
    gate.finit = finit;
    gate.thr = finit + stp * dgtest;
    gate.early = past > 0 ? lp.delta / past : 0.0;
    {
      const double stp_next = 0.5 * (mu + stp);
      gate.early_ok = mode == MODE_LS && (count + 1 < lp.max_linesearch) && !((stp - mu) < lp.machine_prec * stp) &&
                      !(stp_next < lp.min_step) && !(stp_next > lp.max_step);
      const double no_early = past > 0 ? finit + 2.0 * gate.early * (fabs(finit) + 1.0) : gate.thr;
      gate.skip_thr = gate.thr > no_early ? gate.thr : no_early;
    }
    {
      lds_dp pk = pf + kSolvePastDoubles;
      pk[0] = fx; pk[1] = step; pk[2] = stp; pk[3] = finit; pk[4] = dginit; pk[5] = dgtest; pk[6] = dstest; pk[7] = mu;
      pk[8] = nu; pk[9] = cost;
      TOPAY_LDS int* ik = (TOPAY_LDS int*)(pk + 10);
      ik[0] = stage; ik[1] = alm_iter; ik[2] = st_s1_ret; ik[3] = st_s1_it; ik[4] = st_s1_ev; ik[5] = st_s2_ret; ik[6] = st_s2_it;
      ik[7] = st_s2_ev; ik[8] = st_sumb; ik[9] = k; ik[10] = end; ik[11] = bound; ik[12] = count; ik[13] = ret; ik[14] = evals;
      ik[15] = mode; ik[16] = ntrace; ik[17] = (brackt ? 1 : 0) | (touched ? 2 : 0);
      ik[18] = S.nstride; ik[19] = S.trace_cap; ik[20] = s1_past; ik[21] = S.cancel_budget;
      TOPAY_LDS unsigned long long* qk = (TOPAY_LDS unsigned long long*)(pk + 21);
      qk[0] = (unsigned long long)S.x; qk[1] = (unsigned long long)S.g; qk[2] = (unsigned long long)S.xp;
      qk[3] = (unsigned long long)S.gp; qk[4] = (unsigned long long)S.d; qk[5] = (unsigned long long)S.hist_s;
      qk[6] = (unsigned long long)S.hist_y; qk[7] = (unsigned long long)S.hist_ys; qk[8] = (unsigned long long)S.hist_al;
      qk[9] = (unsigned long long)S.stats; qk[10] = (unsigned long long)S.trace; qk[11] = (unsigned long long)mp;
      qk[12] = (unsigned long long)S.grp_tau; qk[13] = (unsigned long long)S.cancel_flag;
    }
    if constexpr (HELPERS) {
      lds_dp cmd = pf + kSolvePastDoubles + kSolveParkDoubles;
      cmd[0] = gate.finit; cmd[1] = gate.thr; cmd[2] = gate.early; cmd[3] = gate.skip_thr;
      cmd[4] = C.lam0; cmd[5] = C.lam1; cmd[6] = C.rho0; cmd[7] = C.rho1;
      TOPAY_LDS int* ic = (TOPAY_LDS int*)(cmd + 8);
      ic[0] = 1; ic[1] = stage; ic[2] = gate.always ? 1 : 0; ic[3] = gate.has_early ? 1 : 0; ic[4] = gate.early_ok ? 1 : 0;
      __syncthreads();
    }
    LSTAMP(15);
    if (stage == 1) f = eval_cost_grad<1, RMAX_E, NWE, OCC>(C, mp, gate);
    else f = eval_cost_grad<2, RMAX_E, NWE, OCC>(C, mp, gate);
#ifdef TOPAY_STAMPS
    lt_ = (long long)__builtin_amdgcn_s_memtime();
#endif
    if (NWE > 1) wg_lds_barrier();
    {
      lds_cdp pk = pf + kSolvePastDoubles;
      fx = uniform_f64(pk[0]); step = uniform_f64(pk[1]); stp = uniform_f64(pk[2]); finit = uniform_f64(pk[3]);
      dginit = uniform_f64(pk[4]); dgtest = uniform_f64(pk[5]); dstest = uniform_f64(pk[6]); mu = uniform_f64(pk[7]);
      nu = uniform_f64(pk[8]); cost = uniform_f64(pk[9]);
      const TOPAY_LDS int* ik = (const TOPAY_LDS int*)(pk + 10);
      auto ui = [&](int q) { return __builtin_amdgcn_readfirstlane(ik[q]); };
      stage = ui(0); alm_iter = ui(1); st_s1_ret = ui(2); st_s1_it = ui(3); st_s1_ev = ui(4); st_s2_ret = ui(5); st_s2_it = ui(6);
      st_s2_ev = ui(7); st_sumb = ui(8); k = ui(9); end = ui(10); bound = ui(11); count = ui(12); ret = ui(13); evals = ui(14);
      mode = ui(15); ntrace = ui(16);
      const int fl = ui(17);
      brackt = (fl & 1) != 0; touched = (fl & 2) != 0;
      S.nstride = ui(18); S.trace_cap = ui(19); s1_past = ui(20); S.cancel_budget = ui(21);
      const TOPAY_LDS unsigned long long* qk = (const TOPAY_LDS unsigned long long*)(pk + 21);
      auto up = [&](int q) {
        const unsigned long long v = qk[q];
        const unsigned lo = (unsigned)__builtin_amdgcn_readfirstlane((int)(v & 0xffffffffu));
        const unsigned hi = (unsigned)__builtin_amdgcn_readfirstlane((int)(v >> 32));
        return ((unsigned long long)hi << 32) | lo;
      };
      S.x = (glb_dp)up(0); S.g = (glb_dp)up(1); S.xp = (glb_dp)up(2); S.gp = (glb_dp)up(3); S.d = (glb_dp)up(4);
      S.hist_s = (glb_dp)up(5); S.hist_y = (glb_dp)up(6); S.hist_ys = (glb_dp)up(7); S.hist_al = (glb_dp)up(8);
      S.stats = (glb_ip)up(9); S.trace = (glb_dp)up(10); mp = (const TOPAY_GLB DevMap*)up(11);
      S.grp_tau = (TOPAY_GLB int*)up(12); S.cancel_flag = (const TOPAY_GLB int*)up(13);
      f = uniform_f64(f);
    }
    evals++;
    LSTAMP(11);
#ifndef TOPAY_STAMPS
    if (S.trace && tid == 0 && ntrace < S.trace_cap) S.trace[ntrace] = f;
#endif
    ntrace++;

    enum { GO_EVAL = 0, GO_LS_BEGIN = 1, GO_RUN_END = 2 };
    int go = GO_EVAL;
    if (mode == MODE_INIT) {
      fx = f;
      if (tid == 0) pf[0] = fx;
      double gmax = 0.0, xmax = 0.0;
      {
        double gv[EPL], xv[EPL], dv[EPL];
        vec_load<EPL>(S.g, n, tid, gv);
        vec_load<EPL>(S.x, n, tid, xv);
#pragma unroll
        for (int t = 0; t < EPL; t++) {
          const bool in = vec_in(tid, t, n);
          dv[t] = -gv[t];
          gmax = in ? fmax(gmax, fabs(gv[t])) : gmax;
          xmax = in ? fmax(xmax, fabs(xv[t])) : xmax;
        }
        vec_store<EPL>(S.d, n, tid, dv);
      }
      gmax = wave_max(gmax);
      xmax = wave_max(xmax);
      k = 0;
      if (gmax / fmax(1.0, xmax) < lp.g_epsilon) {
        ret = TOPAY_LBFGS_CONVERGENCE;
        go = GO_RUN_END;
      } else {
        step = 1.0 / sqrt(wave_sum(vec_dot_part<EPL>(S.d, S.d, n, tid)));
        k = 1;
        end = 0;
        bound = 0;
        go = GO_LS_BEGIN;
      }
    } else {
      ++count;
      int ls = 0;
      if (isinf(f) || isnan(f)) {
        ls = TOPAY_LBFGSERR_INVALID_FUNCVAL;
      } else if (past > 0 && fabs(finit - f) / (fabs(finit) + 1.0) < lp.delta / past) {
        ls = count;
      } else {
        bool accepted = false;
        if (f > finit + stp * dgtest) {
          nu = stp;
          brackt = true;
        } else {
          const double gs = wave_sum(vec_dot_part<EPL>(S.g, S.d, n, tid));
          if (gs < dstest) mu = stp;
          else accepted = true;
        }
        if (accepted) ls = count;
        else if (lp.max_linesearch <= count) ls = TOPAY_LBFGSERR_MAXIMUMLINESEARCH;
        else if (brackt && (nu - mu) < lp.machine_prec * nu) ls = TOPAY_LBFGSERR_WIDTHTOOSMALL;
        else {
          if (brackt) stp = 0.5 * (mu + nu);
          else stp *= 2.0;
          if (stp < lp.min_step) ls = TOPAY_LBFGSERR_MINIMUMSTEP;
          else if (stp > lp.max_step) {
            if (touched) ls = TOPAY_LBFGSERR_MAXIMUMSTEP;
            else { touched = true; stp = lp.max_step; }
          }
        }
      }
      if (ls == 0) {
        {
          double pv[EPL], dv[EPL], xv[EPL];
          vec_load<EPL>(S.xp, n, tid, pv);
          vec_load<EPL>(S.d, n, tid, dv);
#pragma unroll
          for (int t = 0; t < EPL; t++) xv[t] = pv[t] + stp * dv[t];
          vec_store<EPL>(S.x, n, tid, xv);
        }
        go = GO_EVAL;
      } else if (ls < 0) {
        fx = f;
        {
          double pv[EPL], qv[EPL];
          vec_load<EPL>(S.xp, n, tid, pv);
          vec_load<EPL>(S.gp, n, tid, qv);
          vec_store<EPL>(S.x, n, tid, pv);
          vec_store<EPL>(S.g, n, tid, qv);
        }
        ret = ls;
        go = GO_RUN_END;
      } else {
        fx = f;
        step = stp;
        bool fin = false;
        if (stage == 2 && k > lp.max_iterations) { ret = TOPAY_LBFGS_CANCELED; fin = true; }
        if (!fin) {
          double gmax = 0.0, xmax = 0.0;
          {
            double gv[EPL], xv[EPL];
            vec_load<EPL>(S.g, n, tid, gv);
            vec_load<EPL>(S.x, n, tid, xv);
#pragma unroll
            for (int t = 0; t < EPL; t++) {
              const bool in = vec_in(tid, t, n);
              gmax = in ? fmax(gmax, fabs(gv[t])) : gmax;
              xmax = in ? fmax(xmax, fabs(xv[t])) : xmax;
            }
          }
          gmax = wave_max(gmax);
          xmax = wave_max(xmax);
          if (gmax / fmax(1.0, xmax) < lp.g_epsilon) { ret = TOPAY_LBFGS_CONVERGENCE; fin = true; }
        }
        if (!fin && past > 0) {
          if (past <= k) {
            const double rate = fabs(pf[k % past] - fx) / fmax(1.0, fabs(fx));
            if (rate < lp.delta) { ret = TOPAY_LBFGS_STOP; fin = true; }
          }
          if (!fin) {
            ssync();
            if (tid == 0) pf[k % past] = fx;
            ssync();
          }
        }
        if (!fin && lp.max_iterations != 0 && lp.max_iterations <= k) { ret = TOPAY_LBFGSERR_MAXIMUMITERATION; fin = true; }
        if (fin) {
          go = GO_RUN_END;
        } else {
          ++k;
          glb_dp sE = S.hist_s + (size_t)end * S.nstride;
          glb_dp yE = S.hist_y + (size_t)end * S.nstride;
          double ys = 0.0, yy = 0.0, ss = 0.0, gg = 0.0;
          {
            double xv[EPL], pv[EPL], gv[EPL], qv[EPL], sv[EPL], yv[EPL], dv[EPL];
            vec_load<EPL>(S.x, n, tid, xv);
            vec_load<EPL>(S.xp, n, tid, pv);
            vec_load<EPL>(S.g, n, tid, gv);
            vec_load<EPL>(S.gp, n, tid, qv);
#pragma unroll
            for (int t = 0; t < EPL; t++) {
              const bool in = vec_in(tid, t, n);
              const double se = xv[t] - pv[t], ye = gv[t] - qv[t], gpe = qv[t];
              sv[t] = se;
              yv[t] = ye;
              ys += in ? ye * se : 0.0; yy += in ? ye * ye : 0.0; ss += in ? se * se : 0.0; gg += in ? gpe * gpe : 0.0;
              dv[t] = -gv[t];
            }
            vec_store<EPL>(sE, n, tid, sv);
            vec_store<EPL>(yE, n, tid, yv);
            vec_store<EPL>(S.d, n, tid, dv);
          }
          ys = wave_sum(ys); yy = wave_sum(yy); ss = wave_sum(ss); gg = wave_sum(gg);
          S.hist_ys[end] = 1.0 / ys;
          const double cau = ss * sqrt(gg) * lp.cautious_factor;
          if (ys > cau) {
            ++bound;
            bound = mem < bound ? mem : bound;
            end = (end + 1) % mem;
            if (stage == 2) st_sumb += bound;
            constexpr int PF0 = TOPAY_PF_ELEMS / EPL < TOPAY_PF_MAX ? TOPAY_PF_ELEMS / EPL : TOPAY_PF_MAX;
            constexpr int PF = PF0 < 1 ? 1 : PF0;
            SUBSTAMP_BEGIN(C);
            double dr[EPL];
            {
              double gv[EPL];
              vec_load<EPL>(S.g, n, tid, gv);
#pragma unroll
              for (int t = 0; t < EPL; t++) dr[t] = vec_in(tid, t, n) ? -gv[t] : 0.0;
            }
            double sb[PF][EPL], yb[PF][EPL], rb[PF];
            lds_dp alpha = C.X;
            const int endu = __builtin_amdgcn_readfirstlane(end), boundu = __builtin_amdgcn_readfirstlane(bound);
            const int memu = __builtin_amdgcn_readfirstlane(mem), nstr = __builtin_amdgcn_readfirstlane(S.nstride);
            const unsigned rbytes = (unsigned)nstr * 8u;
            typedef const TOPAY_GLB char* glb_ccp;
            auto load_pair = [&](int slot, int jj) {
              const unsigned ro = (unsigned)jj * rbytes;
              const glb_cdp sj = (glb_cdp)((glb_ccp)S.hist_s + ro);
              const glb_cdp yj = (glb_cdp)((glb_ccp)S.hist_y + ro);
#pragma unroll
              for (int p = 0; p < EPL / 2; p++) {
                const int i = 64 * p + tid;
                const dpair sv = row_pair_or_zero<true>(sj, n, i), yv = row_pair_or_zero<true>(yj, n, i);
                sb[slot][2 * p] = sv[0];
                sb[slot][2 * p + 1] = sv[1];
                yb[slot][2 * p] = yv[0];
                yb[slot][2 * p + 1] = yv[1];
              }
              rb[slot] = *(glb_cdp)((glb_ccp)S.hist_ys + (unsigned)jj * 8u);
            };
            auto step1 = [&](int u, int i) {
              double part = 0.0;
#pragma unroll
              for (int t = 0; t < EPL; t++) part = fma(sb[u][t], dr[t], part);
              const double al = wave_sum(part) * rb[u];
              alpha[i] = al;
#pragma unroll
              for (int t = 0; t < EPL; t++) dr[t] = fma(-al, yb[u][t], dr[t]);
            };
            int jl = endu;
#pragma unroll
            for (int u = 0; u < PF; u++) { jl = jl == 0 ? memu - 1 : jl - 1; load_pair(u, jl); }
            int i0 = 0;
            for (; i0 + PF <= boundu; i0 += PF) {
#pragma unroll
              for (int u = 0; u < PF; u++) {
                step1(u, i0 + u);
                jl = jl == 0 ? memu - 1 : jl - 1;
                load_pair(u, jl);
              }
            }
#pragma unroll
            for (int u = 0; u < PF - 1; u++)
              if (i0 + u < boundu) step1(u, i0 + u);
            const double scl = ys / yy;
#pragma unroll
            for (int t = 0; t < EPL; t++) dr[t] *= scl;
            lds_sync();
            auto step2 = [&](int u, int i) {
              const double av = alpha[boundu - 1 - i];
              double part = 0.0;
#pragma unroll
              for (int t = 0; t < EPL; t++) part = fma(yb[u][t], dr[t], part);
              const double beta = wave_sum(part) * rb[u];
              const double co = av - beta;
#pragma unroll
              for (int t = 0; t < EPL; t++) dr[t] = fma(co, sb[u][t], dr[t]);
            };
            jl = endu - boundu;
            jl = jl < 0 ? jl + memu : jl;
#pragma unroll
            for (int u = 0; u < PF; u++) { load_pair(u, jl); jl = jl + 1 == memu ? 0 : jl + 1; }
            for (i0 = 0; i0 + PF <= boundu; i0 += PF) {
#pragma unroll
              for (int u = 0; u < PF; u++) {
                step2(u, i0 + u);
                load_pair(u, jl);
                jl = jl + 1 == memu ? 0 : jl + 1;
              }
            }
#pragma unroll
            for (int u = 0; u < PF - 1; u++)
              if (i0 + u < boundu) step2(u, i0 + u);
            vec_store<EPL>(S.d, n, tid, dr);
            SUBSTAMP_END(C, 10);
          }
          step = 1.0;
          go = GO_LS_BEGIN;
        }
      }
    }

    LSTAMP(12);
    if (go == GO_LS_BEGIN) {
      {
        double xv[EPL], gv[EPL];
        vec_load<EPL>(S.x, n, tid, xv);
        vec_load<EPL>(S.g, n, tid, gv);
        vec_store<EPL>(S.xp, n, tid, xv);
        vec_store<EPL>(S.gp, n, tid, gv);
      }
      stp = step;
      count = 0;
      brackt = false;
      touched = false;
      mu = 0.0;
      nu = lp.max_step;
      int err = 0;
      if (!(stp > 0.0)) err = TOPAY_LBFGSERR_INVALIDPARAMETERS;
      else {
        dginit = wave_sum(vec_dot_part<EPL>(S.gp, S.d, n, tid));
        if (0.0 < dginit) err = TOPAY_LBFGSERR_INCREASEGRADIENT;
      }
      if (err) {
// ... 241 lines not shown
```

Baseline: 7688.

## Keep banded LU factors resident in LDS for small-N and latency kernels

Adds an RES template path where the 14-row banded LU factors stay in an extra LDS region instead of being copied to global memory. The forward/back band sweeps then read coefficients from LDS with a blocked six-row register sweep. This is enabled for the smallest solve/eval class and the latency kernels. It removes global writes and reads of the factors on every cost/gradient evaluation, at the price of extra LDS per workgroup, which could reduce occupancy.

New measurement: 7522. 2.2% lower.

```diff
diff --git a/topay_amd/csrc/topay_eval.h b/topay_amd/csrc/topay_eval.h
--- a/topay_amd/csrc/topay_eval.h
+++ b/topay_amd/csrc/topay_eval.h
@@ -206,7 +206,7 @@
   }
 }
 
-template <int STAGE, int RMAX, int NW, int OCC = 1>
+template <int STAGE, int RMAX, int NW, int OCC = 1, bool RES = false>
 __device__ __noinline__ TOPAY_CALLS_BIG_FUNCTIONS double eval_cost_grad(EvalCtx& C, const TOPAY_GLB DevMap* mp, const GradGate gate) {
   constexpr int NT = 64 * NW;
   const lds_dp c_Tp = uniform_ptr(C.Tp);
@@ -252,7 +252,7 @@
   const lds_dp csr = c_red + RD + 2 * npl;
   TOPAY_LDS unsigned long long* jmask = (TOPAY_LDS unsigned long long*)(c_red + RD + 2 * npl + (NW > 1 ? 2 * NW * 64 : 0));
   constexpr int PBR = eval_pb_rows(NW);
-  minco_generate<NW, OCC>(C);
+  minco_generate<NW, OCC, RES>(C);
 
   auto jerk_terms = [&](int i, double& e_out, double& gdT_out) __attribute__((always_inline)) {
     double w33 = 0, w43 = 0, w44 = 0, w53 = 0, w54 = 0, w55 = 0;
@@ -958,8 +958,14 @@
   if (wave == 0) {
     const bool owner = lane < 9;
     const lds_dp mine = c_adj + (owner ? lane : 8) * rows;
-    band_sweep<2>(mine, owner, (glb_cdp)c_lu, c_X, rows, lane);
-    band_sweep<3>(mine, owner, (glb_cdp)c_lu, c_X, rows, lane);
+    if constexpr (RES) {
+      lds_cdp lu_res = uniform_ptr(C.luL);
+      band_sweep_resident<2>(mine, owner, lu_res, rows);
+      band_sweep_resident<3>(mine, owner, lu_res, rows);
+    } else {
+      band_sweep<2>(mine, owner, (glb_cdp)c_lu, c_X, rows, lane);
+      band_sweep<3>(mine, owner, (glb_cdp)c_lu, c_X, rows, lane);
+    }
   }
   wg_barrier<NW>();
   STAMP(C, 7);
diff --git a/topay_amd/csrc/topay_eval_ctx.h b/topay_amd/csrc/topay_eval_ctx.h
--- a/topay_amd/csrc/topay_eval_ctx.h
+++ b/topay_amd/csrc/topay_eval_ctx.h
@@ -68,6 +68,7 @@
   lds_dp gC;
   glb_dp sbuf;
   int sb_stride;
+  lds_dp luL;
   glb_dp mstash;
   lds_dp pw;
   lds_dp X;
@@ -126,10 +127,10 @@
 __host__ __device__ constexpr int eval_borrow_doubles(int Nmax, int NW) { return eval_union_doubles(Nmax, NW) - 9 * 6 * Nmax; }
 template <typename P>
 struct EvalLds {
-  P Tp, gdT, pcs, pw, red, cL, adj, gC, X;
+  P Tp, gdT, pcs, pw, red, cL, adj, gC, X, luL;
 };
 template <typename L, typename P>
-__host__ __device__ constexpr P eval_lds_plan(L& C, P base, int Nmax, int NW) {
+__host__ __device__ constexpr P eval_lds_plan(L& C, P base, int Nmax, int NW, bool res = false) {
   const int rows = 6 * Nmax;
   P p = base;
   C.Tp = p; p += 5 * Nmax;
@@ -141,14 +142,16 @@
   C.adj = C.cL;
   C.gC = C.adj;
   C.X = p + 9 * rows;
-  return p + eval_union_doubles(Nmax, NW);
+  p += eval_union_doubles(Nmax, NW);
+  if (res) { C.luL = p; p += kLuPerPiece * Nmax; }
+  return p;
 }
-__host__ __device__ constexpr int eval_lds_total(int Nmax, int NW) {
+__host__ __device__ constexpr int eval_lds_total(int Nmax, int NW, bool res = false) {
   EvalLds<int> offsets{};
-  return eval_lds_plan(offsets, 0, Nmax, NW);
+  return eval_lds_plan(offsets, 0, Nmax, NW, res);
 }
-__device__ __forceinline__ void eval_lds_carve(EvalCtx& C, lds_dp base, int Nmax, int NW) {
-  eval_lds_plan(C, base, Nmax, NW);
+__device__ __forceinline__ void eval_lds_carve(EvalCtx& C, lds_dp base, int Nmax, int NW, bool res = false) {
+  eval_lds_plan(C, base, Nmax, NW, res);
   C.npass_lds = eval_npass(Nmax);
 }
 static_assert(eval_lds_total(10, 1) == 1515 && eval_lds_total(15, 1) == 1967 && eval_lds_total(21, 1) == 2509 &&
@@ -158,5 +161,6 @@
               eval_lds_total(32, 4) == 7162 && eval_lds_total(42, 4) == 8066 && eval_lds_total(64, 4) == 10054 &&
               eval_lds_total(85, 4) == 11954 && eval_lds_total(128, 4) == 15840 && eval_lds_total(TOPAY_MAX_N, 4) == 19638,
               "LDS plan, four waves");
+static_assert(eval_lds_total(10, 1, true) == 1515 + 840 && eval_lds_total(32, 4, true) == 7162 + 2688, "LDS plan, resident factors");
 
 }
diff --git a/topay_amd/csrc/topay_host_batch.h b/topay_amd/csrc/topay_host_batch.h
--- a/topay_amd/csrc/topay_host_batch.h
+++ b/topay_amd/csrc/topay_host_batch.h
@@ -268,7 +268,7 @@
     const bool lat = !EVAL && ct[k].lat && (c->latency_mode == 2 || (c->latency_mode == 1 && c->B <= c->simd_slots));
     size_t lds = class_lds_bytes(ct[k], nm);
     if (lat) {
-      lds = (size_t)(eval_lds_total(nm, kLatWaves) + solve_tail_doubles(true)) * sizeof(double);
+      lds = (size_t)(eval_lds_total(nm, kLatWaves, true) + solve_tail_doubles(true)) * sizeof(double);
       grid = nk;
     }
     if (k == topay_ctx::NBUCKET - 2 && !c->cls[topay_ctx::NBUCKET - 1].empty() && c->bstream[k] == c->stream)
diff --git a/topay_amd/csrc/topay_host_ctx.h b/topay_amd/csrc/topay_host_ctx.h
--- a/topay_amd/csrc/topay_host_ctx.h
+++ b/topay_amd/csrc/topay_host_ctx.h
@@ -130,18 +130,21 @@
   int solver_rmax = 0;
   int srmax() const { return solver_rmax ? solver_rmax : rmax; }
   bool helpers() const { return nw > 1; }
+  bool lu_resident = false;
 };
 static const int kLatWaves = 4;
 static const ClassDef kClassTable[TOPAY_NBUCKET] = {
-    {10, 1, 1, k_solve1, k_eval1, 2, k_lat1}, {15, 2, 1, k_solve2, k_eval2, 2, k_lat2}, {21, 2, 1, k_solve2, k_eval2, 2, k_lat2},
+    {10, 1, 1, k_solve1, k_eval1, 2, k_lat1, 0, true}, {15, 2, 1, k_solve2, k_eval2, 2, k_lat2}, {21, 2, 1, k_solve2, k_eval2, 2, k_lat2},
     {32, 3, 1, k_solve3, k_eval3, 2, k_lat3},
     {42, 2, 4, k_long5, k_eval2w4, 2, nullptr, 5}, {64, 2, 4, k_long5, k_eval2w4, 2, nullptr, 5},
     {TOPAY_MAX_N, 4, 4, k_long14, k_eval4w4, 2, nullptr, 14}};
 static const double kOcc2Gain = 1.7;
 static const int kLdsDoublesPerCU = 160 * 1024 / 8;
 static size_t class_lds_bytes(const ClassDef& cd, int nm) {
-  return (size_t)(eval_lds_total(nm, cd.nw) + solve_tail_doubles(cd.helpers())) * sizeof(double);
-}
+  return (size_t)(eval_lds_total(nm, cd.nw, cd.lu_resident) + solve_tail_doubles(cd.helpers())) * sizeof(double);
+}
+static_assert((eval_lds_total(10, 1, true) + solve_tail_doubles(false)) * 8 * sizeof(double) <= (size_t)kLdsDoublesPerCU * 8,
+              "class 0 with resident factors: eight workgroups per compute unit");
 
 __attribute__((constructor)) static void topay_request_hw_queues() { setenv("GPU_MAX_HW_QUEUES", "24", 0); }
 struct topay_ctx;
diff --git a/topay_amd/csrc/topay_host_results.h b/topay_amd/csrc/topay_host_results.h
--- a/topay_amd/csrc/topay_host_results.h
+++ b/topay_amd/csrc/topay_host_results.h
@@ -2,7 +2,7 @@
 #pragma once
 
 static bool class_for_waves(int N, int nw, ClassDef& out) {
-  static const ClassDef w1[] = {{10, 1, 1, nullptr, k_eval1, 2}, {21, 2, 1, nullptr, k_eval2, 2}, {32, 3, 1, nullptr, k_eval3, 2},
+  static const ClassDef w1[] = {{10, 1, 1, nullptr, k_eval1, 2, nullptr, 0, true}, {21, 2, 1, nullptr, k_eval2, 2}, {32, 3, 1, nullptr, k_eval3, 2},
                                 {42, 4, 1, nullptr, k_eval4, 2}, {64, 6, 1, nullptr, k_eval6, 2}};
   static const ClassDef w2[] = {{42, 2, 2, nullptr, k_eval2w2, 2}, {64, 3, 2, nullptr, k_eval3w2, 2}};
   static const ClassDef w4[] = {{85, 2, 4, nullptr, k_eval2w4, 2}, {128, 3, 4, nullptr, k_eval3w4, 2}, {TOPAY_MAX_N, 4, 4, nullptr, k_eval4w4, 2}};
diff --git a/topay_amd/csrc/topay_kernels.h b/topay_amd/csrc/topay_kernels.h
--- a/topay_amd/csrc/topay_kernels.h
+++ b/topay_amd/csrc/topay_kernels.h
@@ -31,12 +31,12 @@
   return (long long)(((unsigned long long)hi << 32) | lo);
 }
 
-template <int NW>
+template <int NW, bool RES = false>
 __host__ __device__ __forceinline__ int eval_lds_doubles(int Nmax_lds) {
-  return eval_lds_total(Nmax_lds, NW);
-}
-
-template <int NW>
+  return eval_lds_total(Nmax_lds, NW, RES);
+}
+
+template <int NW, bool RES = false>
 __device__ __forceinline__ void load_ctx(EvalCtx& C, const DevBatch& Bt, int b, int Nmax_lds) {
   C.tid = threadIdx.x;
   C.lane = threadIdx.x & 63;
@@ -45,7 +45,7 @@
   C.rows = 6 * C.N;
   C.n = 10 * C.N - 8;
   C.red = nullptr; C.adj = nullptr; C.cl_in_lds = 1;
-  eval_lds_carve(C, TOPAY_LDS_PTR, Nmax_lds, NW);
+  eval_lds_carve(C, TOPAY_LDS_PTR, Nmax_lds, NW, RES);
   fill_power_table(C.pw, C.lane);
   C.hd = (glb_cdp)(Bt.head + (size_t)b * kHeadLen);
   C.tl = (glb_cdp)(Bt.tail + (size_t)b * kHeadLen);
@@ -82,13 +82,13 @@
   for (int t = C.tid; t < 2 * N; t += NT) kn[2 + t] = C.pcs[2 * N + 2 + t];
 }
 
-template <int RMAX, int NW, int OCC>
+template <int RMAX, int NW, int OCC, bool RES = false>
 __device__ __forceinline__ void eval_body(const DevBatch& Bt, const DevMap* maps, int stage, int Nmax_lds, int repeats) {
   const int b = Bt.order[blockIdx.x];
   const bool commit = (stage & 16) != 0;
   stage &= 15;
   EvalCtx C;
-  load_ctx<NW>(C, Bt, b, Nmax_lds);
+  load_ctx<NW, RES>(C, Bt, b, Nmax_lds);
   const TOPAY_GLB DevMap* mp = (const TOPAY_GLB DevMap*)(maps + __builtin_amdgcn_readfirstlane(Bt.map_id[b]));
   const long long no = uniform_i64(Bt.noff[b]);
   C.x = (glb_cdp)Bt.x_of(no);
@@ -104,8 +104,8 @@
     gate.always = !cost_only; gate.has_early = false; gate.finit = 0.0; gate.thr = -1.0e300; gate.early = 0.0;
     gate.early_ok = false; gate.skip_thr = 0.0;
     __syncthreads();
-    if (stage == 1) f = eval_cost_grad<1, RMAX, NW, OCC>(C, mp, gate);
-    else f = eval_cost_grad<2, RMAX, NW, OCC>(C, mp, gate);
+    if (stage == 1) f = eval_cost_grad<1, RMAX, NW, OCC, RES>(C, mp, gate);
+    else f = eval_cost_grad<2, RMAX, NW, OCC, RES>(C, mp, gate);
   }
   if (C.tid == 0) {
     Bt.fout[b] = f;
@@ -135,7 +135,7 @@
 template <int OCC>
 __device__ __noinline__ void feasibility_gate_in_solve(const FeasIO F, const TOPAY_GLB DevMap* mp) { feasibility_gate(F, mp); }
 
-template <int RMAX, int OCC, int NWE = 1, int RMAX_E = RMAX>
+template <int RMAX, int OCC, int NWE = 1, int RMAX_E = RMAX, bool RES = false>
 __device__ __forceinline__ void solve_one(const DevBatch& Bt, const DevMap* maps, int Nmax_lds, int b) {
   constexpr int NT = 64 * NWE;
   const unsigned long long t_begin = wall_clock64();
@@ -147,9 +147,9 @@
 #endif
   }
   EvalCtx C;
-  load_ctx<NWE>(C, Bt, b, Nmax_lds);
+  load_ctx<NWE, RES>(C, Bt, b, Nmax_lds);
   const TOPAY_GLB DevMap* mp = (const TOPAY_GLB DevMap*)(maps + __builtin_amdgcn_readfirstlane(Bt.map_id[b]));
-  lds_dp pf = TOPAY_LDS_PTR + eval_lds_doubles<NWE>(Nmax_lds);
+  lds_dp pf = TOPAY_LDS_PTR + eval_lds_doubles<NWE, RES>(Nmax_lds);
   const long long no = uniform_i64(Bt.noff[b]);
   const int n = C.n;
   SolveIO S;
@@ -180,10 +180,10 @@
     C.x = S.x;
     C.g = S.g;
     __syncthreads();
-    if (C.wave == 0) solve_trajectory<RMAX, OCC, NWE, RMAX_E>(C, mp, S, Bt.s1_past[b], pf, success, cost, interrupted);
-    else eval_helper_loop<RMAX_E, NWE, OCC>(C, mp, pf + kSolvePastDoubles + kSolveParkDoubles);
+    if (C.wave == 0) solve_trajectory<RMAX, OCC, NWE, RMAX_E, RES>(C, mp, S, Bt.s1_past[b], pf, success, cost, interrupted);
+    else eval_helper_loop<RMAX_E, NWE, OCC, RES>(C, mp, pf + kSolvePastDoubles + kSolveParkDoubles);
   } else {
-    solve_trajectory<RMAX, OCC>(C, mp, S, Bt.s1_past[b], pf, success, cost, interrupted);
+    solve_trajectory<RMAX, OCC, 1, RMAX, RES>(C, mp, S, Bt.s1_past[b], pf, success, cost, interrupted);
   }
   __syncthreads();
   store_result<NWE>(C, Bt, b);
@@ -240,7 +240,7 @@
   }
 }
 
-template <int RMAX, int OCC, int NWE = 1, int RMAX_E = RMAX>
+template <int RMAX, int OCC, int NWE = 1, int RMAX_E = RMAX, bool RES = false>
 __device__ __forceinline__ void drain_queues(const DevBatch& B, const DevMap* maps, int Nmax_lds, int my_class) {
   const bool queued = B.queue_next != nullptr;
   const int lowest = queued ? B.queue_lowest : my_class;
@@ -282,48 +282,48 @@
         continue;
       }
       if (pos >= count) break;
-      solve_one<RMAX, OCC, NWE, RMAX_E>(B, maps, Nmax_lds, B.order[off + pos]);
+      solve_one<RMAX, OCC, NWE, RMAX_E, RES>(B, maps, Nmax_lds, B.order[off + pos]);
       __syncthreads();
     }
   }
 }
 
-template <int RMAX, int OCC, int NWE = 1, int RMAX_E = RMAX>
+template <int RMAX, int OCC, int NWE = 1, int RMAX_E = RMAX, bool RES = false>
 __device__ __forceinline__ void solve_body(const DevBatch& Bt, const DevMap* maps, int Nmax_lds) {
-  drain_queues<RMAX, OCC, NWE, RMAX_E>(Bt, maps, Nmax_lds, Bt.queue_class);
-}
-
-#define TOPAY_SOLVE_KERNEL(NAME, R, OCC)                                                             \
+  drain_queues<RMAX, OCC, NWE, RMAX_E, RES>(Bt, maps, Nmax_lds, Bt.queue_class);
+}
+
+#define TOPAY_SOLVE_KERNEL(NAME, R, OCC, RES)                                                        \
   __global__ void __launch_bounds__(64, OCC) NAME(DevBatch Bt, const DevMap* maps, int Nmax_lds) {   \
-    solve_body<R, OCC>(Bt, maps, Nmax_lds);                                                          \
-  }
-#define TOPAY_LATENCY_KERNEL(NAME, RS, RE, WE, OCC)                                                        \
+    solve_body<R, OCC, 1, R, RES>(Bt, maps, Nmax_lds);                                               \
+  }
+#define TOPAY_LATENCY_KERNEL(NAME, RS, RE, WE, OCC, RES)                                                   \
   __global__ void __launch_bounds__(64 * WE, OCC) NAME(DevBatch Bt, const DevMap* maps, int Nmax_lds) {    \
-    solve_body<RS, OCC, WE, RE>(Bt, maps, Nmax_lds);                                                       \
-  }
-#define TOPAY_EVAL_KERNEL(NAME, R, W, OCC)                                                                          \
+    solve_body<RS, OCC, WE, RE, RES>(Bt, maps, Nmax_lds);                                                  \
+  }
+#define TOPAY_EVAL_KERNEL(NAME, R, W, OCC, RES)                                                                     \
   __global__ void __launch_bounds__(64 * W, OCC) NAME(DevBatch Bt, const DevMap* maps, int stage, int repeats, int Nmax_lds) { \
-    eval_body<R, W, OCC>(Bt, maps, stage, Nmax_lds, repeats);                                              \
+    eval_body<R, W, OCC, RES>(Bt, maps, stage, Nmax_lds, repeats);                                         \
   }
 #ifndef TOPAY_NO_KERNEL_TABLE
-TOPAY_SOLVE_KERNEL(k_solve1, 1, 2)
-TOPAY_SOLVE_KERNEL(k_solve2, 2, 2)
-TOPAY_SOLVE_KERNEL(k_solve3, 3, 2)
-TOPAY_LATENCY_KERNEL(k_long5, 5, 2, 4, 2)
-TOPAY_LATENCY_KERNEL(k_long14, 14, 4, 4, 2)
-TOPAY_LATENCY_KERNEL(k_lat1, 1, 1, 4, 2)
-TOPAY_LATENCY_KERNEL(k_lat2, 2, 1, 4, 2)
-TOPAY_LATENCY_KERNEL(k_lat3, 3, 1, 4, 2)
-TOPAY_EVAL_KERNEL(k_eval1, 1, 1, 2)
-TOPAY_EVAL_KERNEL(k_eval2, 2, 1, 2)
-TOPAY_EVAL_KERNEL(k_eval3, 3, 1, 2)
-TOPAY_EVAL_KERNEL(k_eval2w2, 2, 2, 2)
-TOPAY_EVAL_KERNEL(k_eval3w2, 3, 2, 2)
-TOPAY_EVAL_KERNEL(k_eval3w4, 3, 4, 2)
-TOPAY_EVAL_KERNEL(k_eval4w4, 4, 4, 2)
-TOPAY_EVAL_KERNEL(k_eval4, 4, 1, 2)
-TOPAY_EVAL_KERNEL(k_eval6, 6, 1, 2)
-TOPAY_EVAL_KERNEL(k_eval2w4, 2, 4, 2)
+TOPAY_SOLVE_KERNEL(k_solve1, 1, 2, true)
+TOPAY_SOLVE_KERNEL(k_solve2, 2, 2, false)
+TOPAY_SOLVE_KERNEL(k_solve3, 3, 2, false)
+TOPAY_LATENCY_KERNEL(k_long5, 5, 2, 4, 2, false)
+TOPAY_LATENCY_KERNEL(k_long14, 14, 4, 4, 2, false)
+TOPAY_LATENCY_KERNEL(k_lat1, 1, 1, 4, 2, true)
+TOPAY_LATENCY_KERNEL(k_lat2, 2, 1, 4, 2, true)
+TOPAY_LATENCY_KERNEL(k_lat3, 3, 1, 4, 2, true)
+TOPAY_EVAL_KERNEL(k_eval1, 1, 1, 2, true)
+TOPAY_EVAL_KERNEL(k_eval2, 2, 1, 2, false)
+TOPAY_EVAL_KERNEL(k_eval3, 3, 1, 2, false)
+TOPAY_EVAL_KERNEL(k_eval2w2, 2, 2, 2, false)
+TOPAY_EVAL_KERNEL(k_eval3w2, 3, 2, 2, false)
+TOPAY_EVAL_KERNEL(k_eval3w4, 3, 4, 2, false)
+TOPAY_EVAL_KERNEL(k_eval4w4, 4, 4, 2, false)
+TOPAY_EVAL_KERNEL(k_eval4, 4, 1, 2, false)
+TOPAY_EVAL_KERNEL(k_eval6, 6, 1, 2, false)
+TOPAY_EVAL_KERNEL(k_eval2w4, 2, 4, 2, false)
 #endif
 
 __global__ void __launch_bounds__(64, 2) k_feasible(DevBatch Bt, const DevMap* maps, double* cseq, double* tk, long long cap_panels,
diff --git a/topay_amd/csrc/topay_minco.h b/topay_amd/csrc/topay_minco.h
--- a/topay_amd/csrc/topay_minco.h
+++ b/topay_amd/csrc/topay_minco.h
@@ -111,7 +111,64 @@
   }
 }
 
-template <int NW, int OCC>
+template <int MODE>
+__device__ __forceinline__ void band_sweep_resident(lds_dp v, bool owner, lds_cdp lu, int rows) {
+  constexpr bool FWD = (MODE == 0 || MODE == 2);
+  constexpr bool SCALE = (MODE == 1 || MODE == 2);
+  constexpr int D0 = (MODE == 0 || MODE == 3) ? 7 : 0;
+  if (owner) {
+    double w[6];
+    double x;
+    if (FWD) {
+      x = v[0];
+#pragma unroll
+      for (int t = 0; t < 6; t++) w[t] = v[1 + t];
+    } else {
+      x = v[rows - 1];
+#pragma unroll
+      for (int t = 0; t < 6; t++) w[t] = v[rows - 2 - t];
+    }
+#pragma unroll 1
+    for (int b0 = 0; b0 < rows; b0 += 6) {
+      double cf[6][6], sc[6], nw[6];
+#pragma unroll
+      for (int u = 0; u < 6; u++) {
+        const int j = FWD ? b0 + u : rows - 1 - (b0 + u);
+#pragma unroll
+        for (int t = 1; t <= 6; t++) {
+          int idx;
+          if (MODE == 0) idx = (D0 + t - 1) * rows + j;
+          else if (MODE == 1) idx = (D0 + 6 - t) * rows + j;
+          else if (MODE == 2) idx = (D0 + 6 - t) * rows + j + t;
+          else idx = (D0 + t - 1) * rows + j - t;
+          cf[u][t - 1] = lu[idx];
+        }
+        if (SCALE) sc[u] = lu[13 * rows + j];
+        int in = FWD ? j + 7 : j - 7;
+        in = in < 0 ? 0 : (in > rows - 1 ? rows - 1 : in);
+        nw[u] = v[in];
+      }
+      double xo[6];
+#pragma unroll
+      for (int u = 0; u < 6; u++) {
+        const double xs = SCALE ? x * sc[u] : x;
+        xo[u] = xs;
+#pragma unroll
+        for (int t = 0; t < 6; t++) w[(u + t) % 6] -= cf[u][t] * xs;
+        x = w[u % 6];
+        w[u % 6] = nw[u];
+      }
+#pragma unroll
+      for (int u = 0; u < 6; u++) {
+        const int j = FWD ? b0 + u : rows - 1 - (b0 + u);
+        v[j] = xo[u];
+      }
+    }
+  }
+  lds_sync();
+}
+
+template <int NW, int OCC, bool RES>
 __device__ __noinline__ void minco_generate(EvalCtx& C) {
   constexpr int NT = 64 * NW;
   const lds_dp c_Tp = C.Tp;
@@ -124,8 +181,8 @@
   const int tid = C.tid, lane = C.lane, wave = __builtin_amdgcn_readfirstlane(C.wave);
   const int N = __builtin_amdgcn_readfirstlane(C.N), rows = __builtin_amdgcn_readfirstlane(C.rows);
   lds_dp cL = C.cL;
-  lds_dp band = cL;
-  lds_dp rdiag = cL + 13 * rows;
+  lds_dp band = RES ? C.luL : cL;
+  lds_dp rdiag = band + 13 * rows;
   glb_cdp Tau = c_x;
   glb_cdp Theta = c_x + N;
   glb_cdp Arc = c_x + 2 * N - 1;
@@ -212,9 +269,11 @@
   STAMP(C, 1);
   for (int t = tid; t < rows; t += NT) rdiag[t] = 1.0 / BAND(t, t);
   wg_barrier<NW>();
-  for (int t = tid; t < 14 * rows; t += NT) c_lu[t] = band[t];
-  if (NW == 1) lds_sync();
-  else { wave_global_sync(); wg_barrier<NW>(); }
+  if constexpr (!RES) {
+    for (int t = tid; t < 14 * rows; t += NT) c_lu[t] = band[t];
+    if (NW == 1) lds_sync();
+    else { wave_global_sync(); wg_barrier<NW>(); }
+  }
   for (int t = tid; t < 9 * rows; t += NT) cL[t] = 0.0;
   wg_barrier<NW>();
   if (tid < 9) {
@@ -239,8 +298,13 @@
   if (wave == 0) {
     const bool owner = lane < 9;
     const lds_dp mine = cL + (owner ? lane : 8) * rows;
-    band_sweep<0>(mine, owner, (glb_cdp)c_lu, c_X, rows, lane);
-    band_sweep<1>(mine, owner, (glb_cdp)c_lu, c_X, rows, lane);
+    if constexpr (RES) {
+      band_sweep_resident<0>(mine, owner, (lds_cdp)band, rows);
+      band_sweep_resident<1>(mine, owner, (lds_cdp)band, rows);
+    } else {
+      band_sweep<0>(mine, owner, (glb_cdp)c_lu, c_X, rows, lane);
+      band_sweep<1>(mine, owner, (glb_cdp)c_lu, c_X, rows, lane);
+    }
   }
   C.cl_in_lds = 1;
   wg_barrier<NW>();
diff --git a/topay_amd/csrc/topay_solve.h b/topay_amd/csrc/topay_solve.h
--- a/topay_amd/csrc/topay_solve.h
+++ b/topay_amd/csrc/topay_solve.h
@@ -84,7 +84,7 @@
   return kSolvePastDoubles + kSolveParkDoubles + (helpers ? TOPAY_CMD_DOUBLES : 0);
 }
 static_assert(kLbfgsMaxMem <= eval_borrow_doubles(1, 1) && kLbfgsMaxMem <= eval_borrow_doubles(1, 4), "the alpha ring fits behind the coefficients");
-template <int RMAX_E, int NWE, int OCC>
+template <int RMAX_E, int NWE, int OCC, bool RES = false>
 __device__ __forceinline__ void eval_helper_loop(EvalCtx& C, const TOPAY_GLB DevMap* mp, lds_dp cmd) {
   for (;;) {
     __syncthreads();
@@ -95,8 +95,8 @@
     C.lam0 = cmd[4]; C.lam1 = cmd[5]; C.rho0 = cmd[6]; C.rho1 = cmd[7];
     const int stage = __builtin_amdgcn_readfirstlane(ic[1]);
     gate.always = ic[2] != 0; gate.has_early = ic[3] != 0; gate.early_ok = ic[4] != 0;
-    if (stage == 1) (void)eval_cost_grad<1, RMAX_E, NWE, OCC>(C, mp, gate);
-    else (void)eval_cost_grad<2, RMAX_E, NWE, OCC>(C, mp, gate);
+    if (stage == 1) (void)eval_cost_grad<1, RMAX_E, NWE, OCC, RES>(C, mp, gate);
+    else (void)eval_cost_grad<2, RMAX_E, NWE, OCC, RES>(C, mp, gate);
     wg_lds_barrier();
   }
 }
@@ -111,7 +111,7 @@
 #else
 #define LSTAMP(k) do { } while (0)
 #endif
-template <int RMAX, int OCC = 2, int NWE = 1, int RMAX_E = RMAX>
+template <int RMAX, int OCC = 2, int NWE = 1, int RMAX_E = RMAX, bool RES = false>
 __device__ __forceinline__ void solve_trajectory(EvalCtx& C, const TOPAY_GLB DevMap* mp, SolveIO& S, int s1_past,
                                                  lds_dp pf , int& success_out,
                                                  double& cost_out, int& interrupted_out) {
@@ -209,8 +209,8 @@
       __syncthreads();
     }
     LSTAMP(15);
-    if (stage == 1) f = eval_cost_grad<1, RMAX_E, NWE, OCC>(C, mp, gate);
-    else f = eval_cost_grad<2, RMAX_E, NWE, OCC>(C, mp, gate);
+    if (stage == 1) f = eval_cost_grad<1, RMAX_E, NWE, OCC, RES>(C, mp, gate);
+    else f = eval_cost_grad<2, RMAX_E, NWE, OCC, RES>(C, mp, gate);
 #ifdef TOPAY_STAMPS
     lt_ = (long long)__builtin_amdgcn_s_memtime();
 #endif
```
